# wh-xu/Hyper-Gen

Hardware: AMD Instinct MI355X
Metric: genomes/sec sketch (k=21,s=1500,D=4096) (higher is better)
Workload: dtype u64

## Files before the change

hyper-gen_amd/__init__.py:

```python
import ctypes as C
import os
import threading
import subprocess

import numpy as np

_HERE = os.path.dirname(os.path.abspath(__file__))
LIB_PATH = (os.environ.get("HYPERGEN_LIB") or None) or os.path.join(_HERE, "libhypergen_hip.so")
CLI_PATH = os.path.join(_HERE, "hyper-gen")

LAYOUT_SCALAR, LAYOUT_AVX2 = 0, 1
GATHER_PEER, GATHER_RCCL = 0, 1
ANI_MASH, ANI_CONTAINMENT, ANI_MAX_CONTAINMENT = 0, 1, 2
PAIRS_MASH, PAIRS_CONTAINMENT, PAIRS_MAX_CONTAINMENT, PAIRS_CONTAINMENT_REF = 1, 2, 4, 8
PAIRS_EMPTY = 0xFFFFFFFF
NORM_ACGT, NORM_U2T = 0, 1
(OK, ERR_INVALID, ERR_NO_DEVICE, ERR_HIP, ERR_OOM, ERR_CAPACITY, ERR_UNSUPPORTED, ERR_IO,
 ERR_INEXACT) = range(9)


T_NAMES = ("kmer", "sort", "encode", "dist_prep", "dist")
T_COUNT = len(T_NAMES)


class HgError(RuntimeError):
    def __init__(self, status, msg):
        super().__init__("hypergen status %d: %s" % (status, msg))
        self.status = status


class SketchParams(C.Structure):
    _fields_ = [("ksize", C.c_uint32), ("canonical", C.c_uint32), ("scaled", C.c_uint64),
                ("seed", C.c_uint64), ("hv_d", C.c_uint32), ("hv_layout", C.c_uint32),
                ("norm_mode", C.c_uint32), ("min_count", C.c_uint32)]


class AniHit(C.Structure):
    _fields_ = [("ref_idx", C.c_uint32), ("qry_idx", C.c_uint32), ("ani", C.c_float)]


ANI_HIT_DTYPE = np.dtype([("ref_idx", "<u4"), ("qry_idx", "<u4"), ("ani", "<f4")])
HAM_HIT_DTYPE = np.dtype([("ref_idx", "<u4"), ("qry_idx", "<u4"), ("dist", "<u4")])


class FileSketch(C.Structure):
    _fields_ = [("ksize", C.c_uint8), ("canonical", C.c_uint8), ("hv_quant_bits", C.c_uint8),
                ("pad", C.c_uint8), ("hv_norm_2", C.c_int32), ("scaled", C.c_uint64),
                ("seed", C.c_uint64), ("hv_d", C.c_uint64), ("file_str", C.c_char_p),
                ("hv", C.POINTER(C.c_int16)), ("hv_len", C.c_uint64)]


EXPORTS = [
    "hg_status_str", "hg_last_error", "hg_version", "hg_ctx_create", "hg_ctx_destroy",
    "hg_ctx_set_stream", "hg_ctx_reset_stream", "hg_ctx_sync", "hg_ctx_sketch_step_counts", "hg_sketch_plan_describe", "hg_logf_dev", "hg_ani_from_dots_dev", "hg_device_count", "hg_dev_alloc", "hg_dev_free",
    "hg_copy_h2d", "hg_copy_d2h", "hg_sketch_params_default", "hg_kmer_hash_sample",
    "hg_kmer_hash_sample_min_count",
    "hg_hv_encode", "hg_sketch_batch_dev", "hg_sketch_batch", "hg_dist_full", "hg_dist_full_dev",
    "hg_dist", "hg_dist_dev", "hg_sort_ani_hits", "hg_hv_quant_bits", "hg_hv_pack", "hg_hv_packed_bytes",
    "hg_hv_unpack", "hg_sketch_file_write", "hg_sketch_file_read", "hg_sketch_file_count",
    "hg_sketch_file_get", "hg_sketch_file_free", "hg_read_merge_seq", "hg_read_merge_seq_into", "hg_free",
    "hg_synth_genomes_dev", "hg_ctx_enable_timing", "hg_ctx_timings", "hg_ctx_last_kernel",
    "hg_hv_binarize_dev", "hg_hamming_full_dev", "hg_hamming_search_dev",
    "hg_ctx_set_debug", "hg_read_fastx_into", "hg_dist_block_dev", "hg_hamming_search_block_dev",
    "hg_multi_create", "hg_multi_destroy", "hg_multi_size", "hg_multi_ctx", "hg_multi_last_error", "hg_shard_range",
    "hg_multi_peer_report", "hg_multi_set_gather", "hg_multi_gather_mode", "hg_multi_gather_report",
    "hg_sketch_batch_multi", "hg_dist_multi", "hg_dist_multi_dev", "hg_hamming_search_multi",
    "hg_sort_ani_hits_dev", "hg_sort_ani_hits_staged", "hg_topk_per_query_dev", "hg_ctx_last_dist_path",
    "hg_ctx_last_hamming_path", "hg_read_fastx_pinned", "hg_pinned_free",
    "hg_sketch_stream_open", "hg_sketch_stream_push", "hg_sketch_stream_pop", "hg_sketch_stream_finish",
    "hg_sketch_stream_last_error", "hg_sketch_stream_close", "hg_sketch_stream_stats", "hg_device_numa_node", "hg_bind_thread_to_numa_node", "hg_dist_tile_order",
    "hg_sketch_stream_push_packed", "hg_pack2_size", "hg_pack2", "hg_unpack2_dev",
    "hg_sketch_stream_try_push", "hg_sketch_stream_max_pending",
    "hg_sketch_batch_dev_packed", "hg_pack2_batch_dev", "hg_pack2_dev",
    "hg_pack2s_size", "hg_pack2s", "hg_sketch_stream_push_packed_sparse",
    "hg_dist_ops_row_bytes", "hg_dist_ops_meta_bytes", "hg_dist_ops_padded_rows", "hg_dist_prep_ops_dev", "hg_dist_block_ops_dev",
    "hg_hv_packed_bytes_naive", "hg_hv_pack_naive", "hg_hv_unpack_naive", "hg_hv_payload_layout", "hg_hv_unpack_batch_dev",
    "hg_sketch_file_read_image", "hg_sketch_file_image", "hg_sketch_file_payload_offset",
    "hg_cluster_init_dev", "hg_cluster_add_hits_dev", "hg_cluster_finish_dev", "hg_cluster_dev", "hg_cluster",
    "hg_cluster_greedy_hits_dev", "hg_cluster_greedy_dev", "hg_cluster_greedy", "hg_ctx_cluster_greedy_rounds",
    "hg_cluster_setcover_hits_dev", "hg_cluster_setcover_dev", "hg_cluster_setcover", "hg_ctx_cluster_setcover_rounds",
    "hg_cluster_tree_hits_dev", "hg_cluster_tree_dev", "hg_cluster_tree", "hg_ctx_cluster_tree_rounds",
    "hg_cluster_average_matrix_dev", "hg_cluster_average_dev", "hg_cluster_average", "hg_ctx_cluster_average_rounds",
    "hg_cluster_stats_matrix_dev", "hg_cluster_stats_dev", "hg_cluster_stats",
    "hg_ctx_set_ani_metric", "hg_ctx_ani_metric", "hg_multi_set_ani_metric",
    "hg_search_topk_dev", "hg_search_topk_block_dev", "hg_search_topk", "hg_search_topk_merge", "hg_search_topk_multi_dev",
    "hg_ani_pairs_dev", "hg_ani_pairs",
]
SEARCH_TOPK_MAX = 64
CLUSTER_AVERAGE_MAX_N = 65536
STATS_NONE = 0xFFFFFFFF


class NodeStat(C.Structure):
    _fields_ = [("within_sum", C.c_uint64), ("within_min", C.c_uint32), ("within_min_idx", C.c_uint32),
                ("outside_max", C.c_uint32), ("outside_max_idx", C.c_uint32)]


class ClusterStat(C.Structure):
    _fields_ = [("within_sum", C.c_uint64), ("size", C.c_uint32), ("first", C.c_uint32), ("medoid", C.c_uint32),
                ("within_min", C.c_uint32), ("within_min_a", C.c_uint32), ("within_min_b", C.c_uint32),
                ("outside_max", C.c_uint32), ("outside_member", C.c_uint32), ("outside_idx", C.c_uint32), ("reserved", C.c_uint32)]


NODE_STAT_DTYPE = np.dtype([(name, np.uint64 if t is C.c_uint64 else np.uint32) for name, t in NodeStat._fields_])
CLUSTER_STAT_DTYPE = np.dtype([(name, np.uint64 if t is C.c_uint64 else np.uint32) for name, t in ClusterStat._fields_])


def source_stamp():
    import hashlib
    h = hashlib.sha256()
    src = os.path.join(_HERE, "csrc")
    files = sorted(f for f in os.listdir(src) if (f.endswith((".hip", ".h", ".cpp")) or f == "Makefile") and f != "hg_cli.cpp")
    for f in [os.path.join(src, x) for x in files] + [os.path.join(_HERE, "..", "include", "hypergen.h")]:
        h.update(os.path.basename(f).encode() + b"\0")
        h.update(open(f, "rb").read())
    return h.hexdigest()[:16]


def cli_source_stamp():
    import hashlib
    h = hashlib.sha256(source_stamp().encode())
    h.update(open(os.path.join(_HERE, "csrc", "hg_cli.cpp"), "rb").read())
    return h.hexdigest()[:16]


def build(force=False):
    if force:
        subprocess.check_call(["make", "-s", "-C", os.path.join(_HERE, "csrc"), "clean"])
    subprocess.check_call(["make", "-s", "-j4", "-C", os.path.join(_HERE, "csrc"), "all"])


_lib = None


def lib():
    global _lib
    if _lib is not None:
        return _lib
    if not os.path.exists(LIB_PATH):
        raise ImportError("libhypergen_hip.so is not built: run `python -c 'import __graft_entry__ as g; "
                          "g.build()'` (there is no CPU fallback)")
    L = C.CDLL(LIB_PATH)
    vp, sz = C.c_void_p, C.c_size_t
    u8p, u64p, i16p, i32p, u32p, f32p = (C.POINTER(t) for t in (
        C.c_uint8, C.c_uint64, C.c_int16, C.c_int32, C.c_uint32, C.c_float))
    sig = {
        "hg_status_str": (C.c_char_p, [C.c_int]),
        "hg_last_error": (C.c_char_p, [vp]),
        "hg_version": (C.c_char_p, []),
        "hg_ctx_create": (C.c_int, [C.c_int, C.POINTER(vp)]),
        "hg_ctx_destroy": (None, [vp]),
        "hg_ctx_set_stream": (C.c_int, [vp, vp]),
        "hg_ctx_reset_stream": (C.c_int, [vp]),
        "hg_ctx_sync": (C.c_int, [vp]),
        "hg_sketch_plan_describe": (C.c_int, [vp, vp, sz, C.c_uint32, C.c_uint64, C.POINTER(C.c_uint64), vp, sz]),
        "hg_logf_dev": (C.c_int, [vp, vp, C.c_uint32, sz, vp]),
        "hg_ani_from_dots_dev": (C.c_int, [vp, vp, vp, vp, sz, C.c_uint32, vp]),
        "hg_ctx_sketch_step_counts": (C.c_int, [vp, C.POINTER(C.c_uint64), C.POINTER(C.c_uint64), C.POINTER(C.c_uint64)]),
        "hg_device_count": (C.c_int, []),
        "hg_dev_alloc": (C.c_int, [vp, sz, C.POINTER(vp)]),
        "hg_dev_free": (C.c_int, [vp, vp]),
        "hg_copy_h2d": (C.c_int, [vp, vp, vp, sz]),
        "hg_copy_d2h": (C.c_int, [vp, vp, vp, sz]),
        "hg_sketch_params_default": (None, [C.POINTER(SketchParams)]),
        "hg_kmer_hash_sample": (C.c_int, [vp, vp, sz, C.c_uint32, C.c_uint64, C.c_uint64, C.c_int,
                                          C.c_uint32, vp, sz, C.POINTER(sz)]),
        "hg_kmer_hash_sample_min_count": (C.c_int, [vp, vp, sz, C.c_uint32, C.c_uint64, C.c_uint64, C.c_int,
                                                    C.c_uint32, C.c_uint32, vp, sz, C.POINTER(sz)]),
        "hg_hv_encode": (C.c_int, [vp, vp, sz, C.c_uint32, C.c_uint32, vp, C.POINTER(C.c_int32)]),
        "hg_sketch_batch_dev": (C.c_int, [vp, vp, vp, vp, sz, C.POINTER(SketchParams), vp, vp, vp]),
        "hg_sketch_batch": (C.c_int, [vp, C.POINTER(vp), C.POINTER(sz), sz, C.POINTER(SketchParams),
                                      vp, vp, vp]),
        "hg_dist_full": (C.c_int, [vp, vp, vp, sz, vp, vp, sz, C.c_uint32, C.c_uint32, vp]),
        "hg_dist_full_dev": (C.c_int, [vp, vp, vp, sz, vp, vp, sz, C.c_uint32, C.c_uint32, vp]),
        "hg_ani_pairs_dev": (C.c_int, [vp, vp, vp, sz, vp, vp, sz, C.c_uint32, C.c_uint32, vp, sz, C.c_uint32, vp, vp]),
        "hg_ani_pairs": (C.c_int, [vp, vp, vp, sz, vp, vp, sz, C.c_uint32, C.c_uint32, vp, sz, C.c_uint32, vp, vp]),
        "hg_dist": (C.c_int, [vp, vp, vp, sz, vp, vp, sz, C.c_uint32, C.c_uint32, C.c_int, C.c_float,
                              vp, sz, C.POINTER(sz)]),
        "hg_dist_dev": (C.c_int, [vp, vp, vp, sz, vp, vp, sz, C.c_uint32, C.c_uint32, C.c_int,
                                  C.c_float, vp, sz, C.POINTER(sz)]),
        "hg_sort_ani_hits": (None, [vp, sz, sz, C.c_int]),
        "hg_hv_quant_bits": (C.c_uint32, [vp, C.c_uint32]),
        "hg_hv_pack": (C.c_int, [vp, C.c_uint32, C.c_uint32, vp]),
        "hg_hv_packed_bytes": (sz, [C.c_uint32, C.c_uint32]),
        "hg_hv_unpack": (C.c_int, [vp, C.c_uint32, C.c_uint32, vp]),
        "hg_sketch_file_write": (C.c_int, [C.c_char_p, C.POINTER(FileSketch), sz]),
        "hg_sketch_file_read": (C.c_int, [C.c_char_p, C.POINTER(vp)]),
        "hg_sketch_file_count": (sz, [vp]),
        "hg_sketch_file_get": (C.POINTER(FileSketch), [vp, sz]),
        "hg_sketch_file_free": (None, [vp]),
        "hg_read_merge_seq": (C.c_int, [C.c_char_p, C.POINTER(vp), C.POINTER(sz)]),
        "hg_read_merge_seq_into": (C.c_int, [C.c_char_p, C.POINTER(vp), C.POINTER(sz), C.POINTER(sz)]),
        "hg_read_fastx_into": (C.c_int, [C.c_char_p, C.c_uint32, C.POINTER(vp), C.POINTER(sz), C.POINTER(sz)]),
        "hg_ctx_set_debug": (C.c_int, [vp, C.c_char_p, C.c_char_p]),
        "hg_free": (None, [vp]),
        "hg_read_fastx_pinned": (C.c_int, [C.c_char_p, C.c_uint32, C.POINTER(vp), C.POINTER(sz), C.POINTER(sz)]),
        "hg_pinned_free": (None, [vp]),
        "hg_device_numa_node": (C.c_int, [C.c_int]),
        "hg_bind_thread_to_numa_node": (C.c_int, [C.c_int, C.c_uint]),
        "hg_dist_tile_order": (C.c_int, [C.c_uint32, C.c_uint32, C.c_uint32, C.c_uint32, C.c_int, C.c_int, C.c_uint64, C.c_uint64,
                                         C.c_void_p, C.c_size_t, C.POINTER(C.c_size_t)]),
        "hg_sketch_stream_open": (C.c_int, [C.POINTER(C.c_int), C.c_int, C.POINTER(SketchParams), C.POINTER(vp)]),
        "hg_sketch_stream_push": (C.c_int, [vp, vp, sz, C.c_uint64]),
        "hg_sketch_stream_pop": (C.c_int, [vp, C.POINTER(C.c_uint64), vp, C.POINTER(C.c_int32), C.POINTER(C.c_uint32),
                                           C.POINTER(C.c_int)]),
        "hg_sketch_stream_push_packed": (C.c_int, [vp, vp, sz, C.c_uint64]),
        "hg_sketch_stream_try_push": (C.c_int, [vp, vp, sz, C.c_uint64, C.c_int]),
        "hg_sketch_stream_max_pending": (sz, [vp]),
        "hg_pack2_size": (sz, [sz]),
        "hg_pack2": (C.c_int, [vp, sz, C.c_uint32, vp]),
        "hg_unpack2_dev": (C.c_int, [vp, vp, sz, vp]),
        "hg_sketch_batch_dev_packed": (C.c_int, [vp, vp, vp, vp, sz, C.POINTER(SketchParams), vp, vp, vp]),
        "hg_pack2_batch_dev": (C.c_int, [vp, vp, vp, vp, sz, C.c_uint32, vp, vp]),
        "hg_pack2_dev": (C.c_int, [vp, vp, sz, C.c_uint32, vp]),
        "hg_dist_ops_row_bytes": (sz, [C.c_uint32]),
        "hg_dist_ops_meta_bytes": (sz, []),
        "hg_dist_ops_padded_rows": (sz, [sz]),
        "hg_dist_prep_ops_dev": (C.c_int, [vp, vp, sz, C.c_uint32, vp, vp, vp]),
        "hg_dist_block_ops_dev": (C.c_int, [vp, vp, vp, vp, sz, sz, vp, vp, sz, vp, vp, sz, sz, C.c_uint32, C.c_uint32, C.c_int,
                                            C.c_float, vp, sz, C.POINTER(sz)]),
        "hg_pack2s_size": (sz, [sz, sz]),
        "hg_pack2s": (C.c_int, [vp, sz, C.c_uint32, vp, sz, C.POINTER(sz)]),
        "hg_sketch_stream_push_packed_sparse": (C.c_int, [vp, vp, sz, sz, C.c_uint64]),
        "hg_sketch_stream_finish": (C.c_int, [vp]),
        "hg_sketch_stream_last_error": (C.c_char_p, [vp]),
        "hg_sketch_stream_close": (None, [vp]),
        "hg_sketch_stream_stats": (C.c_int, [vp, C.c_int, C.POINTER(C.c_double)]),
        "hg_ctx_last_dist_path": (C.c_int, [vp]),
        "hg_ctx_set_ani_metric": (C.c_int, [vp, C.c_int]),
        "hg_ctx_ani_metric": (C.c_int, [vp]),
        "hg_multi_set_ani_metric": (C.c_int, [vp, C.c_int]),
        "hg_ctx_last_hamming_path": (C.c_int, [vp]),
        "hg_sort_ani_hits_dev": (C.c_int, [vp, vp, sz, sz]),
        "hg_sort_ani_hits_staged": (C.c_int, [vp, vp, sz, sz]),
        "hg_topk_per_query_dev": (C.c_int, [vp, vp, sz, sz, C.c_uint32, vp, vp]),
        "hg_dist_block_dev": (C.c_int, [vp, vp, vp, sz, sz, vp, vp, sz, sz, C.c_uint32, C.c_uint32, C.c_int,
                                        C.c_float, vp, sz, C.POINTER(sz)]),
        "hg_hamming_search_block_dev": (C.c_int, [vp, vp, sz, sz, vp, sz, sz, C.c_uint32, C.c_uint32, vp, sz,
                                                  C.POINTER(sz)]),
        "hg_multi_create": (C.c_int, [C.POINTER(C.c_int), C.c_int, C.POINTER(vp)]),
        "hg_multi_destroy": (None, [vp]),
        "hg_multi_size": (C.c_int, [vp]),
        "hg_multi_ctx": (vp, [vp, C.c_int]),
        "hg_multi_last_error": (C.c_char_p, [vp]),
        "hg_multi_peer_report": (C.c_char_p, [vp]),
        "hg_multi_gather_report": (C.c_char_p, [vp]),
        "hg_multi_set_gather": (C.c_int, [vp, C.c_int]),
        "hg_multi_gather_mode": (C.c_int, [vp]),
        "hg_shard_range": (None, [sz, C.c_int, C.c_int, C.POINTER(sz), C.POINTER(sz)]),
        "hg_sketch_batch_multi": (C.c_int, [vp, C.POINTER(vp), C.POINTER(sz), sz, C.POINTER(SketchParams),
                                            vp, vp, vp]),
        "hg_dist_multi": (C.c_int, [vp, vp, vp, sz, vp, vp, sz, C.c_uint32, C.c_uint32, C.c_int, C.c_float,
                                    vp, sz, C.POINTER(sz)]),
        "hg_dist_multi_dev": (C.c_int, [vp, C.POINTER(vp), C.POINTER(vp), C.POINTER(sz), C.POINTER(vp),
                                        C.POINTER(vp), C.POINTER(sz), C.c_uint32, C.c_uint32, C.c_int,
                                        C.c_float, vp, sz, C.POINTER(sz)]),
        "hg_hamming_search_multi": (C.c_int, [vp, vp, sz, vp, sz, C.c_uint32, C.c_uint32, vp, sz, C.POINTER(sz)]),
        "hg_hv_binarize_dev": (C.c_int, [vp, vp, sz, C.c_uint32, vp]),
        "hg_hamming_full_dev": (C.c_int, [vp, vp, sz, vp, sz, C.c_uint32, vp]),
        "hg_hamming_search_dev": (C.c_int, [vp, vp, sz, vp, sz, C.c_uint32, C.c_uint32, vp, sz, C.POINTER(sz)]),
        "hg_ctx_enable_timing": (C.c_int, [vp, C.c_int]),
        "hg_ctx_last_kernel": (C.c_char_p, [vp, C.c_int]),
        "hg_ctx_timings": (C.c_int, [vp, C.POINTER(C.c_float), C.POINTER(C.c_uint32)]),
        "hg_synth_genomes_dev": (C.c_int, [vp, C.c_uint64, sz, C.c_uint64, C.c_uint32, C.c_uint32,
                                           C.c_uint64, vp]),
        "hg_hv_packed_bytes_naive": (sz, [C.c_uint32, C.c_uint32]),
        "hg_hv_pack_naive": (C.c_int, [vp, C.c_uint32, C.c_uint32, vp]),
        "hg_hv_unpack_naive": (C.c_int, [vp, C.c_uint32, C.c_uint32, vp]),
        "hg_hv_payload_layout": (C.c_int, [C.c_uint32, C.c_uint32, sz]),
        "hg_hv_unpack_batch_dev": (C.c_int, [vp, vp, sz, vp, vp, vp, sz, C.c_uint32, vp]),
        "hg_sketch_file_read_image": (C.c_int, [C.c_char_p, C.POINTER(vp)]),
        "hg_sketch_file_image": (vp, [vp, C.POINTER(sz)]),
        "hg_sketch_file_payload_offset": (C.c_uint64, [vp, sz]),
        "hg_cluster_init_dev": (C.c_int, [vp, vp, sz]),
        "hg_cluster_add_hits_dev": (C.c_int, [vp, vp, sz, vp, sz, C.c_float]),
        "hg_cluster_finish_dev": (C.c_int, [vp, vp, sz, vp, C.POINTER(sz)]),
        "hg_cluster_dev": (C.c_int, [vp, vp, vp, sz, C.c_uint32, C.c_uint32, C.c_float, vp, vp, C.POINTER(sz)]),
        "hg_cluster": (C.c_int, [vp, vp, vp, sz, C.c_uint32, C.c_uint32, C.c_float, vp, vp, C.POINTER(sz)]),
        "hg_cluster_greedy_hits_dev": (C.c_int, [vp, sz, vp, sz, C.c_float, vp, vp, vp, C.POINTER(sz)]),
        "hg_cluster_greedy_dev": (C.c_int, [vp, vp, vp, sz, C.c_uint32, C.c_uint32, C.c_float, vp, vp, vp, C.POINTER(sz)]),
        "hg_cluster_greedy": (C.c_int, [vp, vp, vp, sz, C.c_uint32, C.c_uint32, C.c_float, vp, vp, vp, C.POINTER(sz)]),
        "hg_ctx_cluster_greedy_rounds": (C.c_uint64, [vp]),
        "hg_cluster_setcover_hits_dev": (C.c_int, [vp, sz, vp, sz, C.c_float, vp, vp, vp, C.POINTER(sz)]),
        "hg_cluster_setcover_dev": (C.c_int, [vp, vp, vp, sz, C.c_uint32, C.c_uint32, C.c_float, vp, vp, vp, C.POINTER(sz)]),
        "hg_cluster_setcover": (C.c_int, [vp, vp, vp, sz, C.c_uint32, C.c_uint32, C.c_float, vp, vp, vp, C.POINTER(sz)]),
        "hg_ctx_cluster_setcover_rounds": (C.c_uint64, [vp]),
        "hg_cluster_tree_hits_dev": (C.c_int, [vp, sz, vp, sz, C.c_float, vp, sz, C.POINTER(sz), vp, vp, C.POINTER(sz)]),
        "hg_cluster_tree_dev": (C.c_int, [vp, vp, vp, sz, C.c_uint32, C.c_uint32, C.c_float, vp, sz, C.POINTER(sz), vp, vp, C.POINTER(sz)]),
        "hg_cluster_tree": (C.c_int, [vp, vp, vp, sz, C.c_uint32, C.c_uint32, C.c_float, vp, sz, C.POINTER(sz), vp, vp, C.POINTER(sz)]),
        "hg_ctx_cluster_tree_rounds": (C.c_uint64, [vp]),
        "hg_cluster_average_matrix_dev": (C.c_int, [vp, vp, sz, C.c_float, vp, vp, vp, vp, vp, C.POINTER(sz)]),
        "hg_cluster_average_dev": (C.c_int, [vp, vp, vp, sz, C.c_uint32, C.c_uint32, C.c_float, vp, vp, vp, vp, vp, C.POINTER(sz)]),
        "hg_cluster_average": (C.c_int, [vp, vp, vp, sz, C.c_uint32, C.c_uint32, C.c_float, vp, vp, vp, vp, vp, C.POINTER(sz)]),
        "hg_ctx_cluster_average_rounds": (C.c_uint64, [vp]),
        "hg_cluster_stats_matrix_dev": (C.c_int, [vp, vp, sz, vp, sz, vp, vp]),
        "hg_cluster_stats_dev": (C.c_int, [vp, vp, vp, sz, C.c_uint32, C.c_uint32, vp, sz, vp, vp]),
        "hg_cluster_stats": (C.c_int, [vp, vp, vp, sz, C.c_uint32, C.c_uint32, vp, sz, vp, vp]),
        "hg_search_topk_dev": (C.c_int, [vp, vp, vp, sz, vp, vp, sz, C.c_uint32, C.c_uint32, C.c_float, C.c_uint32, vp, vp]),
        "hg_search_topk_block_dev": (C.c_int, [vp, vp, vp, sz, sz, vp, vp, sz, sz, C.c_uint32, C.c_uint32, C.c_float, C.c_uint32,
                                               vp, vp]),
        "hg_search_topk": (C.c_int, [vp, vp, vp, sz, vp, vp, sz, C.c_uint32, C.c_uint32, C.c_float, C.c_uint32, vp, vp]),
        "hg_search_topk_merge": (C.c_int, [C.POINTER(vp), C.POINTER(vp), sz, sz, C.c_uint32, vp, vp]),
        "hg_search_topk_multi_dev": (C.c_int, [vp, C.POINTER(vp), C.POINTER(vp), C.POINTER(sz), C.POINTER(vp), C.POINTER(vp), sz,
                                               C.c_uint32, C.c_uint32, C.c_float, C.c_uint32, vp, vp]),
    }
    for name, (res, args) in sig.items():
        fn = getattr(L, name)
        fn.restype, fn.argtypes = res, args
    _lib = L
    return L


def _ptr(a):
    return C.c_void_p(a.ctypes.data) if isinstance(a, np.ndarray) else C.c_void_p(int(a))


def dist_tile_order(tiles_m, tiles_n, tile_rows=256, tile_cols=320, diagonal_first=False, symmetric=False, ref_off=0, qry_off=0):
    n = C.c_size_t(0)
    st = lib().hg_dist_tile_order(tiles_m, tiles_n, tile_rows, tile_cols, int(diagonal_first), int(symmetric), ref_off, qry_off,
                                  None, 0, C.byref(n))
    if st not in (OK, ERR_CAPACITY):
        raise HgError(st, "hg_dist_tile_order")
    out = np.zeros(max(n.value, 1), np.uint32)
    st = lib().hg_dist_tile_order(tiles_m, tiles_n, tile_rows, tile_cols, int(diagonal_first), int(symmetric), ref_off, qry_off,
                                  C.c_void_p(out.ctypes.data), out.size, C.byref(n))
    if st != OK:
        raise HgError(st, "hg_dist_tile_order")
    return out[: n.value]


def default_params(**kw):
    p = SketchParams()
    lib().hg_sketch_params_default(C.byref(p))
    for k, v in kw.items():
        setattr(p, k, v)
    return p


default_debug = {}


class Context:

    def __init__(self, device=0):
        self._h = C.c_void_p()
        st = lib().hg_ctx_create(device, C.byref(self._h))
        if st != OK:
            raise HgError(st, lib().hg_last_error(None).decode())
        for k, v in default_debug.items():
            self.set_debug(k, v)

    def close(self):
        if self._h:
            lib().hg_ctx_destroy(self._h)
            self._h = C.c_void_p()

    def __enter__(self):
        return self

    def __exit__(self, *a):
        self.close()

    def __del__(self):
        try:
            self.close()
        except Exception:
            pass

    def _ck(self, st, allow=()):
        if st != OK and st not in allow:
            raise HgError(st, lib().hg_last_error(self._h).decode())
        return st

    def set_stream(self, stream_handle):
        self._ck(lib().hg_ctx_set_stream(self._h, C.c_void_p(stream_handle or 0)))

    def set_debug(self, key, value):
        self._ck(lib().hg_ctx_set_debug(self._h, key.encode(), str(value).encode()))

    def reset_stream(self):
        self._ck(lib().hg_ctx_reset_stream(self._h))

    def sync(self):
        self._ck(lib().hg_ctx_sync(self._h))

    def logf_dev(self, d_out, n, d_x=None, first_bits=0):
        self._ck(lib().hg_logf_dev(self._h, C.c_void_p(d_x or 0), first_bits, n, C.c_void_p(d_out)))

    def ani_from_dots_dev(self, d_dot, d_nr, d_nq, n, ksize, d_ani):
        self._ck(lib().hg_ani_from_dots_dev(self._h, C.c_void_p(d_dot), C.c_void_p(d_nr), C.c_void_p(d_nq), n, ksize, C.c_void_p(d_ani)))

    def sketch_step_counts(self):
        a, b, c = C.c_uint64(), C.c_uint64(), C.c_uint64()
        self._ck(lib().hg_ctx_sketch_step_counts(self._h, C.byref(a), C.byref(b), C.byref(c)))
        return int(a.value), int(b.value), int(c.value)

    def last_kernel(self, cls):
        return lib().hg_ctx_last_kernel(self._h, T_NAMES.index(cls)).decode()

    def enable_timing(self, on=True):
        self._ck(lib().hg_ctx_enable_timing(self._h, int(on)))

    def timings(self):
        ms = (C.c_float * T_COUNT)()
        n = (C.c_uint32 * T_COUNT)()
        self._ck(lib().hg_ctx_timings(self._h, ms, n))
        return {name: (float(ms[i]), int(n[i])) for i, name in enumerate(T_NAMES)}

    def kmer_hash_sample(self, seq, ksize=21, scaled=1500, seed=123, canonical=True,
                         norm=NORM_ACGT, threshold=None, cap=None, min_count=1):
        a = np.ascontiguousarray(np.frombuffer(bytes(seq), np.uint8) if not isinstance(seq, np.ndarray) else seq,
                                 dtype=np.uint8)
        thr = (2**64 - 1) // scaled if threshold is None else threshold
        cap = cap if cap is not None else max(1024, a.size // max(1, scaled) * 2 + 1024)
        while True:
            out = np.zeros(max(cap, 1), np.uint64)
            n = C.c_size_t(0)
            if min_count > 1:
                st = lib().hg_kmer_hash_sample_min_count(self._h, _ptr(a) if a.size else None, a.size, ksize,
                                                         C.c_uint64(thr), C.c_uint64(seed), int(canonical), norm, min_count,
                                                         _ptr(out), cap, C.byref(n))
            else:
                st = lib().hg_kmer_hash_sample(self._h, _ptr(a) if a.size else None, a.size, ksize,
                                               C.c_uint64(thr), C.c_uint64(seed), int(canonical), norm,
                                               _ptr(out), cap, C.byref(n))
            if st == ERR_CAPACITY:
                cap = n.value
                continue
            self._ck(st)
            return out[: n.value].copy()

    def unpack2_dev(self, d_blob, n_bps, d_out):
        self._ck(lib().hg_unpack2_dev(self._h, C.c_void_p(d_blob), n_bps, C.c_void_p(d_out)))

    def hv_encode(self, hashes, hv_d=4096, layout=LAYOUT_AVX2):
        h = np.ascontiguousarray(hashes, dtype=np.uint64)
        hv = np.zeros(hv_d, np.int16)
        n2 = C.c_int32(0)
        self._ck(lib().hg_hv_encode(self._h, _ptr(h) if h.size else None, h.size, hv_d, layout,
                                    _ptr(hv), C.byref(n2)))
        return hv, int(n2.value)

    def sketch_batch(self, seqs, params=None):
        p = params or default_params()
        arrs = [np.ascontiguousarray(s, dtype=np.uint8) if isinstance(s, np.ndarray)
                else np.frombuffer(bytes(s), np.uint8) for s in seqs]
        n = len(arrs)
        ptrs = (C.c_void_p * max(n, 1))(*[a.ctypes.data if a.size else None for a in arrs])
        lens = (C.c_size_t * max(n, 1))(*[a.size for a in arrs])
        hv = np.zeros((n, p.hv_d), np.int16)
        n2 = np.zeros(n, np.int32)
        nh = np.zeros(n, np.uint32)
        self._ck(lib().hg_sketch_batch(self._h, ptrs, lens, n, C.byref(p), _ptr(hv), _ptr(n2), _ptr(nh)))
        return hv, n2, nh

    def dist_full(self, ref_hv, ref_n2, qry_hv, qry_n2, ksize=21):
        r = np.ascontiguousarray(ref_hv, np.int16)
        q = np.ascontiguousarray(qry_hv, np.int16)
        rn = np.ascontiguousarray(ref_n2, np.int32)
        qn = np.ascontiguousarray(qry_n2, np.int32)
        out = np.zeros((r.shape[0], q.shape[0]), np.float32)
        self._ck(lib().hg_dist_full(self._h, _ptr(r), _ptr(rn), r.shape[0], _ptr(q), _ptr(qn),
                                    q.shape[0], r.shape[1], ksize, _ptr(out)))
        return out

    def dist(self, ref_hv, ref_n2, qry_hv, qry_n2, ksize=21, symmetric=False, ani_th=85.0, cap=None):
        r = np.ascontiguousarray(ref_hv, np.int16)
        q = np.ascontiguousarray(qry_hv, np.int16)
        rn = np.ascontiguousarray(ref_n2, np.int32)
        qn = np.ascontiguousarray(qry_n2, np.int32)
        cap = cap if cap is not None else max(1024, r.shape[0] * q.shape[0] // 8)
        while True:
            out = np.zeros(cap, ANI_HIT_DTYPE)
            n = C.c_size_t(0)
            st = lib().hg_dist(self._h, _ptr(r), _ptr(rn), r.shape[0], _ptr(q), _ptr(qn), q.shape[0],
                               r.shape[1], ksize, int(symmetric), C.c_float(ani_th), _ptr(out), cap,
                               C.byref(n))
            if st == ERR_CAPACITY:
                cap = n.value
                continue
            self._ck(st)
            return out[: n.value].copy()

    def sketch_batch_dev(self, d_seq, offsets, lens, params, d_hv, d_norm2, d_nhash):
        off = np.ascontiguousarray(offsets, np.uint64)
        ln = np.ascontiguousarray(lens, np.uint64)
        self._ck(lib().hg_sketch_batch_dev(self._h, _ptr(d_seq), _ptr(off), _ptr(ln), off.size,
                                           C.byref(params), _ptr(d_hv), _ptr(d_norm2), _ptr(d_nhash)))

    def sketch_batch_dev_packed(self, d_blobs, offsets, n_bps, params, d_hv, d_norm2, d_nhash):
        off = np.ascontiguousarray(offsets, np.uint64)
        ln = np.ascontiguousarray(n_bps, np.uint64)
        self._ck(lib().hg_sketch_batch_dev_packed(self._h, _ptr(d_blobs), _ptr(off), _ptr(ln), off.size,
                                                  C.byref(params), _ptr(d_hv), _ptr(d_norm2), _ptr(d_nhash)))

    def pack2_batch_dev(self, d_seq, offsets, lens, d_blobs, blob_offsets, norm_mode=NORM_ACGT):
        off = np.ascontiguousarray(offsets, np.uint64)
        ln = np.ascontiguousarray(lens, np.uint64)
        bo = np.ascontiguousarray(blob_offsets, np.uint64)
        self._ck(lib().hg_pack2_batch_dev(self._h, _ptr(d_seq), _ptr(off), _ptr(ln), off.size, norm_mode, _ptr(d_blobs), _ptr(bo)))

    def pack2_dev(self, d_seq, n_bps, d_blob, norm_mode=NORM_ACGT):
        self._ck(lib().hg_pack2_dev(self._h, C.c_void_p(d_seq), n_bps, norm_mode, C.c_void_p(d_blob)))

    def synth_genomes_dev(self, first, n, L, stride, d_out, cluster_size=100, sub_ppm_per_member=1000):
        done = 0
        while done < n:
            m = min(n - done, 32768)
            self._ck(lib().hg_synth_genomes_dev(self._h, first + done, m, L, cluster_size, sub_ppm_per_member,
                                                stride, C.c_void_p(int(d_out) + done * stride)))
            done += m

    def hv_binarize_dev(self, d_hv, n, hv_d, d_bits):
        self._ck(lib().hg_hv_binarize_dev(self._h, _ptr(d_hv), n, hv_d, _ptr(d_bits)))

    def hamming_full_dev(self, d_ref, R, d_qry, Q, hv_d, d_out):
        self._ck(lib().hg_hamming_full_dev(self._h, _ptr(d_ref), R, _ptr(d_qry), Q, hv_d, _ptr(d_out)))

    def hamming_search_dev(self, d_ref, R, d_qry, Q, hv_d, max_dist, d_out, cap):
        n = C.c_size_t(0)
        st = lib().hg_hamming_search_dev(self._h, _ptr(d_ref), R, _ptr(d_qry), Q, hv_d, max_dist, _ptr(d_out), cap,
                                         C.byref(n))
        self._ck(st, allow=(ERR_CAPACITY,))
        return n.value, st

    def dist_full_dev(self, d_ref, d_rn, R, d_qry, d_qn, Q, hv_d, ksize, d_out):
        self._ck(lib().hg_dist_full_dev(self._h, _ptr(d_ref), _ptr(d_rn), R, _ptr(d_qry), _ptr(d_qn), Q,
                                        hv_d, ksize, _ptr(d_out)))

    def dist_block_dev(self, d_ref, d_rn, R, ref_off, d_qry, d_qn, Q, qry_off, hv_d, ksize, symmetric, ani_th,
                       d_out, cap):
        n = C.c_size_t(0)
        st = lib().hg_dist_block_dev(self._h, _ptr(d_ref), _ptr(d_rn), R, ref_off, _ptr(d_qry), _ptr(d_qn), Q,
                                     qry_off, hv_d, ksize, int(symmetric), C.c_float(ani_th), _ptr(d_out), cap,
                                     C.byref(n))
        self._ck(st, allow=(ERR_CAPACITY,))
        return n.value, st

    def dist_prep_ops_dev(self, d_hv, rows, hv_d, d_ops, d_meta, d_flag):
        self._ck(lib().hg_dist_prep_ops_dev(self._h, _ptr(d_hv), rows, hv_d, _ptr(d_ops), _ptr(d_meta), _ptr(d_flag)))

    def dist_block_ops_dev(self, d_ref_ops, d_ref_meta, d_rn, R, ref_off, d_ref_index, d_flags, n_flags, d_qry, d_qn, Q, qry_off,
                           hv_d, ksize, symmetric, ani_th, d_out, cap):
        n = C.c_size_t(0)
        st = lib().hg_dist_block_ops_dev(self._h, _ptr(d_ref_ops), _ptr(d_ref_meta), _ptr(d_rn), R, ref_off,
                                         _ptr(d_ref_index) if d_ref_index else None, _ptr(d_flags) if d_flags else None, n_flags,
                                         _ptr(d_qry), _ptr(d_qn), Q, qry_off, hv_d, ksize, int(symmetric), C.c_float(ani_th),
                                         _ptr(d_out), cap, C.byref(n))
        self._ck(st, allow=(ERR_CAPACITY, ERR_INEXACT))
# ... 470 lines not shown
    a = np.ascontiguousarray(seq, np.uint8)
    n = a.size
    cap = lib().hg_pack2_size(n) if cap is None else cap
    out = np.empty(max(cap, 16), np.uint8)
    size = C.c_size_t(0)
    st = lib().hg_pack2s(_ptr(a), n, norm_mode, _ptr(out), out.size, C.byref(size))
    if st == ERR_CAPACITY:
        return None
    if st != OK:
        raise HgError(st, "hg_pack2s")
    return out[:size.value]


def pack2(seq, norm_mode=0, in_place=False):
    a = np.ascontiguousarray(seq, np.uint8)
    n = a.size
    size = lib().hg_pack2_size(n)
    if in_place:
        buf = np.zeros(max(n, size), np.uint8)
        buf[:n] = a
        st = lib().hg_pack2(_ptr(buf), n, norm_mode, _ptr(buf))
        out = buf[:size]
    else:
        out = np.empty(size, np.uint8)
        st = lib().hg_pack2(_ptr(a), n, norm_mode, _ptr(out))
    if st != OK:
        raise HgError(st, "hg_pack2")
    return out


class PinnedReader:

    def __init__(self, slots=1):
        self._p = [C.c_void_p() for _ in range(slots)]
        self._cap = [C.c_size_t(0) for _ in range(slots)]

    def read(self, path, slot=0, mode=READ_MERGE):
        n = C.c_size_t(0)
        st = lib().hg_read_fastx_pinned(os.fsencode(path), mode, C.byref(self._p[slot]), C.byref(self._cap[slot]), C.byref(n))
        if st != OK:
            raise HgError(st, "hg_read_fastx_pinned(%s)" % path)
        if not n.value:
            return np.zeros(0, np.uint8)
        return np.ctypeslib.as_array(C.cast(self._p[slot], C.POINTER(C.c_uint8)), shape=(n.value,))

    def close(self):
        for p in self._p:
            if p:
                lib().hg_pinned_free(p)
                p.value = None

    def __enter__(self):
        return self

    def __exit__(self, *a):
        self.close()


class SketchStream:

    def __init__(self, device_ids=(0,), params=None):
        self.params = params or default_params()
        ids = (C.c_int * len(device_ids))(*device_ids)
        self._h = C.c_void_p()
        st = lib().hg_sketch_stream_open(ids, len(device_ids), C.byref(self.params), C.byref(self._h))
        if st != OK:
            raise HgError(st, "hg_sketch_stream_open: " + lib().hg_last_error(None).decode())
        self._keep = {}
        self._next = 0
        self._ready = []
        self._lock = threading.Lock()

    def _check(self, st, what):
        if st != OK:
            raise HgError(st, what + ": " + lib().hg_sketch_stream_last_error(self._h).decode())

    def _push(self, a, n_bps, tag, packed):
        with self._lock:
            iid = self._next
            self._next += 1
            self._keep[iid] = (tag, a)
        try:
            while True:
                st = lib().hg_sketch_stream_try_push(self._h, _ptr(a), n_bps, iid, int(packed))
                if st != ERR_CAPACITY:
                    break
                r = self._pop_c()
                if r is not None:
                    with self._lock:
                        self._ready.append(r)
        except BaseException:
            with self._lock:
                self._keep.pop(iid, None)
            raise
        if st != OK:
            with self._lock:
                self._keep.pop(iid, None)
        self._check(st, "hg_sketch_stream_try_push")

    def push(self, seq, tag):
        a = np.ascontiguousarray(seq, np.uint8)
        self._push(a, a.size, tag, 0)

    def push_packed(self, blob, n_bps, tag):
        a = np.ascontiguousarray(blob, np.uint8)
        assert a.size >= lib().hg_pack2_size(n_bps)
        self._push(a, n_bps, tag, 1)

    def push_packed_sparse(self, blob, n_bps, tag):
        a = np.ascontiguousarray(blob, np.uint8)
        tab = (((n_bps + 3) // 4) + 15) & ~15
        if n_bps and (a.size < tab + 8 or a.size < lib().hg_pack2s_size(n_bps, int(a[tab: tab + 4].view("<u4")[0]))):
            raise HgError(ERR_INVALID, "push_packed_sparse: the buffer is shorter than the blob it claims to hold")
        self._push(a, n_bps, tag, 2)

    def finish(self):
        self._check(lib().hg_sketch_stream_finish(self._h), "hg_sketch_stream_finish")

    def _pop_c(self):
        iid, n2, nh, got = C.c_uint64(), C.c_int32(), C.c_uint32(), C.c_int()
        hv = np.empty(self.params.hv_d, np.int16)
        self._check(lib().hg_sketch_stream_pop(self._h, C.byref(iid), _ptr(hv), C.byref(n2), C.byref(nh), C.byref(got)),
                    "hg_sketch_stream_pop")
        if not got.value:
            return None
        with self._lock:
            tag, _ = self._keep.pop(iid.value)
        return tag, hv, n2.value, nh.value

    def pop(self):
        with self._lock:
            if self._ready:
                return self._ready.pop(0)
        return self._pop_c()

    def stats(self, engine=0):
        out = (C.c_double * 6)()
        self._check(lib().hg_sketch_stream_stats(self._h, engine, out), "hg_sketch_stream_stats")
        return dict(zip(("uploader_idle_s", "uploader_no_chunk_s", "uploader_copy_s", "compute_idle_s", "compute_busy_s",
                         "chunks"), out))

    def close(self):
        if self._h:
            lib().hg_sketch_stream_close(self._h)
            self._h = C.c_void_p()

    def __enter__(self):
        return self

    def __exit__(self, *a):
        self.close()


def sketch_plan_describe(offsets, lens, ksize=21, scaled=1500):
    off = np.ascontiguousarray(offsets, np.uint64)
    ln = np.ascontiguousarray(lens, np.uint64)
    counts = (C.c_uint64 * 6)()
    st = lib().hg_sketch_plan_describe(_ptr(off), _ptr(ln), off.size, ksize, scaled, counts, None, 0)
    if st != OK:
        raise HgError(st, "hg_sketch_plan_describe")
    d = dict(zip(("items", "workgroups", "hit_slots", "max_cap", "max_expect", "item_tiles"), (int(x) for x in counts)))
    gf = None
    if ksize <= 32 and d["items"]:
        gf = np.zeros(d["workgroups"] + 1, np.uint32)
        st = lib().hg_sketch_plan_describe(_ptr(off), _ptr(ln), off.size, ksize, scaled, counts, _ptr(gf), gf.size)
        if st != OK:
            raise HgError(st, "hg_sketch_plan_describe")
    return d, gf


def write_sketch_file(path, records):
    arr = (FileSketch * max(len(records), 1))()
    keep = []
    for i, r in enumerate(records):
        hv = np.ascontiguousarray(r["hv"], np.int16)
        name = r["file_str"].encode()
        keep += [hv, name]
        arr[i] = FileSketch(r["ksize"], int(bool(r["canonical"])), r["hv_quant_bits"], 0, r["hv_norm_2"],
                            r["scaled"], r["seed"], r["hv_d"], name,
                            hv.ctypes.data_as(C.POINTER(C.c_int16)), hv.size)
    st = lib().hg_sketch_file_write(os.fsencode(path), arr, len(records))
    if st != OK:
        raise HgError(st, "hg_sketch_file_write(%s)" % path)


def read_sketch_file(path):
    h = C.c_void_p()
    st = lib().hg_sketch_file_read(os.fsencode(path), C.byref(h))
    if st != OK:
        raise HgError(st, "hg_sketch_file_read(%s)" % path)
    try:
        out = []
        for i in range(lib().hg_sketch_file_count(h)):
            r = lib().hg_sketch_file_get(h, i).contents
            hv = np.ctypeslib.as_array(r.hv, shape=(r.hv_len,)).copy() if r.hv_len else np.zeros(0, np.int16)
            out.append(dict(ksize=r.ksize, scaled=r.scaled, canonical=bool(r.canonical), seed=r.seed,
                            hv_d=r.hv_d, hv_quant_bits=r.hv_quant_bits, hv_norm_2=r.hv_norm_2,
                            file_str=r.file_str.decode(), hv=hv))
        return out
    finally:
        lib().hg_sketch_file_free(h)
```

hyper-gen_amd/csrc/hg_api.hip:

```cpp
#include <atomic>
#include <chrono>
#include <cstdlib>
#include <cstring>
#include <new>
#include <string>
#include <thread>

#include "hg_internal.h"

static thread_local std::string g_create_err;

hg_status hg_fail(hg_ctx *ctx, hg_status s, const std::string &msg) {
  if (ctx) ctx->err = msg;
  else g_create_err = msg;
  return s;
}

extern "C" const char *hg_status_str(hg_status s) {
  switch (s) {
    case HG_OK: return "ok";
    case HG_ERR_INVALID: return "invalid argument";
    case HG_ERR_NO_DEVICE: return "no usable HIP device";
    case HG_ERR_HIP: return "HIP runtime error";
    case HG_ERR_OOM: return "out of memory";
    case HG_ERR_CAPACITY: return "output capacity too small";
    case HG_ERR_UNSUPPORTED: return "unsupported parameters";
    case HG_ERR_IO: return "I/O error";
    case HG_ERR_INEXACT: return "no exact device path";
  }
  return "unknown";
}

extern "C" const char *hg_last_error(const hg_ctx *ctx) {
  return ctx ? ctx->err.c_str() : g_create_err.c_str();
}

extern "C" const char *hg_version(void) { return "hypergen-hip 0.1.0 (gfx950)"; }

extern "C" int hg_device_count(void) {
  int n = 0;
  if (hipGetDeviceCount(&n) != hipSuccess) return 0;
  return n;
}

extern "C" hg_status hg_ctx_create(int device_id, hg_ctx **out) {
  if (!out) return hg_fail(nullptr, HG_ERR_INVALID, "out == NULL");
  *out = nullptr;
  int n = 0;
  hipError_t e = hipGetDeviceCount(&n);
  if (e != hipSuccess || n <= 0)
    return hg_fail(nullptr, HG_ERR_NO_DEVICE,
                   std::string("hipGetDeviceCount: ") + (e == hipSuccess ? "0 devices" : hipGetErrorString(e)));
  if (device_id < 0 || device_id >= n)
    return hg_fail(nullptr, HG_ERR_NO_DEVICE, "device id out of range");
  hg_ctx *c = new (std::nothrow) hg_ctx();
  if (!c) return hg_fail(nullptr, HG_ERR_OOM, "ctx allocation");
  c->device = device_id;
  if ((e = hipSetDevice(device_id)) != hipSuccess ||
      (e = hipStreamCreateWithFlags(&c->own_stream, hipStreamNonBlocking)) != hipSuccess) {
    delete c;
    return hg_fail(nullptr, HG_ERR_HIP, std::string("ctx setup: ") + hipGetErrorString(e));
  }
  c->stream = c->own_stream;
  hipDeviceProp_t prop;
  if (hipGetDeviceProperties(&prop, device_id) == hipSuccess) c->n_cu = prop.multiProcessorCount;
  *out = c;
  return HG_OK;
}

extern "C" void hg_ctx_destroy(hg_ctx *c) {
  if (!c) return;
  (void)hipSetDevice(c->device);
  (void)hipStreamSynchronize(c->stream);
  hg_ctx::Buf *bufs[] = {&c->w_items, &c->w_gmeta, &c->w_hits, &c->w_cnt, &c->w_seq, &c->w_hv, &c->w_hits2, &c->w_lsort, &c->w_redo, &c->w_pk, &c->w_pktab,
                         &c->w_misc, &c->w_f16a, &c->w_f16b, &c->w_stats, &c->w_ani, &c->w_hv2, &c->w_cen,
                         &c->w_n2a, &c->w_n2b, &c->w_sorthits, &c->w_clu_res, &c->w_clu, &c->w_clu_hits, &c->w_grd, &c->w_setcover, &c->w_tree, &c->w_average, &c->w_cstats, &c->w_srch_blk, &c->w_srch_lists, &c->w_srch_state, &c->w_srch_out, &c->w_i8a, &c->w_i8b, &c->w_i8misc};
  for (auto *b : bufs)
    if (b->p) (void)hipFree(b->p);
  for (auto &t : c->tile_tabs) {
    if (t.dev.p) (void)hipFree(t.dev.p);
    if (t.uploaded) (void)hipEventDestroy(t.uploaded);
  }
  for (auto &t : c->t_pending) {
    if (t.own_e0) (void)hipEventDestroy(t.e0);
    (void)hipEventDestroy(t.e1);
  }
  for (auto e : c->t_pool) (void)hipEventDestroy(e);
  if (c->h_res) (void)hipHostFree(c->h_res);
  if (c->h_pin) (void)hipHostFree(c->h_pin);
  if (c->h_chk) (void)hipHostFree(c->h_chk);
  if (c->h_plan) (void)hipHostFree(c->h_plan);
  if (c->plan_uploaded) (void)hipEventDestroy(c->plan_uploaded);
  for (auto e : c->copy_events) (void)hipEventDestroy(e);
  for (int i = 0; i < 2; ++i) {
    if (c->pack_buf[i]) (void)hipHostFree(c->pack_buf[i]);
    if (c->pack_ev[i]) (void)hipEventDestroy(c->pack_ev[i]);
  }
  if (c->copy_stream) (void)hipStreamDestroy(c->copy_stream);
  if (c->own_stream) (void)hipStreamDestroy(c->own_stream);
  delete c;
}

static hg_status switch_stream(hg_ctx *c, hipStream_t to) {
  if (to == c->stream) return HG_OK;
  HG_ENTER(c);
  HG_HIP(c, hipStreamSynchronize(c->stream));
  c->stream = to;
  return HG_OK;
}

extern "C" hg_status hg_ctx_set_stream(hg_ctx *c, void *hip_stream) {
  if (!c) return HG_ERR_INVALID;
  return switch_stream(c, reinterpret_cast<hipStream_t>(hip_stream));
}

extern "C" hg_status hg_ctx_reset_stream(hg_ctx *c) {
  if (!c) return HG_ERR_INVALID;
  return switch_stream(c, c->own_stream);
}

extern "C" int hg_ctx_last_dist_path(const hg_ctx *c) { return c ? c->last_dist_path : -1; }

extern "C" hg_status hg_ctx_set_ani_metric(hg_ctx *c, int metric) {
  if (!c) return HG_ERR_INVALID;
  if (metric != HG_ANI_MASH && metric != HG_ANI_CONTAINMENT && metric != HG_ANI_MAX_CONTAINMENT)
    return hg_fail(c, HG_ERR_INVALID, "unknown ANI metric " + std::to_string(metric));
  c->ani_metric = metric;
  return HG_OK;
}

extern "C" int hg_ctx_ani_metric(const hg_ctx *c) { return c ? c->ani_metric : HG_ANI_MASH; }

extern "C" hg_status hg_ctx_set_debug(hg_ctx *c, const char *key, const char *value) {
  if (!c || !key) return HG_ERR_INVALID;
  const std::string k = key, v = value ? value : "";
  if (k == "dist_tile") c->dbg_dist_tile = v;
  else if (k == "sort_test_buckets") c->dbg_sort_buckets = std::atoi(v.c_str());
  else if (k == "pair_limit") c->dbg_pair_limit = std::strtoull(v.c_str(), nullptr, 10);
  else if (k == "cluster_hit_cap") c->dbg_cluster_hit_cap = std::strtoull(v.c_str(), nullptr, 10);
  else if (k == "tree_rounds") c->dbg_tree_rounds = std::strtoull(v.c_str(), nullptr, 10);
  else if (k == "setcover_rounds") c->dbg_setcover_rounds = std::strtoull(v.c_str(), nullptr, 10);
  else if (k == "greedy_rounds") c->dbg_greedy_rounds = std::strtoull(v.c_str(), nullptr, 10);
  else if (k == "average_rounds") c->dbg_average_rounds = std::strtoull(v.c_str(), nullptr, 10);
  else if (k == "average_block_rows") c->dbg_average_block_rows = std::strtoull(v.c_str(), nullptr, 10);
  else if (k == "stats_block_rows") c->dbg_stats_block_rows = std::strtoull(v.c_str(), nullptr, 10);
  else if (k == "search_block_rows") c->dbg_search_block_rows = std::strtoull(v.c_str(), nullptr, 10);
  else if (k == "dist_path") c->dbg_dist_path = v;
  else if (k == "dist_order") c->dbg_dist_order = v;
  else if (k == "ham_path") c->dbg_ham_path = v;
  else if (k == "hostfed") c->dbg_hostfed = v;
  else if (k == "hostfed_stage_bytes") c->dbg_hostfed_stage_bytes = std::strtoull(v.c_str(), nullptr, 10);
  else if (k == "sketch_path") c->dbg_sketch_path = v;
  else if (k == "kmer_input") c->dbg_kmer_input = v;
  else return hg_fail(c, HG_ERR_INVALID, "unknown debug key " + k);
  return HG_OK;
}

extern "C" hg_status hg_ctx_sync(hg_ctx *c) {
  if (!c) return HG_ERR_INVALID;
  HG_ENTER(c);
  HG_HIP(c, hipStreamSynchronize(c->stream));
  return HG_OK;
}

extern "C" hg_status hg_ctx_sketch_step_counts(hg_ctx *c, uint64_t *sync_free, uint64_t *synchronous, uint64_t *redone) {
  if (!c) return HG_ERR_INVALID;
  if (sync_free) *sync_free = c->n_fast_steps;
  if (synchronous) *synchronous = c->n_sync_steps;
  if (redone) *redone = c->n_redone_steps;
  return HG_OK;
}

static hipEvent_t take_event(hg_ctx *c) {
  if (!c->t_pool.empty()) {
    hipEvent_t e = c->t_pool.back();
    c->t_pool.pop_back();
    return e;
  }
  hipEvent_t e = nullptr;
  if (hipEventCreate(&e) != hipSuccess) return nullptr;
  return e;
}

hg_timed::hg_timed(hg_ctx *ctx, int cls_, int after_cls) : c(ctx), cls(cls_) {
  hipEvent_t chain = c->t_chain;
  c->t_chain = nullptr;
  if (!c->timing) return;
  if (after_cls >= 0 && chain && c->t_chain_cls == after_cls) e0 = chain, own_e0 = false;
  else e0 = take_event(c);
  e1 = take_event(c);
  if (e0 && own_e0) (void)hipEventRecord(e0, c->stream);
}
hg_timed::~hg_timed() {
  if (!e0 || !e1) return;
  (void)hipEventRecord(e1, c->stream);
  c->t_pending.push_back({e0, e1, cls, own_e0});
  c->t_chain = e1, c->t_chain_cls = cls;
}

extern "C" hg_status hg_ctx_enable_timing(hg_ctx *c, int on) {
  if (!c) return HG_ERR_INVALID;
  c->timing = on != 0;
  c->t_chain = nullptr, c->t_chain_cls = -1;
  return HG_OK;
}

extern "C" const char *hg_ctx_last_kernel(const hg_ctx *c, int cls) {
  return (c && cls >= 0 && cls < HG_T_COUNT) ? c->last_kernel[cls].c_str() : "";
}

extern "C" hg_status hg_ctx_timings(hg_ctx *c, float ms_sum[HG_T_COUNT], uint32_t launches[HG_T_COUNT]) {
  if (!c || !ms_sum || !launches) return HG_ERR_INVALID;
  for (int i = 0; i < HG_T_COUNT; ++i) ms_sum[i] = 0.f, launches[i] = 0;
  hipError_t first_err = hipSuccess;
  const char *first_what = "";
  for (auto &t : c->t_pending) {
    if (first_err != hipSuccess) break;
    hipError_t e = hipEventSynchronize(t.e1);
    float ms = 0.f;
    if (e == hipSuccess) e = hipEventElapsedTime(&ms, t.e0, t.e1);
    if (e != hipSuccess) {
      first_err = e, first_what = "hg_ctx_timings: event read";
      break;
    }
    if (t.cls >= 0 && t.cls < HG_T_COUNT) ms_sum[t.cls] += ms, launches[t.cls] += 1;
  }
  for (auto &t : c->t_pending) {
    if (t.own_e0) c->t_pool.push_back(t.e0);
    c->t_pool.push_back(t.e1);
  }
  c->t_pending.clear();
  c->t_chain = nullptr;
  if (first_err != hipSuccess) return hg_fail(c, HG_ERR_HIP, std::string(first_what) + ": " + hipGetErrorString(first_err));
  return HG_OK;
}

hg_status hg_ensure(hg_ctx *c, hg_ctx::Buf &b, size_t bytes) {
  if (bytes <= b.cap) return HG_OK;
  HG_HIP(c, hipStreamSynchronize(c->stream));
  if (b.p) {
    (void)hipFree(b.p);
    b.p = nullptr;
    b.cap = 0;
  }
  size_t want = bytes + bytes / 4 + 256;
  hipError_t e = hipMalloc(&b.p, want);
  if (e != hipSuccess) {
    b.p = nullptr;
    return hg_fail(c, HG_ERR_OOM, "hipMalloc(" + std::to_string(want) + "): " + hipGetErrorString(e));
  }
  b.cap = want;
  return HG_OK;
}

namespace {
__global__ void publish_words_kernel(uint32_t *__restrict__ src, uint32_t n, volatile uint32_t *dst, uint32_t seq, uint32_t zero_n) {
  if (threadIdx.x < n) dst[threadIdx.x] = src[threadIdx.x];
  if (threadIdx.x < zero_n) src[threadIdx.x] = 0u;
  __threadfence_system();
  __syncthreads();
  if (threadIdx.x == 0) {
    dst[16] = seq;
    __threadfence_system();
  }
}
}

hg_status hg_publish_words(hg_ctx *c, uint32_t *d_words, uint32_t n, const uint32_t **out, uint32_t zero_n) {
  if (n > 16 || zero_n > 64) return hg_fail(c, HG_ERR_INVALID, "hg_publish_words: at most 16 words");
  if (!c->h_res) {
    void *p = nullptr;
    hipError_t e = hipHostMalloc(&p, 32 * sizeof(uint32_t), hipHostMallocCoherent);
    if (e != hipSuccess) return hg_fail(c, HG_ERR_OOM, std::string("hipHostMalloc: ") + hipGetErrorString(e));
    c->h_res = static_cast<uint32_t *>(p);
    std::memset(c->h_res, 0, 32 * sizeof(uint32_t));
  }
  const uint32_t seq = ++c->res_seq ? c->res_seq : ++c->res_seq;
  hipLaunchKernelGGL(publish_words_kernel, dim3(1), dim3(64), 0, c->stream, d_words, n, c->h_res, seq, zero_n);
  HG_HIP(c, hipGetLastError());
  volatile uint32_t *flag = c->h_res + 16;
  const auto t0 = std::chrono::steady_clock::now();
  bool seen = false;
  for (uint32_t spins = 0; !seen; ++spins) {
    if (*flag == seq) {
      seen = true;
      break;
    }
#if defined(__x86_64__) || defined(__i386__)
    __builtin_ia32_pause();
#else
    std::this_thread::yield();
#endif
    if ((spins & 0x3ff) == 0x3ff &&
        std::chrono::steady_clock::now() - t0 > std::chrono::microseconds(800))
      break;
  }
  if (!seen) {
    const hipError_t e = hipStreamSynchronize(c->stream);
    if (e != hipSuccess) return hg_fail(c, HG_ERR_HIP, std::string("hipStreamSynchronize: ") + hipGetErrorString(e));
    if (*flag != seq) return hg_fail(c, HG_ERR_HIP, "hg_publish_words: the stream finished without publishing");
  }
  std::atomic_thread_fence(std::memory_order_acquire);
  *out = c->h_res;
  return HG_OK;
}

hg_status hg_ensure_pinned(hg_ctx *c, size_t bytes) {
  if (bytes <= c->h_pin_cap) return HG_OK;
  HG_HIP(c, hipStreamSynchronize(c->stream));
  if (c->h_pin) (void)hipHostFree(c->h_pin);
  c->h_pin = nullptr, c->h_pin_cap = 0;
  size_t want = bytes + bytes / 4 + 4096;
  hipError_t e = hipHostMalloc(&c->h_pin, want, hipHostMallocDefault);
  if (e != hipSuccess) return hg_fail(c, HG_ERR_OOM, std::string("hipHostMalloc: ") + hipGetErrorString(e));
  c->h_pin_cap = want;
  return HG_OK;
}

extern "C" hg_status hg_dev_alloc(hg_ctx *c, size_t bytes, void **dptr) {
  if (!c || !dptr) return HG_ERR_INVALID;
  HG_ENTER(c);
  hipError_t e = hipMalloc(dptr, bytes ? bytes : 1);
  if (e != hipSuccess) return hg_fail(c, HG_ERR_OOM, std::string("hipMalloc: ") + hipGetErrorString(e));
  return HG_OK;
}
// ... 38 lines not shown
```

hyper-gen_amd/csrc/hg_internal.h:

```cpp
#pragma once
#include <hip/hip_runtime.h>
#include <stddef.h>
#include <stdint.h>

#include <algorithm>
#include <atomic>
#include <memory>
#include <string>
#include <vector>

#include "../../include/hypergen.h"
#include "hg_pack2.h"

struct hg_sketch_plan {
  std::vector<uint64_t> offs, lens, masks;
  std::vector<uint32_t> caps;
  uint32_t ksize = 0;
  bool packed = false;
  uint64_t scaled = 0, total_slots = 0;
  uint32_t max_cap = 0;
  uint32_t max_expect = 0;
  uint32_t max_hits = 0;
  size_t n_items = 0;
  size_t n_groups = 0;
};
struct hg_genome_batch {
  const uint8_t *d_seq = nullptr;
  const uint64_t *offsets = nullptr, *lens = nullptr;
  const uint64_t *mask_offs = nullptr;
  size_t n = 0;
  bool packed = false;
};
struct hg_sketch_out {
  int16_t *d_hv = nullptr;
  int32_t *d_norm2 = nullptr;
  uint32_t *d_nhash = nullptr;
};
struct hg_sketch_pending {
  bool active = false;
  uint32_t seq = 0;
  int slot = 0;
  std::shared_ptr<const hg_sketch_plan> plan;
  hg_genome_batch batch;
  hg_sketch_params p{};
  hg_sketch_out out;
};

struct hg_ctx {
  int device = 0;
  hipStream_t own_stream = nullptr;
  hipStream_t stream = nullptr;
  std::string err;
  int n_cu = 256;

  struct Buf {
    void *p = nullptr;
    size_t cap = 0;
  };
  Buf w_items;
  Buf w_gmeta;
  Buf w_hits;
  Buf w_cnt;
  Buf w_hits2;
  Buf w_lsort;
  Buf w_redo;
  Buf w_pk;
  Buf w_pktab;
  Buf w_seq;
  Buf w_hv;
  Buf w_misc;
  const void *misc_zeroed = nullptr;
  Buf w_f16a;
  Buf w_f16b;
  Buf w_stats;
  Buf w_ani;
  Buf w_hv2;
  Buf w_n2a, w_n2b;
  Buf w_i8a, w_i8b, w_i8misc;
  struct I8Pad {
    const void *ptr = nullptr;
    uint32_t rows = 0, padded = 0, pitch = 0;
  } i8_pad[2];
  Buf w_cen;
  struct TileTab {
    uint32_t tiles_m = 0, tiles_n = 0, bm = 0, bn = 0, flags = 0, n_slots = 0;
    uint64_t ref_off = 0, qry_off = 0, used = 0;
    Buf dev;
    std::vector<uint32_t> host;
    hipEvent_t uploaded = nullptr;
  } tile_tabs[8];
  uint64_t tile_tab_clock = 0;
  std::string last_kernel_cen;
  const void *cen_sig_ref = nullptr, *cen_sig_qry = nullptr;
  uint32_t cen_sig_r = 0, cen_sig_q = 0, cen_sig_d = 0;
  int last_ham_path = -1;
  std::string last_kernel[HG_T_COUNT];
  std::string last_kernel_i8;
  std::string last_kernel_win;
  int ani_metric = HG_ANI_MASH;
  int last_dist_path = -1;
  const void *i8_sig_ref = nullptr, *i8_sig_qry = nullptr;
  uint32_t i8_sig_r = 0, i8_sig_q = 0, i8_sig_d = 0;
  uint32_t i8_skip = 0;
  Buf w_sorthits;
  Buf w_clu_res;
  Buf w_clu;
  Buf w_clu_hits;
  Buf w_grd;
  uint64_t greedy_rounds = 0;
  Buf w_setcover;
  uint64_t setcover_rounds = 0;
  Buf w_tree;
  uint64_t tree_rounds = 0;
  Buf w_average;
  uint64_t average_rounds = 0;
  Buf w_cstats;
  Buf w_srch_blk;
  Buf w_srch_lists;
  Buf w_srch_state;
  Buf w_srch_out;
  bool timing = false;
  struct TimedLaunch {
    hipEvent_t e0, e1;
    int cls;
    bool own_e0;
  };
  hipEvent_t t_chain = nullptr;
  int t_chain_cls = -1;
  std::vector<TimedLaunch> t_pending;
  std::vector<hipEvent_t> t_pool;
  std::shared_ptr<hg_sketch_plan> plan;
  hipEvent_t plan_uploaded = nullptr;
  bool plan_upload_pending = false;
  void *h_plan = nullptr;
  size_t h_plan_cap = 0;
  hg_sketch_pending pending;
  uint32_t *h_chk = nullptr;
  uint32_t chk_seq = 0;
  uint64_t n_fast_steps = 0, n_sync_steps = 0, n_redone_steps = 0;
  hipStream_t copy_stream = nullptr;
  std::vector<hipEvent_t> copy_events;
  void *pack_buf[2] = {nullptr, nullptr};
  size_t pack_cap[2] = {0, 0};
  hipEvent_t pack_ev[2] = {nullptr, nullptr};
  bool pack_used[2] = {false, false};
  const void *pad_a_ptr = nullptr, *pad_b_ptr = nullptr;
  uint32_t pad_a_rows = 0, pad_a_ldk = 0, pad_b_rows = 0, pad_b_ldk = 0;
  std::vector<const void *> lds_attr_done;
  std::string dbg_dist_tile, dbg_dist_path, dbg_ham_path, dbg_dist_order, dbg_kmer_input, dbg_hostfed, dbg_sketch_path;
  int dbg_sort_buckets = 0;
  uint64_t dbg_cluster_hit_cap = 0;
  uint64_t dbg_greedy_rounds = 0;
  uint64_t dbg_setcover_rounds = 0;
  uint64_t dbg_tree_rounds = 0;
  uint64_t dbg_average_rounds = 0;
  uint64_t dbg_average_block_rows = 0;
  uint64_t dbg_stats_block_rows = 0;
  uint64_t dbg_search_block_rows = 0;
  uint64_t dbg_hostfed_stage_bytes = 0;
  uint64_t dbg_pair_limit = 0;
  void *h_pin = nullptr;
  size_t h_pin_cap = 0;
  uint32_t *h_res = nullptr;
  uint32_t res_seq = 0;
};

hg_status hg_fail(hg_ctx *ctx, hg_status s, const std::string &msg);
hg_status hg_ensure(hg_ctx *ctx, hg_ctx::Buf &b, size_t bytes);
hg_status hg_ensure_pinned(hg_ctx *ctx, size_t bytes);
hg_status hg_publish_words(hg_ctx *ctx, uint32_t *d_words, uint32_t n, const uint32_t **out, uint32_t zero_n = 0);

struct hg_timed {
  hg_ctx *c;
  hipEvent_t e0 = nullptr, e1 = nullptr;
  int cls;
  bool own_e0 = true;
  hg_timed(hg_ctx *ctx, int cls_, int after_cls = -1);
  ~hg_timed();
};

#define HG_HIP(ctx, expr)                                                              \
  do {                                                                                 \
    hipError_t e__ = (expr);                                                           \
    if (e__ != hipSuccess)                                                             \
      return hg_fail((ctx), HG_ERR_HIP,                                                \
                     std::string(#expr) + ": " + hipGetErrorString(e__));              \
  } while (0)

hg_status hg_sketch_resolve(hg_ctx *ctx, bool *redone = nullptr);
#define HG_ENTER(ctx)                                        \
  do {                                                       \
    HG_HIP((ctx), hipSetDevice((ctx)->device));              \
    const hg_status s__ = hg_sketch_resolve((ctx));          \
    if (s__ != HG_OK) return s__;                            \
  } while (0)

struct hg_genome_meta {
  uint64_t seq_off;
  uint64_t n_bps;
  uint64_t hit_off;
  uint32_t hit_cap;
  uint32_t item_first;
  uint64_t mask_off;
};
hg_status hg_sketch_batch_dev_packed_masks(hg_ctx *c, const uint8_t *d_blobs, const uint64_t *code_offs, const uint64_t *mask_offs,
                                           const uint64_t *n_bps, size_t n, const hg_sketch_params *p, int16_t *d_hv,
                                           int32_t *d_norm2, uint32_t *d_nhash);

uint32_t hg_kmer_item_starts(uint32_t ksize);
const char *hg_kmer_kernel_name(uint32_t ksize, bool canonical, bool packed);

hipError_t hg_launch_kmer_sample(hipStream_t st, const uint8_t *d_seq, const hg_genome_meta *d_meta,
                                 const uint32_t *d_item_genome, uint32_t n_items, uint32_t ksize,
                                 uint64_t threshold, uint64_t seed, bool canonical, uint32_t norm_mode,
                                 uint64_t *d_hits, uint32_t *d_cnt, bool packed = false, const uint32_t *d_group_first = nullptr,
                                 uint32_t n_groups = 0);
uint32_t hg_kmer_tile_starts(uint32_t ksize);
uint32_t hg_kmer_item_tiles(uint32_t ksize);
hipError_t hg_launch_pack2(hipStream_t st, const uint8_t *d_seq, const uint64_t *d_tab, uint32_t n, uint32_t blocks_max,
                           uint32_t u2t, uint8_t *d_blobs);
hipError_t hg_launch_unpack2_jobs(hipStream_t st, const uint8_t *d_pk, uint8_t *d_out, const UnpackJob *d_jobs, uint32_t n_jobs, uint32_t n_blocks);
hipError_t hg_launch_expand_runs(hipStream_t st, uint8_t *d_pk, const SparseJob *d_jobs, uint32_t n_jobs, uint32_t n_blocks);

#define HG_SORT_LDS_MAX_KEYS 8192u

inline void hg_note_launch(std::string *launched, const char *name) {
  if (!launched) return;
  if (!launched->empty()) *launched += " + ";
  *launched += name;
}
inline bool attr_done_on_this_device(std::atomic<uint64_t> &mask, bool set) {
  int dev = 0;
  if (hipGetDevice(&dev) != hipSuccess || dev < 0 || dev > 63) return false;
  if (set) mask.fetch_or(1ull << dev);
  return (mask.load() >> dev) & 1;
}
uint32_t hg_sort_lds_keys(uint32_t max_cap);
hipError_t hg_launch_sort_unique_todo(hipStream_t st, const hg_genome_meta *d_meta, const uint32_t *d_todo, uint32_t n_todo,
                                      uint64_t *d_hits, const uint32_t *d_cnt, uint32_t *d_ndistinct, uint32_t max_cap,
                                      uint64_t threshold, uint32_t min_count, std::string *launched = nullptr);
hipError_t hg_launch_sort_unique(hipStream_t st, const hg_genome_meta *d_meta, uint32_t n_genomes,
                                 uint64_t *d_hits, const uint32_t *d_cnt, uint32_t *d_ndistinct,
                                 uint32_t max_cap, uint64_t threshold, uint32_t min_count, uint32_t *d_flags = nullptr,
                                 std::string *launched = nullptr);
#define HG_STEP_OVERFLOW 1u
#define HG_STEP_LARGE_SET 2u
hipError_t hg_launch_sort_unique_rest(hipStream_t st, const hg_genome_meta *d_meta, uint32_t n_genomes, uint64_t *d_hits,
                                      const uint32_t *d_cnt, uint32_t *d_ndistinct, uint32_t done_cap, uint32_t max_cap,
                                      uint64_t threshold, uint32_t min_count, std::string *launched = nullptr);
hipError_t hg_launch_sketch_finish(hipStream_t st, const uint32_t *d_ndistinct, uint32_t *d_nhash, uint32_t n_genomes,
                                   const uint32_t *d_flags, uint32_t *h_slot, uint32_t seq, std::string *launched = nullptr);

struct hg_bucket_job {
  uint64_t hit_off;
  uint64_t mul;
  uint32_t n;
  uint32_t P;
  uint32_t bucket_first, chunk_first;
  uint32_t genome, pad;
};
#define HG_BUCKET_CHUNK 4096u
hipError_t hg_launch_sort_large(hipStream_t st, const hg_bucket_job *d_jobs, uint32_t n_jobs,
                                const uint32_t *d_chunk_job, uint32_t n_chunks, const uint32_t *d_bucket_job,
                                uint32_t n_buckets, uint32_t *d_bk, uint64_t *d_hits, uint64_t *d_tmp,
                                uint32_t *d_ndistinct, uint32_t bucket_cap_keys, uint32_t min_count,
                                std::string *launched = nullptr);
hipError_t hg_launch_sort_inplace(hipStream_t st, const hg_genome_meta *d_meta, const uint32_t *d_todo,
                                  uint32_t n_todo, uint64_t *d_hits, const uint32_t *d_cnt, uint32_t *d_ndistinct,
                                  uint32_t min_count, std::string *launched = nullptr);

#define HG_ENC_SLAB 32768u
#define HG_ENC_WAVE_MAX 16368u
struct hg_encode_split {
  const uint32_t *d_items;
  const uint32_t *d_genomes;
  uint32_t *d_accum;
  uint32_t n_items, n_genomes;
};
hipError_t hg_launch_encode(hipStream_t st, const hg_genome_meta *d_meta, uint32_t n_genomes,
                            const uint64_t *d_hits, const uint32_t *d_ndistinct, uint32_t hv_d,
                            uint32_t layout, int16_t *d_hv, int32_t *d_norm2, const hg_encode_split *split = nullptr,
                            uint32_t max_hashes = ~0u ,
                            std::string *launched = nullptr);

struct hg_dist_args {
  const int16_t *ref_hv;
  const int32_t *ref_n2;
  const int16_t *qry_hv;
  const int32_t *qry_n2;
  uint32_t R, Q, hv_d, ksize;
  float *ani_out;
  hg_ani_hit *hits;
  uint32_t *hit_count;
  uint32_t hit_cap;
  float ani_th;
  int symmetric;
  int ani_metric = HG_ANI_MASH;
  uint32_t ref_off = 0, qry_off = 0;
  const uint8_t *ref_ops = nullptr;
  const void *ref_meta = nullptr;
  const uint32_t *ref_flags = nullptr;
  uint32_t n_flags = 0;
  const uint32_t *ref_index = nullptr;
};
size_t hg_dist_ops_row_bytes_impl(uint32_t hv_d);
size_t hg_dist_ops_meta_bytes_impl();
size_t hg_dist_ops_padded_rows_impl(size_t n);
hg_status hg_run_dist_prep_ops(hg_ctx *c, const int16_t *d_hv, uint32_t rows, uint32_t hv_d, uint8_t *d_ops, void *d_meta,
                               uint32_t *d_flag);
enum : uint32_t {
  HG_RES_COUNT = 0,
  HG_RES_VERDICT = 1,
  HG_RES_WINDOW = 2,
  HG_RES_I8_CTRL = 4,
  HG_RES_MARK = 8,
  HG_RES_I8_KSTEPS = 9,
  HG_RES_WORDS = 16
};
hg_status hg_run_dist(hg_ctx *ctx, const hg_dist_args &a, uint32_t *d_res = nullptr, int *speculated = nullptr);

inline uint64_t hg_pair_limit(const hg_ctx *c) { return c->dbg_pair_limit ? c->dbg_pair_limit : 0xFFFFFFFFull; }
template <class Hit, class Once>
hg_status hg_run_blocks(hg_ctx *c, size_t split, size_t other, Hit *d_out, size_t cap, size_t *n_out, Once once) {
  const size_t per = std::max<size_t>(1, (size_t)(hg_pair_limit(c) / (uint64_t)other));
  size_t total = 0;
  bool full = false;
  *n_out = 0;
  for (size_t i0 = 0; i0 < split; i0 += per) {
    const size_t n = std::min(per, split - i0), room = total < cap ? cap - total : 0;
    size_t got = 0;
    const hg_status bs = once(i0, n, d_out ? d_out + std::min(total, cap) : nullptr, room, &got);
    if (bs == HG_ERR_CAPACITY) full = true;
    else if (bs != HG_OK) return bs;
    total += got;
  }
  *n_out = total;
  if (full || total > cap) return hg_fail(c, HG_ERR_CAPACITY, "hit buffer too small");
  return HG_OK;
}

hg_status hg_run_hamming_mfma(hg_ctx *c, const uint32_t *d_ref_bits, uint32_t R, const uint32_t *d_qry_bits, uint32_t Q,
                              uint32_t hv_d, uint32_t max_dist, hg_ham_hit *d_hits, uint32_t *d_count, uint32_t cap,
                              uint32_t ref_off, uint32_t qry_off, int path );
```

hyper-gen_amd/csrc/hg_kmer_kernels.hip:

```cpp
#include <cstdlib>
#include <utility>

#include "hg_internal.h"

namespace {

constexpr uint64_t P0 = 0xEC99BF0D8372CAABull;
constexpr uint64_t P1 = 0x82434FE90EDCEF39ull;
constexpr uint64_t P2 = 0xD4F06DB99D67BE4Bull;
constexpr uint64_t P3 = 0xBD9CACC22C6E9571ull;
constexpr uint64_t P4 = 0x9C06FAF4D023E3ABull;
constexpr uint64_t P5 = 0xC060724A8424F345ull;
constexpr uint64_t P6 = 0xCB5AF53AE3AAAC31ull;

__device__ __forceinline__ uint64_t mk64(uint32_t lo, uint32_t hi) {
  return (uint64_t)lo | ((uint64_t)hi << 32);
}
#ifndef HG_ROT_ALIGNBIT
#define HG_ROT_ALIGNBIT 1
#endif
__device__ __forceinline__ uint64_t rot64(uint64_t v, unsigned s) {
#if HG_ROT_ALIGNBIT
  if (__builtin_constant_p(s) && s > 0 && s < 64 && s != 32) {
    const uint32_t lo = (uint32_t)v, hi = (uint32_t)(v >> 32);
// ... 151 lines not shown
#define HG_KS_HEAD2(R0, R1, R2, R3) HG_KS_RD(R0, "o0") HG_KS_RD4(R1, "o0") HG_KS_RD(R2, "o1") HG_KS_RD4(R3, "o1")
#define HG_KS_HEAD3(R0, R1, R2, R3, R4, R5) HG_KS_HEAD2(R0, R1, R2, R3) HG_KS_RD(R4, "o2") HG_KS_RD(R5, "o3")
#define HG_KS_TAIL_O1(RL, RH, OL, OH) "ds_read_u8 v" RL ", %[base] offset:%[" OL "]\n\tv_mov_b32 v" RH ", 0"
#define HG_KS_TAIL_O2(RL, RH, OL, OH) "ds_read_u16 v" RL ", %[base] offset:%[" OL "]\n\tv_mov_b32 v" RH ", 0"
#define HG_KS_TAIL_O3(RL, RH, OL, OH) "ds_read_b32 v" RL ", %[base] offset:%[" OL "]\n\tv_mov_b32 v" RH ", 0"
#define HG_KS_TAIL_O4(RL, RH, OL, OH) HG_KS_TAIL_O3(RL, RH, OL, OH)
#define HG_KS_TAIL_E1(RL, RH, OL, OH) HG_KS_RD(RL, OL) "ds_read_u8 v" RH ", %[base] offset:%[" OH "]"
#define HG_KS_TAIL_E2(RL, RH, OL, OH) HG_KS_RD(RL, OL) "ds_read_u16 v" RH ", %[base] offset:%[" OH "]"
#define HG_KS_TAIL_E3(RL, RH, OL, OH) HG_KS_RD(RL, OL) "ds_read_b32 v" RH ", %[base] offset:%[" OH "]"
#define HG_KS_TAIL_E4(RL, RH, OL, OH) HG_KS_TAIL_E3(RL, RH, OL, OH)
#define HG_KS_READ_TEXT_51(R0, R1, R2, R3, R4, R5, R6, R7) HG_KS_HEAD2(R0, R1, R2, R3) HG_KS_TAIL_O1(R4, R5, "o2", "o3")
#define HG_KS_READ_TEXT_52(R0, R1, R2, R3, R4, R5, R6, R7) HG_KS_HEAD2(R0, R1, R2, R3) HG_KS_TAIL_O2(R4, R5, "o2", "o3")
#define HG_KS_READ_TEXT_53(R0, R1, R2, R3, R4, R5, R6, R7) HG_KS_HEAD2(R0, R1, R2, R3) HG_KS_TAIL_O3(R4, R5, "o2", "o3")
#define HG_KS_READ_TEXT_54(R0, R1, R2, R3, R4, R5, R6, R7) HG_KS_HEAD2(R0, R1, R2, R3) HG_KS_TAIL_O4(R4, R5, "o2", "o3")
#define HG_KS_READ_TEXT_61(R0, R1, R2, R3, R4, R5, R6, R7) HG_KS_HEAD2(R0, R1, R2, R3) HG_KS_TAIL_E1(R4, R5, "o2", "o3")
#define HG_KS_READ_TEXT_62(R0, R1, R2, R3, R4, R5, R6, R7) HG_KS_HEAD2(R0, R1, R2, R3) HG_KS_TAIL_E2(R4, R5, "o2", "o3")
#define HG_KS_READ_TEXT_63(R0, R1, R2, R3, R4, R5, R6, R7) HG_KS_HEAD2(R0, R1, R2, R3) HG_KS_TAIL_E3(R4, R5, "o2", "o3")
#define HG_KS_READ_TEXT_64(R0, R1, R2, R3, R4, R5, R6, R7) HG_KS_HEAD2(R0, R1, R2, R3) HG_KS_TAIL_E4(R4, R5, "o2", "o3")
#define HG_KS_READ_TEXT_71(R0, R1, R2, R3, R4, R5, R6, R7) HG_KS_HEAD3(R0, R1, R2, R3, R4, R5) HG_KS_TAIL_O1(R6, R7, "o4", "o5")
#define HG_KS_READ_TEXT_72(R0, R1, R2, R3, R4, R5, R6, R7) HG_KS_HEAD3(R0, R1, R2, R3, R4, R5) HG_KS_TAIL_O2(R6, R7, "o4", "o5")
#define HG_KS_READ_TEXT_73(R0, R1, R2, R3, R4, R5, R6, R7) HG_KS_HEAD3(R0, R1, R2, R3, R4, R5) HG_KS_TAIL_O3(R6, R7, "o4", "o5")
#define HG_KS_READ_TEXT_74(R0, R1, R2, R3, R4, R5, R6, R7) HG_KS_HEAD3(R0, R1, R2, R3, R4, R5) HG_KS_TAIL_O4(R6, R7, "o4", "o5")
#define HG_KS_READ_TEXT_81(R0, R1, R2, R3, R4, R5, R6, R7) HG_KS_HEAD3(R0, R1, R2, R3, R4, R5) HG_KS_TAIL_E1(R6, R7, "o4", "o5")
#define HG_KS_READ_TEXT_82(R0, R1, R2, R3, R4, R5, R6, R7) HG_KS_HEAD3(R0, R1, R2, R3, R4, R5) HG_KS_TAIL_E2(R6, R7, "o4", "o5")
#define HG_KS_READ_TEXT_83(R0, R1, R2, R3, R4, R5, R6, R7) HG_KS_HEAD3(R0, R1, R2, R3, R4, R5) HG_KS_TAIL_E3(R6, R7, "o4", "o5")
#define HG_KS_READ_TEXT_84(R0, R1, R2, R3, R4, R5, R6, R7) HG_KS_HEAD3(R0, R1, R2, R3, R4, R5) HG_KS_TAIL_E4(R6, R7, "o4", "o5")
#define HG_KS_W "s_waitcnt lgkmcnt(0)\n\t"
#define HG_KS_WM(R) HG_KS_W "v_and_b32 v" R ", 0xffffff, v" R "\n\t"
#define HG_KS_WAIT_TEXT_51(R0, R1, R2, R3, R4, R5, R6, R7) HG_KS_W
#define HG_KS_WAIT_TEXT_52(R0, R1, R2, R3, R4, R5, R6, R7) HG_KS_W
#define HG_KS_WAIT_TEXT_53(R0, R1, R2, R3, R4, R5, R6, R7) HG_KS_WM(R4)
#define HG_KS_WAIT_TEXT_54(R0, R1, R2, R3, R4, R5, R6, R7) HG_KS_W
#define HG_KS_WAIT_TEXT_61(R0, R1, R2, R3, R4, R5, R6, R7) HG_KS_W
#define HG_KS_WAIT_TEXT_62(R0, R1, R2, R3, R4, R5, R6, R7) HG_KS_W
#define HG_KS_WAIT_TEXT_63(R0, R1, R2, R3, R4, R5, R6, R7) HG_KS_WM(R5)
#define HG_KS_WAIT_TEXT_64(R0, R1, R2, R3, R4, R5, R6, R7) HG_KS_W
#define HG_KS_WAIT_TEXT_71(R0, R1, R2, R3, R4, R5, R6, R7) HG_KS_W
#define HG_KS_WAIT_TEXT_72(R0, R1, R2, R3, R4, R5, R6, R7) HG_KS_W
#define HG_KS_WAIT_TEXT_73(R0, R1, R2, R3, R4, R5, R6, R7) HG_KS_WM(R6)
#define HG_KS_WAIT_TEXT_74(R0, R1, R2, R3, R4, R5, R6, R7) HG_KS_W
#define HG_KS_WAIT_TEXT_81(R0, R1, R2, R3, R4, R5, R6, R7) HG_KS_W
#define HG_KS_WAIT_TEXT_82(R0, R1, R2, R3, R4, R5, R6, R7) HG_KS_W
#define HG_KS_WAIT_TEXT_83(R0, R1, R2, R3, R4, R5, R6, R7) HG_KS_WM(R7)
#define HG_KS_WAIT_TEXT_84(R0, R1, R2, R3, R4, R5, R6, R7) HG_KS_W
#define HG_KS_REGS0 ("56", "57", "58", "59", "60", "61", "90", "91")
#define HG_KS_REGS1 ("62", "63", "64", "65", "66", "67", "92", "93")
#define HG_KS_PAIRS0 ("v[56:57]", "v[58:59]", "v[60:61]", "v[90:91]")
#define HG_KS_PAIRS1 ("v[62:63]", "v[64:65]", "v[66:67]", "v[92:93]")
#define HG_KS_APPLY(M, ARGS) M ARGS
#define HG_KS_FINAL(AP, AL, AH, BP, BL, BH)                                                                          \
  "v_alignbit_b32 v86, " BL ", " BH ", 9\n\t"                                                                        \
  "v_alignbit_b32 v87, " BH ", " BL ", 9\n\t"                                                                        \
  "v_lshl_add_u64 v[72:73], v[86:87], 0, " AP "\n\t"                                                                 \
  "v_alignbit_b32 v86, " AH ", " AL ", 23\n\t"                                                                       \
  "v_alignbit_b32 v87, " AL ", " AH ", 23\n\t"                                                                       \
  "v_lshl_add_u64 v[88:89], v[86:87], 0, " BP "\n\t"                                                                 \
  HG_KS_LO64("v72", "v73", "%[p0l]", "%[p0h]", "v[74:75]", "v74", "v75")                                             \
  HG_KS_LO64("v88", "v89", "%[p6l]", "%[p6h]", "v[84:85]", "v84", "v85")                                             \
  "v_xor_b32_e32 v72, v74, v84\n\t"                                                                                  \
  "v_xor_b32_e32 v73, v75, v85\n\t"                                                                                  \
  "v_mad_u64_u32 v[74:75], %[junk], v72, %[p5l], 0\n\t"                                                              \
  "v_mov_b32 v68, v75\n\t"                                                                                           \
  "v_mad_u64_u32 v[76:77], %[junk], v73, %[p5l], v[68:69]\n\t"                                                       \
  "v_mad_u64_u32 v[76:77], vcc, v72, %[p5h], v[76:77]\n\t"                                                           \
  "v_mov_b32 v68, v77\n\t"                                                                                           \
  "v_mad_u64_u32 v[78:79], %[junk], v73, %[p5h], v[68:69]\n\t"                                                       \
  "v_addc_co_u32_e32 v79, vcc, 0, v79, vcc\n\t"                                                                      \
  "v_xor_b32_e32 v71, v76, v79\n\t"                                                                                  \
  "v_cmp_ge_u32_e64 %[mask], %[thrh], v71"
#define HG_KS_HASH_TEXT_3(W0, W1, W2, W3)                                                                            \
                                                \
  "v_lshl_add_u64 v[72:73], " W0 ", 0, %[seed]\n\t"                                                                  \
  HG_KS_MUL128("v72", "v73", "%[p3l]", "%[p3h]", "%[seed]", "v[78:79]", "v79")                                       \
  "v_xor_b32_e32 v80, %[kk], v74\n\t"                                                                                \
  "v_mov_b32 v81, v76\n\t"                                                                                           \
                         \
  "v_lshl_add_u64 v[72:73], v[80:81], 0, " W1 "\n\t"                                                                 \
  HG_KS_MUL128("v72", "v73", "%[p2l]", "%[p2h]", "v[80:81]", "v[84:85]", "v85")                                      \
  "v_xor_b32_e32 v82, v78, v74\n\t"                                                                                  \
  "v_xor_b32_e32 v83, v79, v76\n\t"                                                                                  \
                         \
  "v_lshl_add_u64 v[72:73], v[82:83], 0, " W2 "\n\t"                                                                 \
  HG_KS_MUL128("v72", "v73", "%[p1l]", "%[p1h]", "v[82:83]", "v[78:79]", "v79")                                      \
  "v_xor_b32_e32 v80, v84, v74\n\t"                                                                                  \
  "v_xor_b32_e32 v81, v85, v76\n\t"                                                                                  \
  HG_KS_FINAL("v[78:79]", "v78", "v79", "v[80:81]", "v80", "v81")
#define HG_KS_HASH_TEXT_4(W0, W1, W2, W3)                                                                            \
                              \
  "v_lshl_add_u64 v[72:73], " W0 ", 0, %[kk]\n\t"                                                                    \
  HG_KS_MUL128("v72", "v73", "%[p4l]", "%[p4h]", "%[kk]", "v[78:79]", "v79")                                         \
  "v_xor_b32_e32 v80, %[seedl], v74\n\t"                                                                             \
  "v_xor_b32_e32 v81, %[seedh], v76\n\t"                                                                             \
                         \
  "v_lshl_add_u64 v[72:73], v[80:81], 0, " W1 "\n\t"                                                                 \
  HG_KS_MUL128("v72", "v73", "%[p3l]", "%[p3h]", "v[80:81]", "v[84:85]", "v85")                                      \
  "v_xor_b32_e32 v82, v78, v74\n\t"                                                                                  \
  "v_xor_b32_e32 v83, v79, v76\n\t"                                                                                  \
                         \
  "v_lshl_add_u64 v[72:73], v[82:83], 0, " W2 "\n\t"                                                                 \
  HG_KS_MUL128("v72", "v73", "%[p2l]", "%[p2h]", "v[82:83]", "v[78:79]", "v79")                                      \
  "v_xor_b32_e32 v80, v84, v74\n\t"                                                                                  \
  "v_xor_b32_e32 v81, v85, v76\n\t"                                                                                  \
                         \
  "v_lshl_add_u64 v[72:73], v[80:81], 0, " W3 "\n\t"                                                                 \
  HG_KS_MUL128("v72", "v73", "%[p1l]", "%[p1h]", "v[80:81]", "v[84:85]", "v85")                                      \
  "v_xor_b32_e32 v82, v78, v74\n\t"                                                                                  \
  "v_xor_b32_e32 v83, v79, v76\n\t"                                                                                  \
  HG_KS_FINAL("v[84:85]", "v84", "v85", "v[82:83]", "v82", "v83")
#define HG_KS_HASH_INPUTS                                                                                            \
  [seed] "s"(seed), [thrh] "s"((uint32_t)(threshold >> 32)), [kk] "n"(K), [p0l] "s"((uint32_t)P0), [p0h] "s"((uint32_t)(P0 >> 32)),     \
      [p1l] "s"((uint32_t)P1), [p1h] "s"((uint32_t)(P1 >> 32)), [p2l] "s"((uint32_t)P2), [p2h] "s"((uint32_t)(P2 >> 32)), \
      [p3l] "s"((uint32_t)P3), [p3h] "s"((uint32_t)(P3 >> 32)), [p5l] "s"((uint32_t)P5), [p5h] "s"((uint32_t)(P5 >> 32)), \
      [p6l] "s"((uint32_t)P6), [p6h] "s"((uint32_t)(P6 >> 32)), [p4l] "s"((uint32_t)P4), [p4h] "s"((uint32_t)(P4 >> 32)),   \
      [seedl] "s"((uint32_t)seed), [seedh] "s"((uint32_t)(seed >> 32))
#define HG_KS_HASH_CLOBBERS                                                                                          \
  "vcc", "v72", "v73", "v75", "v76", "v77", "v79", "v80", "v81", "v82", "v83", "v84",                 \
      "v85", "v86", "v87", "v88", "v89"

template <int K>
struct GeoS {
  static constexpr int M = 12;
  static constexpr int DW = M / 4;
  static constexpr int WIN = K <= 21 ? 32 : 48;
  static constexpr int LOOK_UNITS = (WIN - M + M - 1) / M;
  static constexpr int TILE = (WG - LOOK_UNITS) * M;
  static constexpr int TILES = 9;
  static constexpr int ITEM = TILE * TILES;
  static constexpr int UNITS = WG;
  static constexpr int NB_T = UNITS * M;
  static constexpr int N_R = NB_T + ((K + 3 - NB_T) & 3);
  static constexpr int S = 4 * (NB_T / 4 + 3);
  static constexpr int ND = (K + 3) / 4, NB = K - 4 * (ND - 1), NW = (K + 7) / 8;
  static_assert(M + K - 1 <= WIN && K <= 32, "a lane's k-mers live in its code window; 2 K bits fit a 64-bit compare");
  static_assert(((N_R - K) & 3) == 3, "reverse phase of start j is 3 - (j & 3)");
  static constexpr int SPAN = NB_T + WIN;
  static constexpr int PAR8 = (TILE % 8) / 4;
  static_assert(TILE % 4 == 0 && ITEM % 4 == 0, "a tile starts at a whole code byte and an aligned ASCII dword");
  static_assert(TILE % 8 == 0 || TILE % 8 == 4, "a tile starts at bit 0 or bit 4 of a bitmap byte");
  static_assert(4 * (DW + 1) <= WIN && (UNITS - 1) * M + WIN <= SPAN, "SPAN covers the last lane's fetches");
  static_assert(SPAN - (UNITS - 1) * M >= WIN && SPAN - (UNITS - 1) * M >= M, "no lane of an interior tile has a base behind the end in its window");
  static_assert(SPAN - K + 1 > (WG - 64) * M, "every wave of an interior tile has k-mer starts");
};
template <int... Ks>
constexpr bool geos_one_geometry_per_class(std::integer_sequence<int, Ks...>) {
  return ((GeoS<Ks + 1>::TILE == GeoS<(Ks + 1 <= 21 ? 21 : 32)>::TILE && GeoS<Ks + 1>::TILES == GeoS<21>::TILES &&
           GeoS<Ks + 1>::SPAN == GeoS<(Ks + 1 <= 21 ? 21 : 32)>::SPAN) && ...);
}
static_assert(geos_one_geometry_per_class(std::make_integer_sequence<int, 32>{}), "TILE, TILES and SPAN depend on K only through WIN");

template <int K, bool CANON, bool PACKED>
__global__ __launch_bounds__(WG) void kmer_sample_shared(
    const uint8_t *__restrict__ seq, const hg_genome_meta *__restrict__ meta,
    const uint32_t *__restrict__ item_genome, uint64_t threshold, uint64_t seed, uint32_t u2t,
    uint64_t *__restrict__ hits, uint32_t *__restrict__ cnt, uint32_t stage_cap, const uint32_t *__restrict__ group_first) {
  using G = GeoS<K>;
  constexpr int M = G::M, DW = G::DW, S = G::S, ND = G::ND, NB = G::NB, NW = G::NW, N_R = G::N_R, WIN = G::WIN;
  typedef typename std::conditional<(WIN > 32), uint64_t, uint32_t>::type inv_t;
  constexpr inv_t MASKK = (inv_t)(((uint64_t)1 << K) - 1);

  const uint32_t tid = threadIdx.x;
  const uint32_t item_lo = group_first ? group_first[blockIdx.x] : blockIdx.x;
  const uint32_t item_hi = group_first ? group_first[blockIdx.x + 1] : blockIdx.x + 1;
  uint32_t g = 0;
  hg_genome_meta gm{};
  uint64_t n_bps = 0, n_starts = 0, item_start = 0;
  const uint8_t *__restrict__ gseq = seq;
  uint32_t tile_no = 0;

  __shared__ HitStage stage;
  __shared__ __attribute__((aligned(16))) uint32_t s_f[4 * S / 4];
  __shared__ __attribute__((aligned(16))) uint32_t s_r[CANON ? 4 * S / 4 : 4];
  __shared__ __attribute__((aligned(16))) uint8_t s_code[(CANON && !PACKED) ? G::NB_T / 4 + 16 : 16];
  __shared__ uint32_t s_val[PACKED ? 4 : G::UNITS + 4];
  __shared__ uint32_t s_dirty[2];
  __shared__ __attribute__((aligned(8))) uint2 s_lut[PACKED ? 256 : 1];
  if (tid == 0) stage.n = 0, s_dirty[0] = 0, s_dirty[1] = 0;
  if constexpr (!PACKED) {
    if (tid < 4) s_val[G::UNITS + tid] = 0;
  } else {
    static_assert(WG == 256, "one table entry per lane");
    uint32_t f = 0, r = 0;
#pragma unroll
    for (int b = 0; b < 4; ++b) {
      const uint32_t cd = (tid >> (2 * b)) & 3u;
      f |= ((0x54474341u >> (8 * cd)) & 0xFFu) << (8 * b);
      r |= ((0x41434754u >> (8 * cd)) & 0xFFu) << (8 * (3 - b));
    }
    s_lut[tid] = make_uint2(f, r);
  }
  __syncthreads();

  using lds_u8p = __attribute__((address_space(3))) const uint8_t *;
  using lds_u16p = __attribute__((address_space(3))) const uint16_t *;
  using lds_u32p = __attribute__((address_space(3))) const uint32_t *;
  const uint32_t aF = (uint32_t)(uintptr_t)(lds_u8p)(reinterpret_cast<const uint8_t *>(s_f)) + M * tid;
  uint32_t aR[M / 4];
#pragma unroll
  for (int gq = 0; gq < M / 4; ++gq)
    aR[gq] = (uint32_t)(uintptr_t)(lds_u8p)(reinterpret_cast<const uint8_t *>(s_r)) + 4u * ((uint32_t)(N_R - K) >> 2) - M * tid - 8u * gq;

  using glb_u8p = __attribute__((address_space(1))) const uint8_t *;
  using glb_u32p = __attribute__((address_space(1))) const uint32_t *;
  using glb_u32up = __attribute__((address_space(1))) const uint32_t __attribute__((aligned(1))) *;
  using glb_u64up = __attribute__((address_space(1))) const uint64_t __attribute__((aligned(1))) *;
  auto tile_base = [](const uint8_t *p) __attribute__((always_inline)) {
    uint64_t a = (uint64_t)(uintptr_t)p;
    asm volatile("" : "+s"(a));
    return (glb_u8p)a;
  };
  uint32_t io_seq = (PACKED ? 3u : (uint32_t)M) * tid;
  uint32_t io_mask = (3u * tid) >> 1;
  auto stage_unit = [&](auto interiorc, uint32_t u, uint64_t tile_start, uint32_t par) __attribute__((always_inline)) {
    constexpr bool INTERIOR = decltype(interiorc)::value;
    const uint64_t P = tile_start + (uint64_t)u * M;
    uint32_t x[DW + 1];
    const int64_t rem64 = INTERIOR ? (int64_t)M : (int64_t)n_bps - (int64_t)P;
    if constexpr (INTERIOR) {
      const glb_u32p src = (glb_u32p)(tile_base(gseq + tile_start) + io_seq);
#pragma unroll
      for (int t = 0; t <= DW; ++t) x[t] = src[t];
    } else if (rem64 + 32 >= 4 * (DW + 1)) {
      const uint32_t *src = reinterpret_cast<const uint32_t *>(gseq + P);
#pragma unroll
      for (int t = 0; t <= DW; ++t) x[t] = src[t];
    } else {
#pragma unroll
      for (int t = 0; t <= DW; ++t) {
        uint32_t w = 0;
        for (int bb = 0; bb < 4; ++bb) {
          const int64_t o = 4 * t + bb;
          w |= (uint32_t)(o < rem64 ? gseq[P + o] : (uint8_t)'N') << (8 * bb);
        }
        x[t] = w;
      }
    }
    if (u2t) {
#pragma unroll
      for (int t = 0; t <= DW; ++t) {
        const uint32_t e = (x[t] & 0xDFDFDFDFu) ^ 0x55555555u;
        const uint32_t nz = ((e & 0x7F7F7F7Fu) + 0x7F7F7F7Fu) | e;
        x[t] ^= (~nz & 0x80808080u) >> 7;
      }
    }
    uint32_t FA[DW + 1], CA[DW + 1];
    uint32_t dacc = 0, codes = 0;
#pragma unroll
    for (int t = 0; t <= DW; ++t) {
      const uint32_t xv = x[t];
      const uint32_t tt = xv ^ (xv >> 1);
      const uint32_t cd = (tt >> 1) & 0x03030303u;
      FA[t] = __builtin_amdgcn_perm(0u, 0x54474341u, cd);
      if (CANON) CA[t] = __builtin_amdgcn_perm(0u, 0x41434754u, cd);
      if (t < DW) {
        dacc |= (xv & 0xDFDFDFDFu) ^ FA[t];
        if (CANON) codes |= __builtin_amdgcn_udot4(cd, 0x40100401u, 0u, false) << (8 * t);
      }
    }
    uint32_t inv = 0;
    const bool dirty = dacc != 0 || rem64 < M;
    if (__any(dirty)) {
#pragma unroll
      for (int t = 0; t < DW; ++t) {
        const uint32_t d = (x[t] & 0xDFDFDFDFu) ^ FA[t];
        const uint32_t z = (((d & 0x7F7F7F7Fu) + 0x7F7F7F7Fu) | d) & 0x80808080u;
        inv |= ((((z >> 7) * 0x01020408u) >> 24) & 0xFu) << (4 * t);
      }
      if (rem64 < M) inv |= rem64 <= 0 ? ~0u : (~0u << (uint32_t)rem64);
      inv &= (1u << M) - 1;
      if ((threadIdx.x & 63) == 0 || dirty) s_dirty[par] = 1u;
    }
    s_val[u] = inv;
    uint32_t *const f0 = s_f + DW * u;
#pragma unroll
    for (int t = 0; t < DW; ++t) {
      f0[t] = FA[t];
      f0[S / 4 + t] = __builtin_amdgcn_alignbyte(FA[t + 1], FA[t], 1);
      f0[2 * (S / 4) + t] = __builtin_amdgcn_alignbyte(FA[t + 1], FA[t], 2);
      f0[3 * (S / 4) + t] = __builtin_amdgcn_alignbyte(FA[t + 1], FA[t], 3);
    }
    if constexpr (CANON) {
#pragma unroll
      for (int t = 0; t < DW; ++t) s_code[DW * u + t] = (uint8_t)(codes >> (8 * t));
#pragma unroll
      for (int ph = 0; ph < 4; ++ph) {
        constexpr int dummy = 0;
        (void)dummy;
        const int psi = (N_R - ph) & 3, JB = (N_R - 4 - psi - ph) / 4;
        const uint32_t sel = (uint32_t)(ph + 3) | ((uint32_t)(ph + 2) << 8) | ((uint32_t)(ph + 1) << 16) | ((uint32_t)ph << 24);
        uint32_t *const r0 = s_r + (3 - psi) * (S / 4) + JB - (int)(DW * u);
#pragma unroll
        for (int t = 0; t < DW; ++t) r0[-t] = __builtin_amdgcn_perm(CA[t + 1], CA[t], sel);
        if (ph > 0 && u == 0) r0[1] = __builtin_amdgcn_perm(CA[0], 0u, sel);
      }
    }
  };

  typedef uint32_t __attribute__((aligned(1))) u32u;
  typedef uint64_t __attribute__((aligned(1))) u64u;
  const uint8_t *__restrict__ gmask = seq;
  auto stage_unit_packed = [&](auto interiorc, uint32_t u, uint64_t tile_start, uint32_t par, uint32_t &c0, uint32_t &c1,
                               uint32_t &c2, inv_t &invw) __attribute__((always_inline)) {
    if constexpr (decltype(interiorc)::value) {
      const glb_u8p cp = tile_base(gseq + (tile_start >> 2)) + io_seq;
      c0 = *(glb_u32up)cp;
      c1 = *(glb_u32up)(cp + 4);
      c2 = WIN > 32 ? *(glb_u32up)(cp + 8) : 0u;
      const uint32_t q = 3u * u + (G::PAR8 ? (uint32_t)(tile_start >> 2) & 1u : 0u);
      const uint64_t mb = *(glb_u64up)(tile_base(gmask + (tile_start >> 3)) + (G::PAR8 ? q >> 1 : io_mask));
      const uint32_t sh = (q & 1u) << 2;
      if constexpr (WIN > 32) invw = (inv_t)(mb >> sh);
      else invw = __builtin_amdgcn_alignbit((uint32_t)(mb >> 32), (uint32_t)mb, sh);
    } else {
    const uint64_t P = tile_start + (uint64_t)u * M;
    const int64_t rem64 = (int64_t)n_bps - (int64_t)P;
    const uint64_t Pc = rem64 > 0 ? P : 0;
    const uint8_t *cp = gseq + (Pc >> 2);
    c0 = *reinterpret_cast<const u32u *>(cp);
    c1 = *reinterpret_cast<const u32u *>(cp + 4);
    c2 = WIN > 32 ? *reinterpret_cast<const u32u *>(cp + 8) : 0u;
    const uint64_t mb = *reinterpret_cast<const u64u *>(gmask + (Pc >> 3));
    invw = (inv_t)(mb >> (uint32_t)(Pc & 7));
    if (rem64 < WIN) invw |= rem64 <= 0 ? ~(inv_t)0 : (inv_t)(~(inv_t)0 << (uint32_t)rem64);
    }
    const bool dirty = invw != 0;
    if (__any(dirty)) {
      if ((threadIdx.x & 63) == 0 || dirty) s_dirty[par] = 1u;
    }
    uint32_t FA[DW + 1], RW[DW + 1];
#pragma unroll
    for (int t = 0; t <= DW; ++t) {
      const uint2 e = s_lut[(c0 >> (8 * t)) & 0xFFu];
      FA[t] = e.x, RW[t] = e.y;
    }
    uint32_t *const f0 = s_f + DW * u;
#pragma unroll
    for (int t = 0; t < DW; ++t) {
      f0[t] = FA[t];
      f0[S / 4 + t] = __builtin_amdgcn_alignbyte(FA[t + 1], FA[t], 1);
      f0[2 * (S / 4) + t] = __builtin_amdgcn_alignbyte(FA[t + 1], FA[t], 2);
      f0[3 * (S / 4) + t] = __builtin_amdgcn_alignbyte(FA[t + 1], FA[t], 3);
    }
    if constexpr (CANON) {
#pragma unroll
      for (int ph = 0; ph < 4; ++ph) {
        const int psi = (N_R - ph) & 3, JB = (N_R - 4 - psi - ph) / 4;
        uint32_t *const r0 = s_r + (3 - psi) * (S / 4) + JB - (int)(DW * u);
#pragma unroll
        for (int t = 0; t < DW; ++t) r0[-t] = ph == 0 ? RW[t] : __builtin_amdgcn_alignbyte(RW[t], RW[t + 1], 4 - ph);
        if (ph > 0 && u == 0) r0[1] = __builtin_amdgcn_alignbyte(0u, RW[0], 4 - ph);
      }
    }
  };

  uint32_t g_next = item_genome[item_lo];
  hg_genome_meta gm_next = meta[g_next];
#pragma unroll 1
  for (uint32_t item = item_lo; item < item_hi; ++item) {
  g = g_next;
  gm = gm_next;
  if (item + 1 < item_hi) {
    g_next = item_genome[item + 1];
    gm_next = meta[g_next];
  }
  n_bps = gm.n_bps;
  if (n_bps < (uint64_t)K) continue;
  n_starts = n_bps - K + 1;
  gseq = seq + gm.seq_off;
  gmask = seq + gm.mask_off;
  item_start = (uint64_t)(item - gm.item_first) * G::ITEM;
  if (item_start >= n_starts) continue;
  const uint64_t item_rem64 = n_bps - item_start;
  const uint32_t item_rem = (item_rem64 >> 32) != 0 ? ~0u : (uint32_t)item_rem64;
#pragma unroll 1
  for (int tile = 0; tile < G::TILES; ++tile, ++tile_no) {
    const uint64_t tile_start = item_start + (uint64_t)tile * G::TILE;
    if ((uint32_t)tile * (uint32_t)G::TILE + (uint32_t)(K - 1) >= item_rem) break;
    const uint32_t par = tile_no & 1u;
    uint32_t pc0 = 0, pc1 = 0, pc2 = 0;
    inv_t pinv = 0;
    asm volatile("" : "+v"(io_seq), "+v"(io_mask));
    const bool interior = (uint32_t)tile * (uint32_t)G::TILE + (uint32_t)G::SPAN <= item_rem;
    bool wave_live = true;
    if (interior) {
      if constexpr (PACKED) stage_unit_packed(std::true_type{}, tid, tile_start, par, pc0, pc1, pc2, pinv);
      else stage_unit(std::true_type{}, tid, tile_start, par);
    } else {
      const uint64_t wave_start = tile_start + (uint64_t)(tid & ~63u) * M;
      if (wave_start < n_starts + (uint64_t)WIN) {
        if constexpr (PACKED) stage_unit_packed(std::false_type{}, tid, tile_start, par, pc0, pc1, pc2, pinv);
        else stage_unit(std::false_type{}, tid, tile_start, par);
      }
      wave_live = wave_start < n_starts;
    }
#ifndef HG_KS_EXP
#define HG_KS_EXP 0
#endif
    if (!(HG_KS_EXP & 1)) __syncthreads();

    const bool tile_dirty = s_dirty[par] != 0u;
    inv_t inv_w = 0;
    if constexpr (PACKED) {
      if (tile_dirty) inv_w = pinv;
    } else if (tile_dirty) {
      if constexpr (WIN > 32)
        inv_w = (inv_t)((uint64_t)s_val[tid] | ((uint64_t)s_val[tid + 1] << M) | ((uint64_t)s_val[tid + 2] << (2 * M)) |
                        ((uint64_t)s_val[tid + 3] << (3 * M)));
      else
        inv_w = (inv_t)(s_val[tid] | (s_val[tid + 1] << M) | (s_val[tid + 2] << (2 * M)));
    }
    uint64_t Gm = 0, Gc = 0;
    uint32_t gf[3] = {0, 0, 0}, wc[3] = {0, 0, 0};
    if constexpr (CANON) {
      uint32_t wl, wh, w2 = 0;
      if constexpr (PACKED) {
        wl = pc0, wh = pc1, w2 = pc2;
      } else {
        const uint32_t bo = (uint32_t)DW * tid;
        const uint32_t *cw = reinterpret_cast<const uint32_t *>(s_code) + (bo >> 2);
        const uint32_t c0 = cw[0], c1 = cw[1], c2 = cw[2], sh = 8u * (bo & 3u);
        wl = __builtin_amdgcn_alignbit(c1, c0, sh), wh = __builtin_amdgcn_alignbit(c2, c1, sh);
        if constexpr (WIN > 32) w2 = __builtin_amdgcn_alignbit(cw[3], c2, sh);
      }
      auto pairrev = [](uint32_t v) {
        const uint32_t br = __builtin_bitreverse32(v);
        return ((br >> 1) & 0x55555555u) | ((br & 0x55555555u) << 1);
      };
      if constexpr (WIN == 32) {
        Gc = ~mk64(wl, wh);
        Gm = mk64(pairrev(wh), pairrev(wl));
      } else {
        wc[0] = ~wl, wc[1] = ~wh, wc[2] = ~w2;
        gf[0] = pairrev(wl), gf[1] = pairrev(wh), gf[2] = pairrev(w2);
      }
    }

    auto strand_base = [&](auto jjc) __attribute__((always_inline)) -> uint32_t {
      constexpr int jj = decltype(jjc)::value;
      uint32_t base = aF;
      if constexpr (CANON && (K & 1) != 0) {
        uint32_t fh, rh;
        if constexpr (WIN == 32) {
          constexpr int SF = 2 * jj, SR = 2 * (32 - K - jj);
          const uint32_t gmh = (uint32_t)(Gm >> 32), gml = (uint32_t)Gm, gch = (uint32_t)(Gc >> 32), gcl = (uint32_t)Gc;
          fh = SF == 0 ? gmh : __builtin_amdgcn_alignbit(gmh, gml, 32 - SF);
          if constexpr (SR == 0) rh = gch;
          else if constexpr (SR < 32) rh = __builtin_amdgcn_alignbit(gch, gcl, 32 - SR);
          else rh = gcl << (SR - 32);
        } else {
          constexpr int o = 2 * jj;
          fh = o == 0 ? gf[0] : __builtin_amdgcn_alignbit(gf[0], gf[1], 32 - o);
          constexpr int e = 2 * jj + 2 * K - 64, off = e + 32, a = off >> 5, sft = off & 31;
          static_assert(off >= 0 && a <= 1, "window inside [0, wc0, wc1, wc2]");
          const uint32_t x_[4] = {0u, wc[0], wc[1], wc[2]};
          rh = sft == 0 ? x_[a + 1] : __builtin_amdgcn_alignbit(x_[a + 2], x_[a + 1], sft);
        }
        uint64_t lt;
        asm("v_cmp_lt_u32_e64 %0, %1, %2" : "=s"(lt) : "v"(rh), "v"(fh));
        asm("v_cndmask_b32_e64 %0, %1, %2, %3" : "=v"(base) : "v"(aF), "v"(aR[jj >> 2]), "s"(lt));
      } else if constexpr (CANON) {
        uint64_t fv, rv;
        if constexpr (WIN == 32) {
          constexpr uint64_t MASK2K = (1ull << (2 * K)) - 1;
          fv = (Gm >> (2 * (32 - K - jj))) & MASK2K;
          rv = (Gc >> (2 * jj)) & MASK2K;
        } else {
          constexpr int o = 2 * jj;
          uint32_t fh, fl;
          if constexpr (o == 0) fh = gf[0], fl = gf[1];
          else fh = __builtin_amdgcn_alignbit(gf[0], gf[1], 32 - o), fl = __builtin_amdgcn_alignbit(gf[1], gf[2], 32 - o);
          constexpr int e = 2 * jj + 2 * K - 64, off = e + 32, a = off >> 5, sft = off & 31;
          static_assert(off >= 0 && a <= 1, "window inside [0, wc0, wc1, wc2]");
          const uint32_t x_[4] = {0u, wc[0], wc[1], wc[2]};
          uint32_t rl, rh;
          if constexpr (sft == 0) rl = x_[a], rh = x_[a + 1];
          else rl = __builtin_amdgcn_alignbit(x_[a + 1], x_[a], sft), rh = __builtin_amdgcn_alignbit(x_[a + 2], x_[a + 1], sft);
          if constexpr (K < 32) {
            constexpr uint32_t LOWCUT = ~((1u << (64 - 2 * K)) - 1u);
            fl &= LOWCUT, rl &= LOWCUT;
          }
          fv = mk64(fl, fh), rv = mk64(rl, rh);
        }
        uint64_t lt;
        asm("v_cmp_lt_u64_e64 %0, %1, %2" : "=s"(lt) : "v"(rv), "v"(fv));
        asm("v_cndmask_b32_e64 %0, %1, %2, %3" : "=v"(base) : "v"(aF), "v"(aR[jj >> 2]), "s"(lt));
      }
      return base;
    };
    auto fetch_words = [&](auto jjc, uint64_t *w) __attribute__((always_inline)) {
      constexpr int jj = decltype(jjc)::value;
      const uint32_t base = strand_base(jjc);
      constexpr int IMM = S * (jj & 3) + 4 * (jj >> 2);
      const lds_u32p src = (lds_u32p)(uintptr_t)(base + (uint32_t)IMM);
      uint32_t d[2 * NW];
#pragma unroll
      for (int m = 0; m < 2 * NW; ++m) {
        if (m < ND - 1 || (m == ND - 1 && NB == 4)) d[m] = src[m];
        else if (m == ND - 1 && NB == 1) d[m] = *(lds_u8p)(uintptr_t)(base + (uint32_t)(IMM + 4 * m));
        else if (m == ND - 1 && NB == 2) d[m] = *(lds_u16p)(uintptr_t)(base + (uint32_t)(IMM + 4 * m));
        else if (m == ND - 1) d[m] = src[m] & 0xFFFFFFu;
        else d[m] = 0;
      }
#pragma unroll
      for (int m = 0; m < NW; ++m) w[m] = mk64(d[2 * m], d[2 * m + 1]);
    };
    uint64_t wq[2][NW];
    const bool hashing = tid < (uint32_t)(WG - G::LOOK_UNITS);
#ifndef HG_KS_ASM
#define HG_KS_ASM 1
#endif
    constexpr bool ASM_BODY = HG_KS_ASM && (NW == 3 || NW == 4);
    uint64_t w0a = 0, w0b = 0, w0c = 0, w0d = 0, w1a = 0, w1b = 0, w1c = 0, w1d = 0;
    uint64_t hmask = 0, hjunk = 0;
    uint32_t hlo0 = 0, hlo1 = 0, hhi = 0;
    uint64_t zpair = 0;
    constexpr int KCASE = 10 * ND + NB;
#define HG_KS_OFFS [o0] "n"(IMM), [o1] "n"(IMM + 8), [o2] "n"(IMM + 16), [o3] "n"(IMM + 20), [o4] "n"(IMM + 24), [o5] "n"(IMM + 28)
#define HG_KS_OUT0 "={v[56:57]}"(w0a), "={v[58:59]}"(w0b), "={v[60:61]}"(w0c), "={v[90:91]}"(w0d)
#define HG_KS_OUT1 "={v[62:63]}"(w1a), "={v[64:65]}"(w1b), "={v[66:67]}"(w1c), "={v[92:93]}"(w1d)
#define HG_KS_IN0 "{v[56:57]}"(w0a), "{v[58:59]}"(w0b), "{v[60:61]}"(w0c), "{v[90:91]}"(w0d)
#define HG_KS_IN1 "{v[62:63]}"(w1a), "{v[64:65]}"(w1b), "{v[66:67]}"(w1c), "{v[92:93]}"(w1d)
#define HG_KS_FIRST(C, N)                                                                                             \
  if constexpr (KCASE == C)                                                                                           \
    asm volatile(HG_KS_APPLY(HG_KS_READ_TEXT_##C, HG_KS_REGS0) : HG_KS_OUT0 : [base] "v"(base), HG_KS_OFFS);
#define HG_KS_EVEN(C, N)                                                                                              \
  if constexpr (KCASE == C)                                                                                           \
    asm volatile(HG_KS_APPLY(HG_KS_WAIT_TEXT_##C, HG_KS_REGS0) HG_KS_APPLY(HG_KS_READ_TEXT_##C, HG_KS_REGS1) "\n\t"   \
                 HG_KS_APPLY(HG_KS_HASH_TEXT_##N, HG_KS_PAIRS0)                                                       \
                 : [mask] "=s"(hmask), [junk] "=&s"(hjunk), "=&{v74}"(hlo0), "=&{v78}"(hlo1), "=&{v71}"(hhi), "={v[68:69]}"(zpair), HG_KS_OUT1     \
                 : HG_KS_HASH_INPUTS, "{v[68:69]}"(zpair), [base] "v"(base), HG_KS_OFFS, HG_KS_IN0                    \
                 : HG_KS_HASH_CLOBBERS);
#define HG_KS_ODD(C, N)                                                                                               \
  if constexpr (KCASE == C)                                                                                           \
    asm volatile(HG_KS_APPLY(HG_KS_WAIT_TEXT_##C, HG_KS_REGS1) HG_KS_APPLY(HG_KS_READ_TEXT_##C, HG_KS_REGS0) "\n\t"   \
                 HG_KS_APPLY(HG_KS_HASH_TEXT_##N, HG_KS_PAIRS1)                                                       \
                 : [mask] "=s"(hmask), [junk] "=&s"(hjunk), "=&{v74}"(hlo0), "=&{v78}"(hlo1), "=&{v71}"(hhi), "={v[68:69]}"(zpair), HG_KS_OUT0     \
                 : HG_KS_HASH_INPUTS, "{v[68:69]}"(zpair), [base] "v"(base), HG_KS_OFFS, HG_KS_IN1                    \
                 : HG_KS_HASH_CLOBBERS);
#define HG_KS_LAST(C, N)                                                                                              \
  if constexpr (KCASE == C)                                                                                           \
    asm volatile(HG_KS_APPLY(HG_KS_WAIT_TEXT_##C, HG_KS_REGS1) HG_KS_APPLY(HG_KS_HASH_TEXT_##N, HG_KS_PAIRS1)         \
                 : [mask] "=s"(hmask), [junk] "=&s"(hjunk), "=&{v74}"(hlo0), "=&{v78}"(hlo1), "=&{v71}"(hhi), "={v[68:69]}"(zpair)                 \
                 : HG_KS_HASH_INPUTS, "{v[68:69]}"(zpair), HG_KS_IN1                                                  \
                 : HG_KS_HASH_CLOBBERS);
#define HG_KS_ALL_CASES(X) X(51, 3) X(52, 3) X(53, 3) X(54, 3) X(61, 3) X(62, 3) X(63, 3) X(64, 3) \
                           X(71, 4) X(72, 4) X(73, 4) X(74, 4) X(81, 4) X(82, 4) X(83, 4) X(84, 4)
    auto kmers_asm = [&](auto checkc) __attribute__((always_inline)) {
      constexpr bool CHECK = decltype(checkc)::value;
      if constexpr (ASM_BODY) {
        {
          const uint32_t base = strand_base(std::integral_constant<int, 0>{});
          constexpr int IMM = 0;
          HG_KS_ALL_CASES(HG_KS_FIRST)
        }
        static_for(std::make_integer_sequence<int, M>{}, [&](auto jc) {
          constexpr int j = decltype(jc)::value;
          const bool valid = !CHECK || ((inv_w >> j) & MASKK) == 0;
          if constexpr (j + 1 < M) {
            const uint32_t base = strand_base(std::integral_constant<int, j + 1>{});
            constexpr int IMM = S * ((j + 1) & 3) + 4 * ((j + 1) >> 2);
            if constexpr ((j & 1) == 0) {
              HG_KS_ALL_CASES(HG_KS_EVEN)
            } else {
              HG_KS_ALL_CASES(HG_KS_ODD)
            }
          } else {
            static_assert((M & 1) == 0, "the last k-mer's words are in the parity-1 buffer");
            HG_KS_ALL_CASES(HG_KS_LAST)
          }
          if (hmask != 0) {
            const uint64_t h = mk64(hlo0 ^ hlo1, hhi);
            if (h < threshold && valid && hashing) stage_hit(stage, stage_cap, h, gm, g, hits, cnt);
          }
        });
      }
    };
#undef HG_KS_FIRST
#undef HG_KS_EVEN
#undef HG_KS_ODD
#undef HG_KS_LAST
    auto run_kmers = [&](auto checkc) __attribute__((always_inline)) {
      constexpr bool CHECK = decltype(checkc)::value;
      static_for(std::make_integer_sequence<int, M>{}, [&](auto jc) {
        constexpr int j = decltype(jc)::value;
        const bool valid = !CHECK || ((inv_w >> j) & MASKK) == 0;
        if constexpr (j == 0) fetch_words(jc, wq[0]);
        if constexpr (j + 1 < M) fetch_words(std::integral_constant<int, j + 1>{}, wq[(j + 1) & 1]);
        const uint64_t h = t1ha2_fixed_w<K>(wq[j & 1], seed);
        if (valid && hashing && h < threshold) stage_hit(stage, stage_cap, h, gm, g, hits, cnt);
      });
    };
    if (wave_live) {
      if constexpr (ASM_BODY) {
        if (!tile_dirty) kmers_asm(std::false_type{});
        else kmers_asm(std::true_type{});
      } else {
        if (!tile_dirty) run_kmers(std::false_type{});
        else run_kmers(std::true_type{});
      }
    }
    if (!(HG_KS_EXP & 1)) __syncthreads();
    if (tid == 0) s_dirty[par] = 0u;
    if (dense_sampling(threshold)) {
      if (HG_KS_EXP & 1) __syncthreads();
      flush_hits_if_filling(stage, stage_cap, gm, g, hits, cnt);
    }
  }
  if (item + 1 < item_hi) flush_hits<true>(stage, stage_cap, gm, g, hits, cnt);
  else flush_hits(stage, stage_cap, gm, g, hits, cnt);
  }
}

__device__ __forceinline__ uint32_t base_code(uint8_t c, uint32_t u2t) {
  uint8_t u = c & 0xDF;
  if (u == 'A') return 0;
  if (u == 'C') return 1;
  if (u == 'G') return 2;
  if (u == 'T') return 3;
  if (u2t && u == 'U') return 3;
  return 4;
}

constexpr uint32_t LONG_TILE = 1536;
constexpr uint32_t LONG_BYTES = 2048;
#ifndef HG_LK_PITCH
#define HG_LK_PITCH 16
#endif
constexpr uint32_t LONG_DW = LONG_BYTES / 4 + HG_LK_PITCH;
static_assert(GEN_ITEM % LONG_TILE == 0 && LONG_TILE % 8 == 0 && LONG_BYTES == 8 * WG && LONG_TILE + 254 <= LONG_BYTES, "long-k tile geometry");

struct LdsStrand {
  const uint32_t *base;
  uint32_t d0, d1;
  bool cached;
  __device__ __forceinline__ uint32_t dword(uint32_t i) const {
    if (cached && __builtin_constant_p(i) && i == 0) return d0;
    if (cached && __builtin_constant_p(i) && i == 1) return d1;
    return base[i];
  }
  __device__ __forceinline__ uint64_t word(uint32_t byte_off, uint32_t nbytes) const {
    uint32_t lo = dword(byte_off / 4), hi = nbytes > 4 ? dword(byte_off / 4 + 1) : 0u;
    if (nbytes < 4) lo &= (1u << (8 * nbytes)) - 1;
    else if (nbytes > 4 && nbytes < 8) hi &= (1u << (8 * (nbytes - 4))) - 1;
    return mk64(lo, hi);
  }
};

__device__ __forceinline__ uint64_t rot64p(uint64_t v, unsigned s) {
  uint64_t r = rot64(v, s);
  asm("" : "+v"(r));
  return r;
}

template <uint32_t LEN>
__device__ __forceinline__ uint64_t t1ha2_long(const LdsStrand &sb, uint32_t len_rt, uint64_t seed) {
  const uint32_t len0 = LEN ? LEN : len_rt;
  uint64_t a = seed, b = (uint64_t)len0;
  uint32_t off = 0, len = len0;
  {
    uint64_t c = rot64((uint64_t)len, 23) + ~seed;
    uint64_t d = ~(uint64_t)len + rot64(seed, 19);
    auto round = [&]() __attribute__((always_inline)) {
      const uint64_t w0 = sb.word(off, 8), w1 = sb.word(off + 8, 8), w2 = sb.word(off + 16, 8), w3 = sb.word(off + 24, 8);
      off += 32;
      const uint64_t d02 = w0 + rot64p(w2 + d, 56);
      const uint64_t c13 = w1 + rot64p(w3 + c, 19);
      d ^= b + rot64p(w1, 38);
      c ^= a + rot64p(w0, 57);
      b ^= lo64mul<P6>(c13 + w2);
      a ^= lo64mul<P5>(d02 + w3);
    };
    if constexpr (LEN != 0) {
      static_assert(LEN > 32 && LEN <= 64, "compile-time lengths: one or two rounds");
      round();
      if constexpr (LEN == 64) round();
    } else {
      do round();
      while (off + 31 < len);
    }
    a ^= lo64mul<P6>(c + rot64p(d, 23));
    b ^= lo64mul<P5>(rot64p(c, 19) + d);
    len &= 31;
  }
  uint32_t rem = len;
  if (rem > 24) { mixup64<P4>(a, b, sb.word(off, 8)); off += 8, rem -= 8; }
  if (rem > 16) { mixup64<P3>(b, a, sb.word(off, 8)); off += 8, rem -= 8; }
  if (rem > 8) { mixup64<P2>(a, b, sb.word(off, 8)); off += 8, rem -= 8; }
  if (rem > 0) mixup64<P1>(b, a, sb.word(off, rem));
  return final64(a, b);
}

__device__ __forceinline__ void long_classify_ascii(uint32_t x, uint32_t u2t, uint32_t &fa, uint32_t &ca, uint32_t &bad) {
  if (u2t) {
    const uint32_t e = (x & 0xDFDFDFDFu) ^ 0x55555555u;
    const uint32_t nz = ((e & 0x7F7F7F7Fu) + 0x7F7F7F7Fu) | e;
    x ^= (~nz & 0x80808080u) >> 7;
  }
  const uint32_t tt = x ^ (x >> 1);
  const uint32_t cd = (tt >> 1) & 0x03030303u;
  const uint32_t f = __builtin_amdgcn_perm(0u, 0x54474341u, cd), c = __builtin_amdgcn_perm(0u, 0x41434754u, cd);
  const uint32_t dif = (x & 0xDFDFDFDFu) ^ f;
  const uint32_t z = (((dif & 0x7F7F7F7Fu) + 0x7F7F7F7Fu) | dif) & 0x80808080u;
  bad = (z >> 7) * 0xFFu;
  fa = f & ~bad, ca = c & ~bad;
}
__device__ __forceinline__ void long_classify_codes(uint32_t codes, uint32_t inv4, uint32_t &fa, uint32_t &ca, uint32_t &bad) {
  const uint32_t cd = (codes & 3u) | ((codes & 0xCu) << 6) | ((codes & 0x30u) << 12) | ((codes & 0xC0u) << 18);
  bad = (((inv4 & 15u) * 0x00204081u) & 0x01010101u) * 0xFFu;
  fa = __builtin_amdgcn_perm(0u, 0x54474341u, cd) & ~bad;
  ca = __builtin_amdgcn_perm(0u, 0x41434754u, cd) & ~bad;
}

template <int KC, bool PACKED>
__global__ __launch_bounds__(WG) void kmer_sample_long(
    const uint8_t *__restrict__ seq, const hg_genome_meta *__restrict__ meta,
    const uint32_t *__restrict__ item_genome, uint32_t ksize_rt, uint64_t threshold, uint64_t seed,
    uint32_t canonical, uint32_t u2t, uint64_t *__restrict__ hits, uint32_t *__restrict__ cnt, uint32_t stage_cap) {
  __shared__ HitStage stage;
  __shared__ uint32_t s_f[4 * LONG_DW], s_rc[4 * LONG_DW];
  __shared__ uint32_t s_inv[LONG_BYTES / 32 + 12];
  __shared__ uint32_t s_anybad[2];
  const uint32_t ksize = KC ? (uint32_t)KC : ksize_rt;
  const uint32_t item = blockIdx.x, tid = threadIdx.x;
  const uint32_t g = item_genome[item];
  const hg_genome_meta gm = meta[g];
  const uint64_t n_bps = gm.n_bps;
  if (n_bps < ksize) return;
  const uint64_t n_starts = n_bps - ksize + 1;
  const uint8_t *__restrict__ gseq = seq + gm.seq_off;
  const uint8_t *__restrict__ gmask = seq + gm.mask_off;
  const uint64_t item_start = (uint64_t)(item - gm.item_first) * GEN_ITEM;
  if (tid == 0) stage.n = 0;
  if (tid < 4) s_f[tid * LONG_DW + LONG_BYTES / 4] = 0u, s_rc[tid * LONG_DW + LONG_BYTES / 4] = 0u;
  if (tid < 12) s_inv[LONG_BYTES / 32 + tid] = 0u;
  if (tid < 2) s_anybad[tid] = 0u;
  typedef uint32_t __attribute__((aligned(1))) u32u_t;
  uint32_t tile_par = 0;

  for (uint64_t tile0 = item_start; tile0 < item_start + GEN_ITEM && tile0 < n_starts; tile0 += LONG_TILE, tile_par ^= 1u) {
    __syncthreads();
    if (tid == 0) s_anybad[tile_par ^ 1u] = 0u;
    if (dense_sampling(threshold)) flush_hits_if_filling(stage, stage_cap, gm, g, hits, cnt);
    {
      const uint64_t pos0 = tile0 + (uint64_t)tid * 8;
      uint32_t fa[4], ca[4], bad[4];
#pragma unroll
      for (int t = 0; t < 4; ++t) {
        const int64_t q = (int64_t)pos0 + 4 * t - 4;
        fa[t] = ca[t] = 0u, bad[t] = ~0u;
        if (q >= 0 && (uint64_t)q < n_bps) {
          if constexpr (PACKED) {
            const uint32_t codes = gseq[(uint64_t)q >> 2];
            const uint32_t inv4 = (uint32_t)gmask[(uint64_t)q >> 3] >> ((uint32_t)q & 4u);
            long_classify_codes(codes, inv4, fa[t], ca[t], bad[t]);
          } else {
            long_classify_ascii(*reinterpret_cast<const u32u_t *>(gseq + q), u2t, fa[t], ca[t], bad[t]);
          }
          const uint64_t left = n_bps - (uint64_t)q;
          if (left < 4) {
            const uint32_t keep = (1u << (8 * (uint32_t)left)) - 1u;
            fa[t] &= keep, ca[t] &= keep, bad[t] |= ~keep;
          }
        }
      }
#pragma unroll
      for (uint32_t ph = 0; ph < 4; ++ph) {
        s_f[ph * LONG_DW + 2 * tid] = ph ? __builtin_amdgcn_alignbyte(fa[2], fa[1], ph) : fa[1];
        s_f[ph * LONG_DW + 2 * tid + 1] = ph ? __builtin_amdgcn_alignbyte(fa[3], fa[2], ph) : fa[2];
      }
      const uint32_t r0 = __builtin_bswap32(ca[0]), r1 = __builtin_bswap32(ca[1]), r2 = __builtin_bswap32(ca[2]);
      const uint32_t j1 = LONG_BYTES / 4 - 1 - 2 * tid;
#pragma unroll
      for (uint32_t ph = 0; ph < 4; ++ph) {
        s_rc[ph * LONG_DW + j1] = ph ? __builtin_amdgcn_alignbyte(r0, r1, ph) : r1;
        s_rc[ph * LONG_DW + j1 - 1] = ph ? __builtin_amdgcn_alignbyte(r1, r2, ph) : r2;
      }
      const uint32_t b8 = ((((bad[1] & 0x01010101u) * 0x01020408u) >> 24) & 15u) | (((((bad[2] & 0x01010101u) * 0x01020408u) >> 24) & 15u) << 4);
      reinterpret_cast<uint8_t *>(s_inv)[tid] = (uint8_t)b8;
      if (b8 != 0u) s_anybad[tile_par] = 1u;
    }
    __syncthreads();
#ifndef HG_LK_DIRTY
#define HG_LK_DIRTY 1
#endif
    const bool tile_dirty = !HG_LK_DIRTY || s_anybad[tile_par] != 0u;
    const uint64_t left_starts = n_starts - tile0;
    const uint32_t lim = left_starts < LONG_TILE ? (uint32_t)left_starts : LONG_TILE;
    const uint32_t jn = lim > tid ? (lim - tid + WG - 1) / WG : 0u;
    const uint32_t rb0 = LONG_BYTES - ksize - tid;
    const uint32_t *fp = s_f + (tid & 3u) * LONG_DW + (tid >> 2);
    const uint32_t *rp = s_rc + (rb0 & 3u) * LONG_DW + (rb0 >> 2);
#ifndef HG_LK_UNROLL
#define HG_LK_UNROLL 1
#endif
#pragma unroll HG_LK_UNROLL
    for (uint32_t j = 0; j < jn; ++j, fp += WG / 4, rp -= WG / 4) {
      if (tile_dirty) {
        const uint32_t p = tid + WG * j, dw = p >> 5, sh = p & 31u;
        bool any_bad;
        if constexpr (KC != 0) {
          const uint32_t d0 = s_inv[dw], d1 = s_inv[dw + 1], d2 = s_inv[dw + 2];
          const uint32_t w0 = __builtin_amdgcn_alignbit(d1, d0, sh), w1 = __builtin_amdgcn_alignbit(d2, d1, sh);
          constexpr uint32_t M1 = KC >= 64 ? ~0u : (1u << (KC - 32)) - 1u;
          any_bad = (w0 | (w1 & M1)) != 0u;
        } else {
          uint32_t acc = 0;
          for (uint32_t t = 0; 32 * t < ksize; ++t) {
            const uint32_t w = __builtin_amdgcn_alignbit(s_inv[dw + t + 1], s_inv[dw + t], sh);
            const uint32_t left = ksize - 32 * t;
            acc |= left >= 32 ? w : w & ((1u << left) - 1u);
          }
          any_bad = acc != 0u;
        }
        if (any_bad) continue;
      }
      const uint32_t fd0 = fp[0], fd1 = fp[1];
      uint32_t rd0 = 0, rd1 = 0;
      bool use_rc = false;
      if (canonical) {
        rd0 = rp[0], rd1 = rp[1];
        const uint64_t fw = mk64(__builtin_bswap32(fd1), __builtin_bswap32(fd0));
        const uint64_t rw = mk64(__builtin_bswap32(rd1), __builtin_bswap32(rd0));
        if (fw != rw) {
          use_rc = rw < fw;
        } else {
          for (uint32_t t = 2; 4 * t < ksize; ++t) {
            uint32_t fd = __builtin_bswap32(fp[t]), rd = __builtin_bswap32(rp[t]);
            const uint32_t left = ksize - 4 * t;
            if (left < 4) fd &= ~0u << (8 * (4 - left)), rd &= ~0u << (8 * (4 - left));
            if (fd != rd) {
              use_rc = rd < fd;
              break;
            }
          }
        }
      }
#ifndef HG_LK_CACHE
#define HG_LK_CACHE 1
#endif
      const LdsStrand sel{use_rc ? rp : fp, use_rc ? rd0 : fd0, use_rc ? rd1 : fd1, HG_LK_CACHE != 0};
      const uint64_t h = t1ha2_long<(uint32_t)KC>(sel, ksize, seed);
      if (h < threshold) stage_hit(stage, stage_cap, h, gm, g, hits, cnt);
    }
  }
  flush_hits(stage, stage_cap, gm, g, hits, cnt);
}

}

const char *hg_kmer_kernel_name(uint32_t k, bool canonical, bool packed) {
  static thread_local char buf[64];
  if (k > 32) {
    snprintf(buf, sizeof buf, "kmer_sample_long<%u, %s>", k <= 64 ? k : 0u, packed ? "true" : "false");
    return buf;
  }
  snprintf(buf, sizeof buf, "kmer_sample_shared<%u, %s, %s>", k, canonical ? "true" : "false", packed ? "true" : "false");
  return buf;
}

uint32_t hg_kmer_item_starts(uint32_t k) {
  if (k > 32) return GEN_ITEM;
  return k >= 22 ? (uint32_t)GeoS<32>::ITEM : (uint32_t)GeoS<21>::ITEM;
}

uint32_t hg_kmer_tile_starts(uint32_t k) {
  if (k > 32) return 0;
  return k >= 22 ? (uint32_t)GeoS<32>::TILE : (uint32_t)GeoS<21>::TILE;
}
uint32_t hg_kmer_item_tiles(uint32_t k) { return k > 32 ? 0u : 3u * (uint32_t)GeoS<21>::TILES; }

hipError_t hg_launch_kmer_sample(hipStream_t st, const uint8_t *d_seq, const hg_genome_meta *d_meta,
                                 const uint32_t *d_item_genome, uint32_t n_items, uint32_t ksize,
                                 uint64_t threshold, uint64_t seed, bool canonical, uint32_t norm_mode,
                                 uint64_t *d_hits, uint32_t *d_cnt, bool packed, const uint32_t *d_group_first,
                                 uint32_t n_groups) {
  if (n_items == 0) return hipSuccess;
  if (ksize > 32 || n_groups == 0) d_group_first = nullptr;
  const uint32_t n_wg = d_group_first ? n_groups : n_items;
  const uint32_t u2t = (norm_mode == HG_NORM_U2T && !packed) ? 1u : 0u;
  auto stage_entries = [&](uint32_t tile_starts) {
    const double per_tile = (double)tile_starts * ((double)threshold / 18446744073709551616.0);
    uint32_t cap = HIT_STAGE;
    while (cap < HIT_STAGE_MAX && (double)cap < 2.0 * per_tile + 128.0) cap <<= 1;
    return cap;
  };
  const uint32_t cap_s = stage_entries((uint32_t)GeoS<21>::TILE), cap_l = stage_entries(LONG_TILE);
#define HG_K_LAUNCH(KK, CN, PK)                                                                            \
  hipLaunchKernelGGL((kmer_sample_shared<KK, CN, PK>), dim3(n_wg), dim3(WG), cap_s * sizeof(uint64_t), st, d_seq, d_meta, \
                     d_item_genome, threshold, seed, u2t, d_hits, d_cnt, cap_s, d_group_first)
#define HG_K_CASE(KK)                                                                                     \
  case KK:                                                                                                \
    if (canonical && packed) HG_K_LAUNCH(KK, true, true);                                                 \
    else if (canonical) HG_K_LAUNCH(KK, true, false);                                                     \
    else if (packed) HG_K_LAUNCH(KK, false, true);                                                        \
    else HG_K_LAUNCH(KK, false, false);                                                                   \
    return hipGetLastError();
  switch (ksize) {
    HG_K_CASE(1) HG_K_CASE(2) HG_K_CASE(3) HG_K_CASE(4) HG_K_CASE(5) HG_K_CASE(6) HG_K_CASE(7) HG_K_CASE(8)
    HG_K_CASE(9) HG_K_CASE(10) HG_K_CASE(11) HG_K_CASE(12) HG_K_CASE(13) HG_K_CASE(14) HG_K_CASE(15) HG_K_CASE(16)
    HG_K_CASE(17) HG_K_CASE(18) HG_K_CASE(19) HG_K_CASE(20) HG_K_CASE(21) HG_K_CASE(22) HG_K_CASE(23) HG_K_CASE(24)
    HG_K_CASE(25) HG_K_CASE(26) HG_K_CASE(27) HG_K_CASE(28) HG_K_CASE(29) HG_K_CASE(30) HG_K_CASE(31) HG_K_CASE(32)
    default:
      break;
  }
#undef HG_K_CASE
#undef HG_K_LAUNCH
#define HG_KL_LAUNCH(PK, KK)                                                                                                   \
  hipLaunchKernelGGL((kmer_sample_long<KK, PK>), dim3(n_items), dim3(WG), cap_l * sizeof(uint64_t), st, d_seq, d_meta, d_item_genome, \
                     ksize, threshold, seed, canonical ? 1u : 0u, u2t, d_hits, d_cnt, cap_l)
#define HG_KL_CASE(KK)                        \
  case KK:                                    \
    if (packed) HG_KL_LAUNCH(true, KK);       \
    else HG_KL_LAUNCH(false, KK);             \
    return hipGetLastError();
  switch (ksize) {
    HG_KL_CASE(33) HG_KL_CASE(34) HG_KL_CASE(35) HG_KL_CASE(36) HG_KL_CASE(37) HG_KL_CASE(38) HG_KL_CASE(39) HG_KL_CASE(40)
    HG_KL_CASE(41) HG_KL_CASE(42) HG_KL_CASE(43) HG_KL_CASE(44) HG_KL_CASE(45) HG_KL_CASE(46) HG_KL_CASE(47) HG_KL_CASE(48)
    HG_KL_CASE(49) HG_KL_CASE(50) HG_KL_CASE(51) HG_KL_CASE(52) HG_KL_CASE(53) HG_KL_CASE(54) HG_KL_CASE(55) HG_KL_CASE(56)
    HG_KL_CASE(57) HG_KL_CASE(58) HG_KL_CASE(59) HG_KL_CASE(60) HG_KL_CASE(61) HG_KL_CASE(62) HG_KL_CASE(63) HG_KL_CASE(64)
    default:
      break;
  }
#undef HG_KL_CASE
  if (packed) HG_KL_LAUNCH(true, 0);
  else HG_KL_LAUNCH(false, 0);
#undef HG_KL_LAUNCH
  return hipGetLastError();
}
```

hyper-gen_amd/csrc/hg_sketch.h:

```cpp
#pragma once
#include <utility>

#include "hg_internal.h"

struct hg_batch_tables {
  std::vector<hg_genome_meta> meta;
  std::vector<uint32_t> item_genome;
  std::vector<uint32_t> group_first;
  size_t n_groups = 0;
  uint64_t total_slots = 0;
  uint32_t max_cap = 0, max_expect = 0;
  size_t n_items = 0;
  bool reused = false;
  uint32_t max_hits = ~0u;
  std::vector<std::pair<uint32_t, uint32_t>> big;
};

hg_status hg_check_sketch_params(hg_ctx *c, const hg_sketch_params *p);
inline size_t hg_plan_group_offset(size_t n_items) { return (n_items + 3) & ~(size_t)3; }
inline const uint32_t *hg_plan_group_table(const hg_ctx *c, size_t n_items, size_t n_groups) {
  return n_groups ? static_cast<const uint32_t *>(c->w_items.p) + hg_plan_group_offset(n_items) : nullptr;
}

hg_status hg_plan_build(hg_ctx *c, const hg_genome_batch &b, uint32_t ksize, uint64_t scaled,
                        const std::vector<uint32_t> *want_caps, hg_batch_tables &t);
hg_status hg_plan_get(hg_ctx *c, const hg_genome_batch &b, uint32_t ksize, uint64_t scaled, hg_batch_tables &t, bool with_meta = true);
void hg_plan_tables_from_cache(const hg_sketch_plan &pl, size_t n, hg_batch_tables &t, bool with_meta = true);
hg_status hg_plan_commit(hg_ctx *c, const hg_batch_tables &t, const hg_genome_batch &b, uint32_t ksize, uint64_t scaled);

hg_status hg_pack_batch(hg_ctx *c, const uint8_t *d_seq, const uint64_t *seq_offs, const uint64_t *lens, size_t n,
                        uint32_t norm_mode, uint8_t *d_blobs, const uint64_t *blob_offs);

struct hg_sample_fetch {
  size_t max_hashes = 0;
  const uint64_t *h_hashes = nullptr;
  uint32_t nd = 0;
  bool valid = false;
};

hg_status hg_sketch_front(hg_ctx *c, const hg_genome_batch &b, const hg_sketch_params *p, uint64_t threshold,
                          const hg_batch_tables &t, bool sync_free, uint32_t *sort_cap);

hg_status hg_sample_batch_sync(hg_ctx *c, const hg_genome_batch &b, const hg_sketch_params *p, uint64_t threshold,
                               hg_batch_tables &t, bool planned, uint32_t **d_ndistinct_out, hg_sample_fetch *fetch);
hg_status hg_sketch_batch_sync(hg_ctx *c, const hg_genome_batch &b, const hg_sketch_params *p, const hg_sketch_out &out,
                               hg_batch_tables *planned = nullptr);

hg_status hg_sketch_step(hg_ctx *c, const hg_genome_batch &b, const hg_sketch_params *p, const hg_sketch_out &out);
```

hyper-gen_amd/csrc/hg_sketch_plan.hip:

```cpp
#include <algorithm>
#include <cstring>

#include "hg_sketch.h"

static uint32_t round_cap(uint64_t cap) {
  if (cap > HG_SORT_LDS_MAX_KEYS) {
    uint64_t p = 1;
    while (p < cap) p <<= 1;
    cap = p;
  }
  return cap > 0xFFFFFFF0ull ? 0xFFFFFFF0u : (uint32_t)cap;
}

hg_status hg_check_sketch_params(hg_ctx *c, const hg_sketch_params *p) {
  if (!p) return hg_fail(c, HG_ERR_INVALID, "params == NULL");
  if (p->ksize < 1) return hg_fail(c, HG_ERR_INVALID, "ksize must be >= 1");
  if (p->ksize > 255) return hg_fail(c, HG_ERR_UNSUPPORTED, "ksize must be <= 255 (the reference's -k is u8)");
  if (p->scaled < 1) return hg_fail(c, HG_ERR_INVALID, "scaled must be >= 1");
  if (p->hv_layout > HG_LAYOUT_AVX2 || p->norm_mode > HG_NORM_U2T) return hg_fail(c, HG_ERR_INVALID, "bad layout / norm mode");
  if (p->hv_d == 0 || p->hv_d > 32768) return hg_fail(c, HG_ERR_UNSUPPORTED, "hv_d must be in 1..32768");
  return HG_OK;
}

hg_status hg_plan_build(hg_ctx *c, const hg_genome_batch &b, uint32_t ksize, uint64_t scaled,
                        const std::vector<uint32_t> *want_caps, hg_batch_tables &t) {
  const uint64_t item_starts = hg_kmer_item_starts(ksize);
  const uint32_t tile_starts = hg_kmer_tile_starts(ksize), item_tiles = hg_kmer_item_tiles(ksize);
  const uint32_t full_item_tiles = tile_starts ? (uint32_t)((item_starts + tile_starts - 1) / tile_starts) : 0;
  bool group_open = false;
  t.group_first.clear();
  uint32_t group_tiles = 0;
  t.meta.resize(b.n);
  t.item_genome.clear();
  t.reused = false;
  uint64_t slot = 0, max_expect = 0;
  uint32_t max_cap = 0;
  for (size_t g = 0; g < b.n; ++g) {
    if (b.offsets[g] & 3) return hg_fail(c, HG_ERR_INVALID, "genome offsets must be multiples of 4");
    hg_genome_meta &m = t.meta[g];
    m.seq_off = b.offsets[g];
    m.n_bps = b.lens[g];
    m.mask_off = b.mask_offs ? b.mask_offs[g] : m.seq_off + hg_pack2_code_bytes(m.n_bps);
    const uint64_t n_starts = m.n_bps >= ksize ? m.n_bps - ksize + 1 : 0;
    const uint64_t expect = n_starts / scaled;
    uint64_t cap = expect * 2 + 1024;
    if (cap > n_starts) cap = n_starts;
    if (want_caps && (*want_caps)[g] > cap) cap = (*want_caps)[g];
    if (cap == 0) cap = 1;
    m.hit_cap = round_cap(cap);
    m.hit_off = slot;
    slot += m.hit_cap;
    max_cap = std::max(max_cap, m.hit_cap);
    max_expect = std::max(max_expect, std::min(expect, n_starts));
    const uint64_t n_items = (n_starts + item_starts - 1) / item_starts;
    if (t.item_genome.size() + n_items > 0x7FFFFFFFull)
      return hg_fail(c, HG_ERR_UNSUPPORTED, "batch too large for one launch; split it");
    m.item_first = (uint32_t)t.item_genome.size();
    if (tile_starts) {
      for (uint64_t it = 0; it < n_items; ++it) {
        const uint64_t starts = std::min<uint64_t>(item_starts, n_starts - it * item_starts);
        const uint32_t tiles = (uint32_t)((starts + tile_starts - 1) / tile_starts);
        const bool alone = tiles >= full_item_tiles;
        if (!group_open || alone || group_tiles + tiles > item_tiles) {
          t.group_first.push_back((uint32_t)(t.item_genome.size() + it));
          group_tiles = 0;
        }
        group_tiles += tiles;
        group_open = !alone;
      }
    }
    t.item_genome.insert(t.item_genome.end(), (size_t)n_items, (uint32_t)g);
  }
  t.n_groups = t.group_first.size();
  if (t.n_groups) t.group_first.push_back((uint32_t)t.item_genome.size());
  t.total_slots = slot;
  t.max_cap = max_cap;
  t.max_expect = (uint32_t)std::min<uint64_t>(max_expect, 0xFFFFFFF0ull);
  t.n_items = t.item_genome.size();
  return HG_OK;
}

hg_status hg_plan_get(hg_ctx *c, const hg_genome_batch &b, uint32_t ksize, uint64_t scaled, hg_batch_tables &t, bool with_meta) {
  const hg_sketch_plan *pl = c->plan.get();
  const bool match = pl && pl->ksize == ksize && pl->scaled == scaled && pl->packed == b.packed && pl->offs.size() == b.n &&
                     std::memcmp(pl->offs.data(), b.offsets, b.n * 8) == 0 && std::memcmp(pl->lens.data(), b.lens, b.n * 8) == 0 &&
                     (b.mask_offs ? pl->masks.size() == b.n && std::memcmp(pl->masks.data(), b.mask_offs, b.n * 8) == 0 : pl->masks.empty());
  if (!match) return hg_plan_build(c, b, ksize, scaled, nullptr, t);
  hg_plan_tables_from_cache(*pl, b.n, t, with_meta);
  return HG_OK;
}

void hg_plan_tables_from_cache(const hg_sketch_plan &pl, size_t n, hg_batch_tables &t, bool with_meta) {
  t.total_slots = pl.total_slots, t.max_cap = pl.max_cap, t.max_expect = pl.max_expect, t.n_items = pl.n_items;
  t.n_groups = pl.n_groups, t.reused = true;
  t.item_genome.clear();
  t.group_first.clear();
  if (!with_meta) {
    t.meta.clear();
    return;
  }
  t.meta.resize(n);
  uint64_t slot = 0;
  for (size_t g = 0; g < n; ++g) {
    t.meta[g].hit_cap = pl.caps[g];
    t.meta[g].hit_off = slot;
    slot += pl.caps[g];
  }
}

hg_status hg_plan_commit(hg_ctx *c, const hg_batch_tables &t, const hg_genome_batch &b, uint32_t ksize, uint64_t scaled) {
  if (t.reused) return HG_OK;
  const size_t n = b.n;
  c->plan.reset();
  hg_status s;
  const size_t n_items = t.item_genome.size();
  if ((s = hg_ensure(c, c->w_gmeta, n * sizeof(hg_genome_meta) + 16)) != HG_OK) return s;
  const size_t items_words = t.n_groups ? hg_plan_group_offset(n_items) + t.n_groups + 1 : n_items;
  if ((s = hg_ensure(c, c->w_items, items_words * sizeof(uint32_t) + 16)) != HG_OK) return s;
  const size_t pin_meta = (n * sizeof(hg_genome_meta) + 63) & ~(size_t)63;
  const size_t need = pin_meta + items_words * sizeof(uint32_t) + 64;
  if (c->plan_upload_pending) {
    HG_HIP(c, hipEventSynchronize(c->plan_uploaded));
    c->plan_upload_pending = false;
  }
  if (need > c->h_plan_cap) {
    if (c->h_plan) (void)hipHostFree(c->h_plan);
    c->h_plan = nullptr, c->h_plan_cap = 0;
    const size_t want = need + need / 4 + 4096;
    hipError_t e = hipHostMalloc(&c->h_plan, want, hipHostMallocDefault);
    if (e != hipSuccess) return hg_fail(c, HG_ERR_OOM, std::string("hipHostMalloc: ") + hipGetErrorString(e));
    c->h_plan_cap = want;
  }
  if (!c->plan_uploaded) HG_HIP(c, hipEventCreateWithFlags(&c->plan_uploaded, hipEventDisableTiming));
  auto *pin = static_cast<uint8_t *>(c->h_plan);
  std::memcpy(pin, t.meta.data(), n * sizeof(hg_genome_meta));
  HG_HIP(c, hipMemcpyAsync(c->w_gmeta.p, pin, n * sizeof(hg_genome_meta), hipMemcpyHostToDevice, c->stream));
  if (n_items) {
    std::memcpy(pin + pin_meta, t.item_genome.data(), n_items * sizeof(uint32_t));
    if (t.n_groups) {
      std::memset(pin + pin_meta + n_items * sizeof(uint32_t), 0, (hg_plan_group_offset(n_items) - n_items) * sizeof(uint32_t));
      std::memcpy(pin + pin_meta + hg_plan_group_offset(n_items) * sizeof(uint32_t), t.group_first.data(), (t.n_groups + 1) * sizeof(uint32_t));
    }
    HG_HIP(c, hipMemcpyAsync(c->w_items.p, pin + pin_meta, items_words * sizeof(uint32_t), hipMemcpyHostToDevice, c->stream));
  }
  HG_HIP(c, hipEventRecord(c->plan_uploaded, c->stream));
  c->plan_upload_pending = true;
  auto pl = std::make_shared<hg_sketch_plan>();
  pl->offs.assign(b.offsets, b.offsets + n);
  pl->lens.assign(b.lens, b.lens + n);
  if (b.mask_offs) pl->masks.assign(b.mask_offs, b.mask_offs + n);
  pl->caps.resize(n);
  for (size_t g = 0; g < n; ++g) pl->caps[g] = t.meta[g].hit_cap;
  pl->ksize = ksize, pl->scaled = scaled, pl->packed = b.packed;
  pl->total_slots = t.total_slots, pl->max_cap = t.max_cap, pl->max_expect = t.max_expect, pl->n_items = n_items;
  pl->n_groups = t.n_groups;
  c->plan = std::move(pl);
  return HG_OK;
}

hg_status hg_pack_batch(hg_ctx *c, const uint8_t *d_seq, const uint64_t *seq_offs, const uint64_t *lens, size_t n,
                        uint32_t norm_mode, uint8_t *d_blobs, const uint64_t *blob_offs) {
  if (n == 0) return HG_OK;
  hg_status s;
  if ((s = hg_ensure(c, c->w_pktab, 3 * n * sizeof(uint64_t) + 64)) != HG_OK) return s;
  if ((s = hg_ensure_pinned(c, 3 * n * sizeof(uint64_t) + 64)) != HG_OK) return s;
  HG_HIP(c, hipStreamSynchronize(c->stream));
  auto *tab = static_cast<uint64_t *>(c->h_pin);
  uint64_t max_len = 0;
  for (size_t g = 0; g < n; ++g) {
    if ((seq_offs[g] & 3) || (blob_offs[g] & 15)) return hg_fail(c, HG_ERR_INVALID, "pack2: sequence offsets must be multiples of 4, blob offsets of 16");
    tab[3 * g] = seq_offs[g], tab[3 * g + 1] = lens[g], tab[3 * g + 2] = blob_offs[g];
    max_len = std::max(max_len, lens[g]);
  }
  HG_HIP(c, hipMemcpyAsync(c->w_pktab.p, tab, 3 * n * sizeof(uint64_t), hipMemcpyHostToDevice, c->stream));
  const uint64_t groups = (hg_pack2_mask_bytes(max_len) + 3) / 4;
  const uint64_t blocks = (groups + 255) / 256;
  if (blocks > 0x7FFFFFFFull) return hg_fail(c, HG_ERR_UNSUPPORTED, "pack2: genome too long for one launch");
  if (blocks)
    HG_HIP(c, hg_launch_pack2(c->stream, d_seq, static_cast<const uint64_t *>(c->w_pktab.p), (uint32_t)n, (uint32_t)blocks,
                              norm_mode == HG_NORM_U2T ? 1u : 0u, d_blobs));
  HG_HIP(c, hipStreamSynchronize(c->stream));
  return HG_OK;
}

extern "C" hg_status hg_sketch_plan_describe(const uint64_t *offsets, const uint64_t *lens, size_t n, uint32_t ksize, uint64_t scaled,
                                             uint64_t counts[6], uint32_t *group_first, size_t cap) {
  if ((n && (!offsets || !lens)) || !counts || ksize < 1 || ksize > 255 || scaled < 1) return HG_ERR_INVALID;
  hg_batch_tables t;
  const hg_status s = hg_plan_build(nullptr, {nullptr, offsets, lens, nullptr, n, false}, ksize, scaled, nullptr, t);
  if (s != HG_OK) return s;
  const uint32_t tile = hg_kmer_tile_starts(ksize);
  counts[0] = t.n_items, counts[1] = t.n_groups ? t.n_groups : t.n_items, counts[2] = t.total_slots, counts[3] = t.max_cap;
  counts[4] = t.max_expect, counts[5] = tile ? (hg_kmer_item_starts(ksize) + tile - 1) / tile : 0;
  if (group_first) {
    if (t.group_first.size() > cap) return HG_ERR_CAPACITY;
    for (size_t i = 0; i < t.group_first.size(); ++i) group_first[i] = t.group_first[i];
  }
  return HG_OK;
}
```

hyper-gen_amd/csrc/hg_sketch_step.hip:

```cpp
#include <algorithm>
#include <atomic>
#include <chrono>
#include <cstring>
#include <thread>

#include <unistd.h>

#include "hg_sketch.h"

namespace {

uint32_t first_sort_cap(const hg_ctx *c, const hg_batch_tables &t, bool sync_free) {
  const uint64_t seen = t.reused ? c->plan->max_hits : 0;
  if (!sync_free)
    return seen ? (uint32_t)std::min<uint64_t>(t.max_cap, seen + seen / 8 + 16) : t.max_cap;
  const uint64_t base = seen ? seen : t.max_expect;
  const uint64_t margin = base + base / 8 + 24 <= 64 ? 24 : 64;
  return (uint32_t)std::min<uint64_t>(t.max_cap, base + base / 8 + margin);
}

bool step_can_be_sync_free(const hg_ctx *c, const hg_batch_tables &t, size_t n) {
  if (c->dbg_sketch_path == "sync" || c->dbg_sort_buckets) return false;
  if (n == 0 || n > 0x7FFFFFFFull) return false;
  return (uint64_t)t.max_expect + t.max_expect / 8 + 64 <= HG_SORT_LDS_MAX_KEYS;
}

hg_status wait_check_word(hg_ctx *c, int slot, uint32_t seq, uint32_t *flags) {
  volatile uint32_t *w = c->h_chk + 16 * slot;
  const auto t0 = std::chrono::steady_clock::now();
  for (uint32_t spins = 0;; ++spins) {
    if (w[1] == seq) break;
    if (spins < 4096) {
#if defined(__x86_64__) || defined(__i386__)
      __builtin_ia32_pause();
#else
      std::this_thread::yield();
#endif
      continue;
    }
    ::usleep(50);
    if ((spins & 0x3ff) == 0 && std::chrono::steady_clock::now() - t0 > std::chrono::seconds(2)) {
      const hipError_t e = hipStreamSynchronize(c->stream);
      if (e != hipSuccess) return hg_fail(c, HG_ERR_HIP, std::string("hipStreamSynchronize: ") + hipGetErrorString(e));
      if (w[1] != seq) return hg_fail(c, HG_ERR_HIP, "sketch step: the stream finished without publishing its check word");
      break;
    }
  }
  std::atomic_thread_fence(std::memory_order_acquire);
  *flags = w[0];
  return HG_OK;
}

hg_status redo_step(hg_ctx *c, const hg_sketch_pending &pd) {
  ++c->n_redone_steps;
  return hg_sketch_batch_sync(c, pd.batch, &pd.p, pd.out);
}

}

hg_status hg_sketch_front(hg_ctx *c, const hg_genome_batch &b, const hg_sketch_params *p, uint64_t threshold,
                          const hg_batch_tables &t, bool sync_free, uint32_t *sort_cap) {
  const size_t n = b.n;
  hg_status s;
  if ((s = hg_ensure(c, c->w_hits, t.total_slots * sizeof(uint64_t) + 16)) != HG_OK) return s;
  if ((s = hg_ensure(c, c->w_cnt, (2 * n + 16) * sizeof(uint32_t) + 16)) != HG_OK) return s;
  auto *d_meta = static_cast<hg_genome_meta *>(c->w_gmeta.p);
  auto *d_hits = static_cast<uint64_t *>(c->w_hits.p);
  auto *d_cnt = static_cast<uint32_t *>(c->w_cnt.p);
  uint32_t *d_nd = d_cnt + n, *d_flags = sync_free ? d_cnt + 2 * n : nullptr;
  HG_HIP(c, hipMemsetAsync(d_cnt, 0, (2 * n + (sync_free ? 16 : 0)) * sizeof(uint32_t), c->stream));
  {
    hg_timed tm(c, HG_T_KMER);
    c->last_kernel[HG_T_KMER] = hg_kmer_kernel_name(p->ksize, p->canonical != 0, b.packed);
    HG_HIP(c, hg_launch_kmer_sample(c->stream, b.d_seq, d_meta, static_cast<const uint32_t *>(c->w_items.p), (uint32_t)t.n_items,
                                    p->ksize, threshold, p->seed, p->canonical != 0, p->norm_mode, d_hits, d_cnt, b.packed,
                                    hg_plan_group_table(c, t.n_items, t.n_groups), (uint32_t)t.n_groups));
  }
  *sort_cap = first_sort_cap(c, t, sync_free);
  hg_timed tm(c, HG_T_SORT, HG_T_KMER);
  std::string *names = &c->last_kernel[HG_T_SORT];
  names->clear();
  HG_HIP(c, hg_launch_sort_unique(c->stream, d_meta, (uint32_t)n, d_hits, d_cnt, d_nd, *sort_cap, threshold, p->min_count, d_flags, names));
  if (sync_free)
    HG_HIP(c, hg_launch_sort_unique_rest(c->stream, d_meta, (uint32_t)n, d_hits, d_cnt, d_nd, *sort_cap, t.max_cap, threshold, p->min_count, names));
  return HG_OK;
}

hg_status hg_sketch_resolve(hg_ctx *c, bool *redone) {
  if (redone) *redone = false;
  if (!c->pending.active) return HG_OK;
  const hg_sketch_pending pd = std::move(c->pending);
  c->pending = hg_sketch_pending{};
  uint32_t flags = 0;
  hg_status s = wait_check_word(c, pd.slot, pd.seq, &flags);
  if (s != HG_OK || !flags) return s;
  if (redone) *redone = true;
  return redo_step(c, pd);
}

hg_status hg_sketch_step(hg_ctx *c, const hg_genome_batch &b, const hg_sketch_params *p, const hg_sketch_out &out) {
  const size_t n = b.n;
  hg_status s;
  hg_batch_tables t;
  if ((s = hg_plan_get(c, b, p->ksize, p->scaled, t, false)) != HG_OK) return s;
  if (!step_can_be_sync_free(c, t, n)) {
    bool redone = false;
    if ((s = hg_sketch_resolve(c, &redone)) != HG_OK) return s;
    if (!redone && t.reused) hg_plan_tables_from_cache(*c->plan, n, t);
    return hg_sketch_batch_sync(c, b, p, out, redone ? nullptr : &t);
  }
  if (!c->h_chk) {
    void *q = nullptr;
    const hipError_t e = hipHostMalloc(&q, 32 * sizeof(uint32_t), hipHostMallocCoherent);
    if (e != hipSuccess) return hg_fail(c, HG_ERR_OOM, std::string("hipHostMalloc: ") + hipGetErrorString(e));
    c->h_chk = static_cast<uint32_t *>(q);
    std::memset(c->h_chk, 0, 32 * sizeof(uint32_t));
  }
  if ((s = hg_plan_commit(c, t, b, p->ksize, p->scaled)) != HG_OK) return s;
  const uint64_t threshold = UINT64_MAX / p->scaled;
  uint32_t sort_cap = 0;
  if ((s = hg_sketch_front(c, b, p, threshold, t, true, &sort_cap)) != HG_OK) return s;
  const int slot = c->pending.active ? 1 - c->pending.slot : 0;
  const uint32_t seq = c->chk_seq + 1 ? c->chk_seq + 1 : 1;
  {
    auto *d_cnt = static_cast<uint32_t *>(c->w_cnt.p);
    uint32_t *d_nd = d_cnt + n, *d_flags = d_cnt + 2 * n;
    hg_timed tm(c, HG_T_ENCODE, HG_T_SORT);
    std::string *names = &c->last_kernel[HG_T_ENCODE];
    names->clear();
    HG_HIP(c, hg_launch_encode(c->stream, static_cast<hg_genome_meta *>(c->w_gmeta.p), (uint32_t)n, static_cast<uint64_t *>(c->w_hits.p),
                               d_nd, p->hv_d, p->hv_layout, out.d_hv, out.d_norm2, nullptr,
                               std::min<uint32_t>(t.max_cap, HG_SORT_LDS_MAX_KEYS), names));
    HG_HIP(c, hg_launch_sketch_finish(c->stream, d_nd, out.d_nhash, (uint32_t)n, d_flags, c->h_chk + 16 * slot, seq, names));
  }
  c->chk_seq = seq;
  ++c->n_fast_steps;

  const hg_sketch_plan &pl = *c->plan;
  hg_sketch_pending cur{true, seq, slot, c->plan,
                        {b.d_seq, pl.offs.data(), pl.lens.data(), pl.masks.empty() ? nullptr : pl.masks.data(), b.n, b.packed}, *p, out};
  bool redone = false;
  if ((s = hg_sketch_resolve(c, &redone)) != HG_OK) return s;
  if (redone) {
    return redo_step(c, cur);
  }
  c->pending = std::move(cur);
  return HG_OK;
}
```

include/hypergen.h:

```cpp
#ifndef HYPERGEN_H
#define HYPERGEN_H

#include <stddef.h>
#include <stdint.h>

#ifdef __cplusplus
extern "C" {
#endif

typedef struct hg_ctx hg_ctx;

typedef enum {
  HG_OK = 0,
  HG_ERR_INVALID = 1,
  HG_ERR_NO_DEVICE = 2,
  HG_ERR_HIP = 3,
  HG_ERR_OOM = 4,
  HG_ERR_CAPACITY = 5,
  HG_ERR_UNSUPPORTED = 6,
  HG_ERR_IO = 7,
  HG_ERR_INEXACT = 8
} hg_status;

const char *hg_status_str(hg_status s);
const char *hg_last_error(const hg_ctx *ctx);
const char *hg_version(void);

hg_status hg_ctx_create(int device_id, hg_ctx **out);
void hg_ctx_destroy(hg_ctx *ctx);
hg_status hg_ctx_set_stream(hg_ctx *ctx, void *hip_stream);
hg_status hg_ctx_reset_stream(hg_ctx *ctx);
hg_status hg_ctx_sync(hg_ctx *ctx);
hg_status hg_ctx_sketch_step_counts(hg_ctx *ctx, uint64_t *sync_free, uint64_t *synchronous, uint64_t *redone);
int hg_device_count(void);
hg_status hg_ctx_set_debug(hg_ctx *ctx, const char *key, const char *value);

#define HG_T_KMER 0
#define HG_T_SORT 1
#define HG_T_ENCODE 2
#define HG_T_DIST_PREP 3
#define HG_T_DIST 4
#define HG_T_COUNT 5
hg_status hg_ctx_enable_timing(hg_ctx *ctx, int on);
hg_status hg_ctx_timings(hg_ctx *ctx, float ms_sum[HG_T_COUNT], uint32_t launches[HG_T_COUNT]);
const char *hg_ctx_last_kernel(const hg_ctx *ctx, int cls);

hg_status hg_dev_alloc(hg_ctx *ctx, size_t bytes, void **dptr);
hg_status hg_dev_free(hg_ctx *ctx, void *dptr);
hg_status hg_copy_h2d(hg_ctx *ctx, void *dst_dev, const void *src_host, size_t bytes);
hg_status hg_copy_d2h(hg_ctx *ctx, void *dst_host, const void *src_dev, size_t bytes);

#define HG_LAYOUT_SCALAR 0u
#define HG_LAYOUT_AVX2 1u
#define HG_NORM_ACGT 0u
#define HG_NORM_U2T 1u

typedef struct {
  uint32_t ksize;
  uint32_t canonical;
  uint64_t scaled;
  uint64_t seed;
  uint32_t hv_d;
  uint32_t hv_layout;
  uint32_t norm_mode;
  uint32_t min_count;
} hg_sketch_params;


void hg_sketch_params_default(hg_sketch_params *p);

hg_status hg_kmer_hash_sample(hg_ctx *ctx, const uint8_t *seq, size_t n_bps,
                              uint32_t ksize, uint64_t threshold, uint64_t seed,
                              int canonical, uint32_t norm_mode, uint64_t *out_hashes,
                              size_t cap, size_t *n_out);
hg_status hg_kmer_hash_sample_min_count(hg_ctx *ctx, const uint8_t *seq, size_t n_bps,
                                        uint32_t ksize, uint64_t threshold, uint64_t seed,
                                        int canonical, uint32_t norm_mode, uint32_t min_count,
                                        uint64_t *out_hashes, size_t cap, size_t *n_out);

hg_status hg_hv_encode(hg_ctx *ctx, const uint64_t *hashes, size_t n, uint32_t hv_d,
                       uint32_t hv_layout, int16_t *hv_out, int32_t *norm2_out);

hg_status hg_sketch_batch_dev(hg_ctx *ctx, const uint8_t *d_seq, const uint64_t *offsets,
                              const uint64_t *lens, size_t n, const hg_sketch_params *p,
                              int16_t *d_hv, int32_t *d_norm2, uint32_t *d_nhash);
#define HG_NHASH_PENDING 0xFFFFFFFFu
hg_status hg_sketch_plan_describe(const uint64_t *offsets, const uint64_t *lens, size_t n, uint32_t ksize, uint64_t scaled,
                                  uint64_t counts[6], uint32_t *group_first, size_t cap);
hg_status hg_sketch_batch_dev_packed(hg_ctx *ctx, const uint8_t *d_blobs, const uint64_t *offsets,
                                     const uint64_t *n_bps, size_t n, const hg_sketch_params *p,
                                     int16_t *d_hv, int32_t *d_norm2, uint32_t *d_nhash);
hg_status hg_sketch_batch(hg_ctx *ctx, const uint8_t *const *seqs, const size_t *lens,
                          size_t n, const hg_sketch_params *p, int16_t *hv_out,
                          int32_t *norm2_out, uint32_t *nhash_out);

hg_status hg_dist_full(hg_ctx *ctx, const int16_t *ref_hv, const int32_t *ref_norm2,
                       size_t R, const int16_t *qry_hv, const int32_t *qry_norm2, size_t Q,
                       uint32_t hv_d, uint32_t ksize, float *ani_out);
hg_status hg_dist_full_dev(hg_ctx *ctx, const int16_t *d_ref_hv, const int32_t *d_ref_norm2,
                           size_t R, const int16_t *d_qry_hv, const int32_t *d_qry_norm2,
                           size_t Q, uint32_t hv_d, uint32_t ksize, float *d_ani_out);
hg_status hg_logf_dev(hg_ctx *ctx, const float *d_x, uint32_t first_bits, size_t n, float *d_out);
hg_status hg_ani_from_dots_dev(hg_ctx *ctx, const int32_t *d_dot, const int32_t *d_norm2_r, const int32_t *d_norm2_q,
                               size_t n, uint32_t ksize, float *d_ani);

#define HG_ANI_MASH 0
#define HG_ANI_CONTAINMENT 1
#define HG_ANI_MAX_CONTAINMENT 2
hg_status hg_ctx_set_ani_metric(hg_ctx *ctx, int metric);
int hg_ctx_ani_metric(const hg_ctx *ctx);

typedef struct {
  uint32_t ref_idx;
  uint32_t qry_idx;
  float ani;
} hg_ani_hit;

hg_status hg_dist(hg_ctx *ctx, const int16_t *ref_hv, const int32_t *ref_norm2, size_t R,
                  const int16_t *qry_hv, const int32_t *qry_norm2, size_t Q, uint32_t hv_d,
                  uint32_t ksize, int symmetric, float ani_th, hg_ani_hit *out, size_t cap,
                  size_t *n_out);
hg_status hg_dist_dev(hg_ctx *ctx, const int16_t *d_ref_hv, const int32_t *d_ref_norm2,
                      size_t R, const int16_t *d_qry_hv, const int32_t *d_qry_norm2, size_t Q,
                      uint32_t hv_d, uint32_t ksize, int symmetric, float ani_th,
                      hg_ani_hit *d_out, size_t cap, size_t *n_out);

hg_status hg_dist_block_dev(hg_ctx *ctx, const int16_t *d_ref_hv, const int32_t *d_ref_norm2, size_t R,
                            size_t ref_off, const int16_t *d_qry_hv, const int32_t *d_qry_norm2, size_t Q,
                            size_t qry_off, uint32_t hv_d, uint32_t ksize, int symmetric, float ani_th,
                            hg_ani_hit *d_out, size_t cap, size_t *n_out);

size_t hg_dist_ops_row_bytes(uint32_t hv_d);
size_t hg_dist_ops_meta_bytes(void);
size_t hg_dist_ops_padded_rows(size_t rows);
hg_status hg_dist_prep_ops_dev(hg_ctx *ctx, const int16_t *d_hv, size_t rows, uint32_t hv_d, uint8_t *d_ops,
                               uint8_t *d_meta, uint32_t *d_flag);
hg_status hg_dist_block_ops_dev(hg_ctx *ctx, const uint8_t *d_ref_ops, const uint8_t *d_ref_meta, const int32_t *d_ref_norm2,
                                size_t R, size_t ref_off, const uint32_t *d_ref_index, const uint32_t *d_flags,
                                size_t n_flags, const int16_t *d_qry_hv, const int32_t *d_qry_norm2, size_t Q,
                                size_t qry_off, uint32_t hv_d, uint32_t ksize, int symmetric, float ani_th,
                                hg_ani_hit *d_out, size_t cap, size_t *n_out);

int hg_ctx_last_dist_path(const hg_ctx *ctx);

void hg_sort_ani_hits(hg_ani_hit *hits, size_t n, size_t Q, int symmetric);

hg_status hg_sort_ani_hits_dev(hg_ctx *ctx, hg_ani_hit *d_hits, size_t n, size_t Q);
hg_status hg_sort_ani_hits_staged(hg_ctx *ctx, hg_ani_hit *hits, size_t n, size_t Q);

hg_status hg_topk_per_query_dev(hg_ctx *ctx, const hg_ani_hit *d_hits, size_t n, size_t Q, uint32_t k,
                                hg_ani_hit *d_out, uint32_t *d_counts);

#define HG_PAIRS_MASH 1u
#define HG_PAIRS_CONTAINMENT 2u
#define HG_PAIRS_MAX_CONTAINMENT 4u
#define HG_PAIRS_CONTAINMENT_REF 8u
#define HG_PAIRS_EMPTY 0xFFFFFFFFu
hg_status hg_ani_pairs_dev(hg_ctx *ctx, const int16_t *d_ref_hv, const int32_t *d_ref_norm2, size_t R,
                           const int16_t *d_qry_hv, const int32_t *d_qry_norm2, size_t Q, uint32_t hv_d, uint32_t ksize,
                           const hg_ani_hit *d_pairs, size_t n_pairs, uint32_t columns, float *d_ani, int32_t *d_dot);
hg_status hg_ani_pairs(hg_ctx *ctx, const int16_t *ref_hv, const int32_t *ref_norm2, size_t R, const int16_t *qry_hv,
                       const int32_t *qry_norm2, size_t Q, uint32_t hv_d, uint32_t ksize, const hg_ani_hit *pairs,
                       size_t n_pairs, uint32_t columns, float *ani, int32_t *dot);

#define HG_SEARCH_TOPK_MAX 64u
#define HG_SEARCH_BLOCK_BYTES ((size_t)256 << 20)
hg_status hg_search_topk_dev(hg_ctx *ctx, const int16_t *d_ref_hv, const int32_t *d_ref_norm2, size_t R,
                             const int16_t *d_qry_hv, const int32_t *d_qry_norm2, size_t Q, uint32_t hv_d, uint32_t ksize,
                             float ani_th, uint32_t k, hg_ani_hit *d_out, uint32_t *d_counts);
hg_status hg_search_topk_block_dev(hg_ctx *ctx, const int16_t *d_ref_hv, const int32_t *d_ref_norm2, size_t R, size_t ref_off,
                                   const int16_t *d_qry_hv, const int32_t *d_qry_norm2, size_t Q, size_t qry_off,
                                   uint32_t hv_d, uint32_t ksize, float ani_th, uint32_t k, hg_ani_hit *d_out,
                                   uint32_t *d_counts);
hg_status hg_search_topk(hg_ctx *ctx, const int16_t *ref_hv, const int32_t *ref_norm2, size_t R, const int16_t *qry_hv,
                         const int32_t *qry_norm2, size_t Q, uint32_t hv_d, uint32_t ksize, float ani_th, uint32_t k,
                         hg_ani_hit *out, uint32_t *counts);
hg_status hg_search_topk_merge(const hg_ani_hit *const *lists, const uint32_t *const *counts, size_t n_lists, size_t Q,
                               uint32_t k, hg_ani_hit *out, uint32_t *counts_out);

hg_status hg_cluster_init_dev(hg_ctx *ctx, uint32_t *d_rep, size_t n);
hg_status hg_cluster_add_hits_dev(hg_ctx *ctx, uint32_t *d_rep, size_t n, const hg_ani_hit *d_hits, size_t n_hits,
                                  float ani_th);
hg_status hg_cluster_finish_dev(hg_ctx *ctx, uint32_t *d_rep, size_t n, uint32_t *d_cluster, size_t *n_clusters);
hg_status hg_cluster_dev(hg_ctx *ctx, const int16_t *d_hv, const int32_t *d_norm2, size_t n, uint32_t hv_d, uint32_t ksize,
                         float ani_th, uint32_t *d_rep, uint32_t *d_cluster, size_t *n_clusters);
hg_status hg_cluster(hg_ctx *ctx, const int16_t *hv, const int32_t *norm2, size_t n, uint32_t hv_d, uint32_t ksize,
                     float ani_th, uint32_t *rep, uint32_t *cluster, size_t *n_clusters);

hg_status hg_cluster_greedy_hits_dev(hg_ctx *ctx, size_t n, const hg_ani_hit *d_hits, size_t n_hits, float ani_th,
                                     uint32_t *d_rep, uint32_t *d_cluster, float *d_ani, size_t *n_clusters);
hg_status hg_cluster_greedy_dev(hg_ctx *ctx, const int16_t *d_hv, const int32_t *d_norm2, size_t n, uint32_t hv_d,
                                uint32_t ksize, float ani_th, uint32_t *d_rep, uint32_t *d_cluster, float *d_ani,
                                size_t *n_clusters);
hg_status hg_cluster_greedy(hg_ctx *ctx, const int16_t *hv, const int32_t *norm2, size_t n, uint32_t hv_d, uint32_t ksize,
                            float ani_th, uint32_t *rep, uint32_t *cluster, float *ani, size_t *n_clusters);
uint64_t hg_ctx_cluster_greedy_rounds(const hg_ctx *ctx);

hg_status hg_cluster_setcover_hits_dev(hg_ctx *ctx, size_t n, const hg_ani_hit *d_hits, size_t n_hits, float ani_th,
                                       uint32_t *d_rep, uint32_t *d_cluster, float *d_ani, size_t *n_clusters);
hg_status hg_cluster_setcover_dev(hg_ctx *ctx, const int16_t *d_hv, const int32_t *d_norm2, size_t n, uint32_t hv_d,
                                  uint32_t ksize, float ani_th, uint32_t *d_rep, uint32_t *d_cluster, float *d_ani,
                                  size_t *n_clusters);
hg_status hg_cluster_setcover(hg_ctx *ctx, const int16_t *hv, const int32_t *norm2, size_t n, uint32_t hv_d, uint32_t ksize,
                              float ani_th, uint32_t *rep, uint32_t *cluster, float *ani, size_t *n_clusters);
uint64_t hg_ctx_cluster_setcover_rounds(const hg_ctx *ctx);

hg_status hg_cluster_tree_hits_dev(hg_ctx *ctx, size_t n, const hg_ani_hit *d_hits, size_t n_hits, float ani_th,
                                   hg_ani_hit *d_tree, size_t tree_cap, size_t *n_edges, uint32_t *d_rep, uint32_t *d_cluster,
                                   size_t *n_clusters);
hg_status hg_cluster_tree_dev(hg_ctx *ctx, const int16_t *d_hv, const int32_t *d_norm2, size_t n, uint32_t hv_d, uint32_t ksize,
                              float ani_th, hg_ani_hit *d_tree, size_t tree_cap, size_t *n_edges, uint32_t *d_rep,
                              uint32_t *d_cluster, size_t *n_clusters);
hg_status hg_cluster_tree(hg_ctx *ctx, const int16_t *hv, const int32_t *norm2, size_t n, uint32_t hv_d, uint32_t ksize,
                          float ani_th, hg_ani_hit *tree, size_t tree_cap, size_t *n_edges, uint32_t *rep, uint32_t *cluster,
                          size_t *n_clusters);
uint64_t hg_ctx_cluster_tree_rounds(const hg_ctx *ctx);

#define HG_CLUSTER_AVERAGE_MAX_N 65536u
hg_status hg_cluster_average_matrix_dev(hg_ctx *ctx, const float *d_ani, size_t n, float ani_th, uint32_t *d_rep,
                                        uint32_t *d_cluster, uint32_t *d_into, float *d_level, uint32_t *d_size, size_t *n_clusters);
hg_status hg_cluster_average_dev(hg_ctx *ctx, const int16_t *d_hv, const int32_t *d_norm2, size_t n, uint32_t hv_d, uint32_t ksize,
                                 float ani_th, uint32_t *d_rep, uint32_t *d_cluster, uint32_t *d_into, float *d_level,
                                 uint32_t *d_size, size_t *n_clusters);
hg_status hg_cluster_average(hg_ctx *ctx, const int16_t *hv, const int32_t *norm2, size_t n, uint32_t hv_d, uint32_t ksize,
                             float ani_th, uint32_t *rep, uint32_t *cluster, uint32_t *into, float *level, uint32_t *size,
                             size_t *n_clusters);
uint64_t hg_ctx_cluster_average_rounds(const hg_ctx *ctx);

#define HG_STATS_NONE 0xFFFFFFFFu
typedef struct {
  uint64_t within_sum;
  uint32_t within_min, within_min_idx;
  uint32_t outside_max, outside_max_idx;
} hg_node_stat;
typedef struct {
  uint64_t within_sum;
  uint32_t size, first, medoid;
  uint32_t within_min, within_min_a, within_min_b;
  uint32_t outside_max, outside_member, outside_idx;
  uint32_t reserved;
} hg_cluster_stat;
// ... 143 lines not shown
```

Measured before the change: 126,500.

## Replace static item grouping with persistent workgroups pulling items via atomic tickets

The kmer sampling kernel now launches a persistent grid sized from occupancy (workgroups per CU times CU count), and each workgroup claims items dynamically from a global atomic ticket counter, prefetching the next item's metadata during the first tile. This replaces the host-built static group_first table that packed short items into groups. The aim is better load balance across variable-length genomes and less host planning and upload work, at the cost of per-item atomics, an extra barrier and an occupancy query cached per configuration.

```diff
diff --git a/hyper-gen_amd/__init__.py b/hyper-gen_amd/__init__.py
--- a/hyper-gen_amd/__init__.py
+++ b/hyper-gen_amd/__init__.py
@@ -52,7 +52,7 @@
 
 EXPORTS = [
     "hg_status_str", "hg_last_error", "hg_version", "hg_ctx_create", "hg_ctx_destroy",
-    "hg_ctx_set_stream", "hg_ctx_reset_stream", "hg_ctx_sync", "hg_ctx_sketch_step_counts", "hg_sketch_plan_describe", "hg_logf_dev", "hg_ani_from_dots_dev", "hg_device_count", "hg_dev_alloc", "hg_dev_free",
+    "hg_ctx_set_stream", "hg_ctx_reset_stream", "hg_ctx_sync", "hg_ctx_sketch_step_counts", "hg_sketch_plan_describe", "hg_ctx_kmer_grid", "hg_kmer_geometry", "hg_logf_dev", "hg_ani_from_dots_dev", "hg_device_count", "hg_dev_alloc", "hg_dev_free",
     "hg_copy_h2d", "hg_copy_d2h", "hg_sketch_params_default", "hg_kmer_hash_sample",
     "hg_kmer_hash_sample_min_count",
     "hg_hv_encode", "hg_sketch_batch_dev", "hg_sketch_batch", "hg_dist_full", "hg_dist_full_dev",
@@ -154,6 +154,8 @@
         "hg_ctx_reset_stream": (C.c_int, [vp]),
         "hg_ctx_sync": (C.c_int, [vp]),
         "hg_sketch_plan_describe": (C.c_int, [vp, vp, sz, C.c_uint32, C.c_uint64, C.POINTER(C.c_uint64), vp, sz]),
+        "hg_ctx_kmer_grid": (C.c_int, [vp, C.POINTER(C.c_uint32)]),
+        "hg_kmer_geometry": (C.c_int, [C.c_uint32, C.POINTER(C.c_uint32)]),
         "hg_logf_dev": (C.c_int, [vp, vp, C.c_uint32, sz, vp]),
         "hg_ani_from_dots_dev": (C.c_int, [vp, vp, vp, vp, sz, C.c_uint32, vp]),
         "hg_ctx_sketch_step_counts": (C.c_int, [vp, C.POINTER(C.c_uint64), C.POINTER(C.c_uint64), C.POINTER(C.c_uint64)]),
@@ -395,6 +397,11 @@
         self._ck(lib().hg_ctx_sketch_step_counts(self._h, C.byref(a), C.byref(b), C.byref(c)))
         return int(a.value), int(b.value), int(c.value)
 
+    def kmer_grid(self):
+        n = C.c_uint32()
+        self._ck(lib().hg_ctx_kmer_grid(self._h, C.byref(n)))
+        return int(n.value)
+
     def last_kernel(self, cls):
         return lib().hg_ctx_last_kernel(self._h, T_NAMES.index(cls)).decode()
 
@@ -1171,6 +1178,14 @@
         self.close()
 
 
+def kmer_geometry(ksize):
+    out = (C.c_uint32 * 4)()
+    st = lib().hg_kmer_geometry(ksize, out)
+    if st != OK:
+        raise HgError(st, "hg_kmer_geometry")
+    return dict(zip(("tile", "item_tiles", "item", "span"), (int(x) for x in out)))
+
+
 def sketch_plan_describe(offsets, lens, ksize=21, scaled=1500):
     off = np.ascontiguousarray(offsets, np.uint64)
     ln = np.ascontiguousarray(lens, np.uint64)
diff --git a/hyper-gen_amd/csrc/hg_api.hip b/hyper-gen_amd/csrc/hg_api.hip
--- a/hyper-gen_amd/csrc/hg_api.hip
+++ b/hyper-gen_amd/csrc/hg_api.hip
@@ -171,6 +171,18 @@
   return HG_OK;
 }
 
+extern "C" hg_status hg_ctx_kmer_grid(hg_ctx *c, uint32_t *workgroups) {
+  if (!c || !workgroups) return HG_ERR_INVALID;
+  *workgroups = c->kmer_grid;
+  return HG_OK;
+}
+
+extern "C" hg_status hg_kmer_geometry(uint32_t ksize, uint32_t out[4]) {
+  if (!out || ksize < 1 || ksize > 255) return HG_ERR_INVALID;
+  out[0] = hg_kmer_tile_starts(ksize), out[1] = hg_kmer_item_tiles(ksize), out[2] = hg_kmer_item_starts(ksize), out[3] = hg_kmer_tile_span(ksize);
+  return HG_OK;
+}
+
 static hipEvent_t take_event(hg_ctx *c) {
   if (!c->t_pool.empty()) {
     hipEvent_t e = c->t_pool.back();
diff --git a/hyper-gen_amd/csrc/hg_internal.h b/hyper-gen_amd/csrc/hg_internal.h
--- a/hyper-gen_amd/csrc/hg_internal.h
+++ b/hyper-gen_amd/csrc/hg_internal.h
@@ -22,7 +22,9 @@
   uint32_t max_expect = 0;
   uint32_t max_hits = 0;
   size_t n_items = 0;
-  size_t n_groups = 0;
+};
+struct hg_kmer_residency {
+  uint16_t wg_per_cu[33][2][2][5] = {};
 };
 struct hg_genome_batch {
   const uint8_t *d_seq = nullptr;
@@ -130,6 +132,8 @@
   std::vector<TimedLaunch> t_pending;
   std::vector<hipEvent_t> t_pool;
   std::shared_ptr<hg_sketch_plan> plan;
+  hg_kmer_residency kmer_res;
+  uint32_t kmer_grid = 0;
   hipEvent_t plan_uploaded = nullptr;
   bool plan_upload_pending = false;
   void *h_plan = nullptr;
@@ -213,10 +217,11 @@
 hipError_t hg_launch_kmer_sample(hipStream_t st, const uint8_t *d_seq, const hg_genome_meta *d_meta,
                                  const uint32_t *d_item_genome, uint32_t n_items, uint32_t ksize,
                                  uint64_t threshold, uint64_t seed, bool canonical, uint32_t norm_mode,
-                                 uint64_t *d_hits, uint32_t *d_cnt, bool packed = false, const uint32_t *d_group_first = nullptr,
-                                 uint32_t n_groups = 0);
+                                 uint64_t *d_hits, uint32_t *d_cnt, bool packed, uint32_t *d_ticket, hg_kmer_residency *res,
+                                 uint32_t n_cu, uint32_t *grid_out = nullptr);
 uint32_t hg_kmer_tile_starts(uint32_t ksize);
 uint32_t hg_kmer_item_tiles(uint32_t ksize);
+uint32_t hg_kmer_tile_span(uint32_t ksize);
 hipError_t hg_launch_pack2(hipStream_t st, const uint8_t *d_seq, const uint64_t *d_tab, uint32_t n, uint32_t blocks_max,
                            uint32_t u2t, uint8_t *d_blobs);
 hipError_t hg_launch_unpack2_jobs(hipStream_t st, const uint8_t *d_pk, uint8_t *d_out, const UnpackJob *d_jobs, uint32_t n_jobs, uint32_t n_blocks);
diff --git a/hyper-gen_amd/csrc/hg_kmer_kernels.hip b/hyper-gen_amd/csrc/hg_kmer_kernels.hip
--- a/hyper-gen_amd/csrc/hg_kmer_kernels.hip
+++ b/hyper-gen_amd/csrc/hg_kmer_kernels.hip
@@ -327,15 +327,13 @@
 __global__ __launch_bounds__(WG) void kmer_sample_shared(
     const uint8_t *__restrict__ seq, const hg_genome_meta *__restrict__ meta,
     const uint32_t *__restrict__ item_genome, uint64_t threshold, uint64_t seed, uint32_t u2t,
-    uint64_t *__restrict__ hits, uint32_t *__restrict__ cnt, uint32_t stage_cap, const uint32_t *__restrict__ group_first) {
+    uint64_t *__restrict__ hits, uint32_t *__restrict__ cnt, uint32_t stage_cap, uint32_t *__restrict__ ticket, uint32_t n_items) {
   using G = GeoS<K>;
   constexpr int M = G::M, DW = G::DW, S = G::S, ND = G::ND, NB = G::NB, NW = G::NW, N_R = G::N_R, WIN = G::WIN;
   typedef typename std::conditional<(WIN > 32), uint64_t, uint32_t>::type inv_t;
   constexpr inv_t MASKK = (inv_t)(((uint64_t)1 << K) - 1);
 
   const uint32_t tid = threadIdx.x;
-  const uint32_t item_lo = group_first ? group_first[blockIdx.x] : blockIdx.x;
-  const uint32_t item_hi = group_first ? group_first[blockIdx.x + 1] : blockIdx.x + 1;
   uint32_t g = 0;
   hg_genome_meta gm{};
   uint64_t n_bps = 0, n_starts = 0, item_start = 0;
@@ -348,8 +346,9 @@
   __shared__ __attribute__((aligned(16))) uint8_t s_code[(CANON && !PACKED) ? G::NB_T / 4 + 16 : 16];
   __shared__ uint32_t s_val[PACKED ? 4 : G::UNITS + 4];
   __shared__ uint32_t s_dirty[2];
+  __shared__ uint32_t s_ticket[2];
   __shared__ __attribute__((aligned(8))) uint2 s_lut[PACKED ? 256 : 1];
-  if (tid == 0) stage.n = 0, s_dirty[0] = 0, s_dirty[1] = 0;
+  if (tid == 0) stage.n = 0, s_dirty[0] = 0, s_dirty[1] = 0, s_ticket[1] = atomicAdd(ticket, 1u);
   if constexpr (!PACKED) {
     if (tid < 4) s_val[G::UNITS + tid] = 0;
   } else {
@@ -527,24 +526,24 @@
     }
   };
 
-  uint32_t g_next = item_genome[item_lo];
+  uint32_t item = __builtin_amdgcn_readfirstlane(s_ticket[1]);
+  if (item >= n_items) return;
+  uint32_t g_next = item_genome[item];
   hg_genome_meta gm_next = meta[g_next];
 #pragma unroll 1
-  for (uint32_t item = item_lo; item < item_hi; ++item) {
+  for (;;) {
   g = g_next;
   gm = gm_next;
-  if (item + 1 < item_hi) {
-    g_next = item_genome[item + 1];
-    gm_next = meta[g_next];
-  }
+  uint32_t t_next = 0;
+  if (tid == 0) t_next = atomicAdd(ticket, 1u);
+  uint32_t item_next = 0;
+  bool handed = false;
   n_bps = gm.n_bps;
-  if (n_bps < (uint64_t)K) continue;
-  n_starts = n_bps - K + 1;
+  n_starts = n_bps >= (uint64_t)K ? n_bps - K + 1 : 0;
   gseq = seq + gm.seq_off;
   gmask = seq + gm.mask_off;
   item_start = (uint64_t)(item - gm.item_first) * G::ITEM;
-  if (item_start >= n_starts) continue;
-  const uint64_t item_rem64 = n_bps - item_start;
+  const uint64_t item_rem64 = item_start < n_starts ? n_bps - item_start : 0;
   const uint32_t item_rem = (item_rem64 >> 32) != 0 ? ~0u : (uint32_t)item_rem64;
 #pragma unroll 1
   for (int tile = 0; tile < G::TILES; ++tile, ++tile_no) {
@@ -567,10 +566,16 @@
       }
       wave_live = wave_start < n_starts;
     }
-#ifndef HG_KS_EXP
-#define HG_KS_EXP 0
-#endif
-    if (!(HG_KS_EXP & 1)) __syncthreads();
+    if (tile == 0 && tid == 0) s_ticket[0] = t_next;
+    __syncthreads();
+    if (tile == 0) {
+      item_next = __builtin_amdgcn_readfirstlane(s_ticket[0]);
+      handed = true;
+      if (item_next < n_items) {
+        g_next = item_genome[item_next];
+        gm_next = meta[g_next];
+      }
+    }
 
     const bool tile_dirty = s_dirty[par] != 0u;
     inv_t inv_w = 0;
@@ -773,16 +778,24 @@
         else run_kmers(std::true_type{});
       }
     }
-    if (!(HG_KS_EXP & 1)) __syncthreads();
+    __syncthreads();
     if (tid == 0) s_dirty[par] = 0u;
-    if (dense_sampling(threshold)) {
-      if (HG_KS_EXP & 1) __syncthreads();
-      flush_hits_if_filling(stage, stage_cap, gm, g, hits, cnt);
-    }
-  }
-  if (item + 1 < item_hi) flush_hits<true>(stage, stage_cap, gm, g, hits, cnt);
-  else flush_hits(stage, stage_cap, gm, g, hits, cnt);
-  }
+    if (dense_sampling(threshold)) flush_hits_if_filling(stage, stage_cap, gm, g, hits, cnt);
+  }
+  if (!handed) {
+    if (tid == 0) s_ticket[0] = t_next;
+    __syncthreads();
+    item_next = __builtin_amdgcn_readfirstlane(s_ticket[0]);
+    if (item_next < n_items) {
+      g_next = item_genome[item_next];
+      gm_next = meta[g_next];
+    }
+  }
+  item = item_next;
+  if (item >= n_items) break;
+  flush_hits<true>(stage, stage_cap, gm, g, hits, cnt);
+  }
+  flush_hits(stage, stage_cap, gm, g, hits, cnt);
 }
 
 __device__ __forceinline__ uint32_t base_code(uint8_t c, uint32_t u2t) {
@@ -1041,16 +1054,19 @@
   if (k > 32) return 0;
   return k >= 22 ? (uint32_t)GeoS<32>::TILE : (uint32_t)GeoS<21>::TILE;
 }
-uint32_t hg_kmer_item_tiles(uint32_t k) { return k > 32 ? 0u : 3u * (uint32_t)GeoS<21>::TILES; }
+uint32_t hg_kmer_item_tiles(uint32_t k) { return k > 32 ? 0u : (uint32_t)GeoS<21>::TILES; }
+uint32_t hg_kmer_tile_span(uint32_t k) {
+  if (k > 32) return 0;
+  return k >= 22 ? (uint32_t)GeoS<32>::SPAN : (uint32_t)GeoS<21>::SPAN;
+}
 
 hipError_t hg_launch_kmer_sample(hipStream_t st, const uint8_t *d_seq, const hg_genome_meta *d_meta,
                                  const uint32_t *d_item_genome, uint32_t n_items, uint32_t ksize,
                                  uint64_t threshold, uint64_t seed, bool canonical, uint32_t norm_mode,
-                                 uint64_t *d_hits, uint32_t *d_cnt, bool packed, const uint32_t *d_group_first,
-                                 uint32_t n_groups) {
+                                 uint64_t *d_hits, uint32_t *d_cnt, bool packed, uint32_t *d_ticket, hg_kmer_residency *res,
+                                 uint32_t n_cu, uint32_t *grid_out) {
+  if (grid_out) *grid_out = ksize > 32 ? n_items : 0;
   if (n_items == 0) return hipSuccess;
-  if (ksize > 32 || n_groups == 0) d_group_first = nullptr;
-  const uint32_t n_wg = d_group_first ? n_groups : n_items;
   const uint32_t u2t = (norm_mode == HG_NORM_U2T && !packed) ? 1u : 0u;
   auto stage_entries = [&](uint32_t tile_starts) {
     const double per_tile = (double)tile_starts * ((double)threshold / 18446744073709551616.0);
@@ -1059,9 +1075,22 @@
     return cap;
   };
   const uint32_t cap_s = stage_entries((uint32_t)GeoS<21>::TILE), cap_l = stage_entries(LONG_TILE);
-#define HG_K_LAUNCH(KK, CN, PK)                                                                            \
-  hipLaunchKernelGGL((kmer_sample_shared<KK, CN, PK>), dim3(n_wg), dim3(WG), cap_s * sizeof(uint64_t), st, d_seq, d_meta, \
-                     d_item_genome, threshold, seed, u2t, d_hits, d_cnt, cap_s, d_group_first)
+  uint32_t slot_cap = 0;
+  while ((HIT_STAGE << slot_cap) < cap_s) ++slot_cap;
+  uint16_t *const wg_per_cu = ksize <= 32 ? &res->wg_per_cu[ksize][canonical ? 1 : 0][packed ? 1 : 0][slot_cap] : nullptr;
+#define HG_K_LAUNCH(KK, CN, PK)                                                                                          \
+  do {                                                                                                                   \
+    if (*wg_per_cu == 0) {                                                                                               \
+      int nb = 0;                                                                                                        \
+      const hipError_t e = hipOccupancyMaxActiveBlocksPerMultiprocessor(&nb, kmer_sample_shared<KK, CN, PK>, WG, cap_s * sizeof(uint64_t)); \
+      if (e != hipSuccess) return e;                                                                                     \
+      *wg_per_cu = (uint16_t)std::min(std::max(nb, 1), 64);                                                              \
+    }                                                                                                                    \
+    const uint32_t n_wg = (uint32_t)std::min<uint64_t>(n_items, (uint64_t)*wg_per_cu * std::max(n_cu, 1u));              \
+    if (grid_out) *grid_out = n_wg;                                                                                      \
+    hipLaunchKernelGGL((kmer_sample_shared<KK, CN, PK>), dim3(n_wg), dim3(WG), cap_s * sizeof(uint64_t), st, d_seq, d_meta, \
+                       d_item_genome, threshold, seed, u2t, d_hits, d_cnt, cap_s, d_ticket, n_items);                    \
+  } while (0)
 #define HG_K_CASE(KK)                                                                                     \
   case KK:                                                                                                \
     if (canonical && packed) HG_K_LAUNCH(KK, true, true);                                                 \
diff --git a/hyper-gen_amd/csrc/hg_sketch.h b/hyper-gen_amd/csrc/hg_sketch.h
--- a/hyper-gen_amd/csrc/hg_sketch.h
+++ b/hyper-gen_amd/csrc/hg_sketch.h
@@ -6,8 +6,6 @@
 struct hg_batch_tables {
   std::vector<hg_genome_meta> meta;
   std::vector<uint32_t> item_genome;
-  std::vector<uint32_t> group_first;
-  size_t n_groups = 0;
   uint64_t total_slots = 0;
   uint32_t max_cap = 0, max_expect = 0;
   size_t n_items = 0;
@@ -17,10 +15,7 @@
 };
 
 hg_status hg_check_sketch_params(hg_ctx *c, const hg_sketch_params *p);
-inline size_t hg_plan_group_offset(size_t n_items) { return (n_items + 3) & ~(size_t)3; }
-inline const uint32_t *hg_plan_group_table(const hg_ctx *c, size_t n_items, size_t n_groups) {
-  return n_groups ? static_cast<const uint32_t *>(c->w_items.p) + hg_plan_group_offset(n_items) : nullptr;
-}
+inline size_t hg_cnt_ticket_word(size_t n) { return 2 * n + 16; }
 
 hg_status hg_plan_build(hg_ctx *c, const hg_genome_batch &b, uint32_t ksize, uint64_t scaled,
                         const std::vector<uint32_t> *want_caps, hg_batch_tables &t);
diff --git a/hyper-gen_amd/csrc/hg_sketch_plan.hip b/hyper-gen_amd/csrc/hg_sketch_plan.hip
--- a/hyper-gen_amd/csrc/hg_sketch_plan.hip
+++ b/hyper-gen_amd/csrc/hg_sketch_plan.hip
@@ -25,11 +25,6 @@
 hg_status hg_plan_build(hg_ctx *c, const hg_genome_batch &b, uint32_t ksize, uint64_t scaled,
                         const std::vector<uint32_t> *want_caps, hg_batch_tables &t) {
   const uint64_t item_starts = hg_kmer_item_starts(ksize);
-  const uint32_t tile_starts = hg_kmer_tile_starts(ksize), item_tiles = hg_kmer_item_tiles(ksize);
-  const uint32_t full_item_tiles = tile_starts ? (uint32_t)((item_starts + tile_starts - 1) / tile_starts) : 0;
-  bool group_open = false;
-  t.group_first.clear();
-  uint32_t group_tiles = 0;
   t.meta.resize(b.n);
   t.item_genome.clear();
   t.reused = false;
@@ -56,23 +51,8 @@
     if (t.item_genome.size() + n_items > 0x7FFFFFFFull)
       return hg_fail(c, HG_ERR_UNSUPPORTED, "batch too large for one launch; split it");
     m.item_first = (uint32_t)t.item_genome.size();
-    if (tile_starts) {
-      for (uint64_t it = 0; it < n_items; ++it) {
-        const uint64_t starts = std::min<uint64_t>(item_starts, n_starts - it * item_starts);
-        const uint32_t tiles = (uint32_t)((starts + tile_starts - 1) / tile_starts);
-        const bool alone = tiles >= full_item_tiles;
-        if (!group_open || alone || group_tiles + tiles > item_tiles) {
-          t.group_first.push_back((uint32_t)(t.item_genome.size() + it));
-          group_tiles = 0;
-        }
-        group_tiles += tiles;
-        group_open = !alone;
-      }
-    }
     t.item_genome.insert(t.item_genome.end(), (size_t)n_items, (uint32_t)g);
   }
-  t.n_groups = t.group_first.size();
-  if (t.n_groups) t.group_first.push_back((uint32_t)t.item_genome.size());
   t.total_slots = slot;
   t.max_cap = max_cap;
   t.max_expect = (uint32_t)std::min<uint64_t>(max_expect, 0xFFFFFFF0ull);
@@ -92,9 +72,8 @@
 
 void hg_plan_tables_from_cache(const hg_sketch_plan &pl, size_t n, hg_batch_tables &t, bool with_meta) {
   t.total_slots = pl.total_slots, t.max_cap = pl.max_cap, t.max_expect = pl.max_expect, t.n_items = pl.n_items;
-  t.n_groups = pl.n_groups, t.reused = true;
+  t.reused = true;
   t.item_genome.clear();
-  t.group_first.clear();
   if (!with_meta) {
     t.meta.clear();
     return;
@@ -115,7 +94,7 @@
   hg_status s;
   const size_t n_items = t.item_genome.size();
   if ((s = hg_ensure(c, c->w_gmeta, n * sizeof(hg_genome_meta) + 16)) != HG_OK) return s;
-  const size_t items_words = t.n_groups ? hg_plan_group_offset(n_items) + t.n_groups + 1 : n_items;
+  const size_t items_words = n_items;
   if ((s = hg_ensure(c, c->w_items, items_words * sizeof(uint32_t) + 16)) != HG_OK) return s;
   const size_t pin_meta = (n * sizeof(hg_genome_meta) + 63) & ~(size_t)63;
   const size_t need = pin_meta + items_words * sizeof(uint32_t) + 64;
@@ -137,10 +116,6 @@
   HG_HIP(c, hipMemcpyAsync(c->w_gmeta.p, pin, n * sizeof(hg_genome_meta), hipMemcpyHostToDevice, c->stream));
   if (n_items) {
     std::memcpy(pin + pin_meta, t.item_genome.data(), n_items * sizeof(uint32_t));
-    if (t.n_groups) {
-      std::memset(pin + pin_meta + n_items * sizeof(uint32_t), 0, (hg_plan_group_offset(n_items) - n_items) * sizeof(uint32_t));
-      std::memcpy(pin + pin_meta + hg_plan_group_offset(n_items) * sizeof(uint32_t), t.group_first.data(), (t.n_groups + 1) * sizeof(uint32_t));
-    }
     HG_HIP(c, hipMemcpyAsync(c->w_items.p, pin + pin_meta, items_words * sizeof(uint32_t), hipMemcpyHostToDevice, c->stream));
   }
   HG_HIP(c, hipEventRecord(c->plan_uploaded, c->stream));
@@ -153,7 +128,6 @@
   for (size_t g = 0; g < n; ++g) pl->caps[g] = t.meta[g].hit_cap;
   pl->ksize = ksize, pl->scaled = scaled, pl->packed = b.packed;
   pl->total_slots = t.total_slots, pl->max_cap = t.max_cap, pl->max_expect = t.max_expect, pl->n_items = n_items;
-  pl->n_groups = t.n_groups;
   c->plan = std::move(pl);
   return HG_OK;
 }
@@ -189,12 +163,32 @@
   hg_batch_tables t;
   const hg_status s = hg_plan_build(nullptr, {nullptr, offsets, lens, nullptr, n, false}, ksize, scaled, nullptr, t);
   if (s != HG_OK) return s;
-  const uint32_t tile = hg_kmer_tile_starts(ksize);
-  counts[0] = t.n_items, counts[1] = t.n_groups ? t.n_groups : t.n_items, counts[2] = t.total_slots, counts[3] = t.max_cap;
-  counts[4] = t.max_expect, counts[5] = tile ? (hg_kmer_item_starts(ksize) + tile - 1) / tile : 0;
+  const uint64_t item_starts = hg_kmer_item_starts(ksize);
+  const uint32_t tile = hg_kmer_tile_starts(ksize), full_tiles = hg_kmer_item_tiles(ksize), group_cap = 3 * full_tiles;
+  std::vector<uint32_t> gf;
+  if (tile) {
+    bool group_open = false;
+    uint32_t group_tiles = 0;
+    for (size_t it = 0; it < t.n_items; ++it) {
+      const hg_genome_meta &m = t.meta[t.item_genome[it]];
+      const uint64_t n_starts = m.n_bps - ksize + 1;
+      const uint64_t starts = std::min<uint64_t>(item_starts, n_starts - (it - m.item_first) * item_starts);
+      const uint32_t tiles = (uint32_t)((starts + tile - 1) / tile);
+      const bool alone = tiles >= full_tiles;
+      if (!group_open || alone || group_tiles + tiles > group_cap) {
+        gf.push_back((uint32_t)it);
+        group_tiles = 0;
+      }
+      group_tiles += tiles;
+      group_open = !alone;
+    }
+    if (!gf.empty()) gf.push_back((uint32_t)t.n_items);
+  }
+  counts[0] = t.n_items, counts[1] = gf.empty() ? t.n_items : gf.size() - 1, counts[2] = t.total_slots, counts[3] = t.max_cap;
+  counts[4] = t.max_expect, counts[5] = full_tiles;
   if (group_first) {
-    if (t.group_first.size() > cap) return HG_ERR_CAPACITY;
-    for (size_t i = 0; i < t.group_first.size(); ++i) group_first[i] = t.group_first[i];
+    if (gf.size() > cap) return HG_ERR_CAPACITY;
+    for (size_t i = 0; i < gf.size(); ++i) group_first[i] = gf[i];
   }
   return HG_OK;
 }
diff --git a/hyper-gen_amd/csrc/hg_sketch_step.hip b/hyper-gen_amd/csrc/hg_sketch_step.hip
--- a/hyper-gen_amd/csrc/hg_sketch_step.hip
+++ b/hyper-gen_amd/csrc/hg_sketch_step.hip
@@ -63,18 +63,18 @@
   const size_t n = b.n;
   hg_status s;
   if ((s = hg_ensure(c, c->w_hits, t.total_slots * sizeof(uint64_t) + 16)) != HG_OK) return s;
-  if ((s = hg_ensure(c, c->w_cnt, (2 * n + 16) * sizeof(uint32_t) + 16)) != HG_OK) return s;
+  if ((s = hg_ensure(c, c->w_cnt, (hg_cnt_ticket_word(n) + 1) * sizeof(uint32_t) + 16)) != HG_OK) return s;
   auto *d_meta = static_cast<hg_genome_meta *>(c->w_gmeta.p);
   auto *d_hits = static_cast<uint64_t *>(c->w_hits.p);
   auto *d_cnt = static_cast<uint32_t *>(c->w_cnt.p);
   uint32_t *d_nd = d_cnt + n, *d_flags = sync_free ? d_cnt + 2 * n : nullptr;
-  HG_HIP(c, hipMemsetAsync(d_cnt, 0, (2 * n + (sync_free ? 16 : 0)) * sizeof(uint32_t), c->stream));
+  HG_HIP(c, hipMemsetAsync(d_cnt, 0, (hg_cnt_ticket_word(n) + 1) * sizeof(uint32_t), c->stream));
   {
     hg_timed tm(c, HG_T_KMER);
     c->last_kernel[HG_T_KMER] = hg_kmer_kernel_name(p->ksize, p->canonical != 0, b.packed);
     HG_HIP(c, hg_launch_kmer_sample(c->stream, b.d_seq, d_meta, static_cast<const uint32_t *>(c->w_items.p), (uint32_t)t.n_items,
                                     p->ksize, threshold, p->seed, p->canonical != 0, p->norm_mode, d_hits, d_cnt, b.packed,
-                                    hg_plan_group_table(c, t.n_items, t.n_groups), (uint32_t)t.n_groups));
+                                    d_cnt + hg_cnt_ticket_word(n), &c->kmer_res, (uint32_t)c->n_cu, &c->kmer_grid));
   }
   *sort_cap = first_sort_cap(c, t, sync_free);
   hg_timed tm(c, HG_T_SORT, HG_T_KMER);
diff --git a/include/hypergen.h b/include/hypergen.h
--- a/include/hypergen.h
+++ b/include/hypergen.h
@@ -87,6 +87,8 @@
 #define HG_NHASH_PENDING 0xFFFFFFFFu
 hg_status hg_sketch_plan_describe(const uint64_t *offsets, const uint64_t *lens, size_t n, uint32_t ksize, uint64_t scaled,
                                   uint64_t counts[6], uint32_t *group_first, size_t cap);
+hg_status hg_ctx_kmer_grid(hg_ctx *ctx, uint32_t *workgroups);
+hg_status hg_kmer_geometry(uint32_t ksize, uint32_t out[4]);
 hg_status hg_sketch_batch_dev_packed(hg_ctx *ctx, const uint8_t *d_blobs, const uint64_t *offsets,
                                      const uint64_t *n_bps, size_t n, const hg_sketch_params *p,
                                      int16_t *d_hv, int32_t *d_norm2, uint32_t *d_nhash);
```

Measured after the change: 127,700, median of 6. About the same (+1.0%).
